# jasperlinthorst/reveal

Measured on AMD Instinct MI355X. Metric: Mbp/s indexed+MUM-anchored (reveal rem), higher is better.
Workload: dtype int32

## Files before the change

reveal_amd/csrc/rv_align.hip:

```cpp
#include "rv_index.h"
#include "rv_split.h"
#include "rv_decide.h"
static_assert(RV_TSUB_TILE == RV_SPLIT_TILE, "one tile -> sub-index table serves the split passes and the multi-sample picker");
#include "rv_leaf.h"
#include "rv_cascade.h"
#include <string.h>
#include <algorithm>
#include <chrono>
#include <thread>
#include <atomic>
#include "rv_graphrem.h"

namespace {

double now_s() {
    return std::chrono::duration<double>(std::chrono::steady_clock::now().time_since_epoch()).count();
}

u64 hash_step(u64 acc, u64 i, int64_t v) {
    u64 x = (u64)v + (i + 1) * 0x9E3779B97F4A7C15ULL;
    x ^= x >> 30; x *= 0xbf58476d1ce4e5b9ULL;
    x ^= x >> 27; x *= 0x94d049bb133111ebULL;
    x ^= x >> 31;
    return acc + x;
// ... 133 lines not shown
    bool leaf_pending[RV_LEVEL_BUFS + 1] = {};
    size_t leaf_anchor_cap = 0, leaf_trace_cap = 0;
    std::vector<uint8_t> leaf_done;
    std::vector<RvLeafRoot> leaf_roots[2];
    Packer pk;
    std::vector<int> stamp; int epoch = 0;
    std::vector<sa_t> cb, ce, mb, me, cut_lo, cut_hi, mend_pos;
    std::vector<uint8_t> cc;
    std::vector<int> ctab_first, mtab_first, cut_first, mend_first, split_subs;
    std::vector<u32> sub_off_h;
    std::vector<int> tile_sub;
    std::vector<int64_t> mpre, sub_start, woff, toff, next_ss;
    const int64_t *d_next_ss = nullptr;
    const int *d_next_want = nullptr;
    const int *d_next_tsub = nullptr;
    std::vector<int> next_tsub;
    std::vector<u32> pick_l; std::vector<sa_t> pick_pos;
    std::vector<u32> child_base, child_n;
    std::vector<RvBubbleDesc> descs;
    std::vector<std::vector<RvBubbleDesc>> rounds;
    std::vector<RvBubbleDesc> kids_small, kids_big, kids_lds;
    struct Kid { int64_t off, n; int c0, c1; int64_t m0, wsum; };
    std::vector<Kid> kid_tmp;
    std::vector<u32> an_l; std::vector<int64_t> an_off, an_pos;
    bool trace_on = false;
    std::vector<rv_trace> trace;
    rv_align_stats st{};
    double lg[8] = {0}, lgx[8] = {0}, lg_t0 = 0;
    int leaf_flip = 0;
    bool leaf_launch_due = false, hook_early = false;
    size_t last_leaf_count = 0;
    bool running = false;
    u32 *lf_counters = nullptr; unsigned long long *lf_stats = nullptr; u32 *lf_l = nullptr; int64_t *lf_pos = nullptr; rv_trace *lf_tr = nullptr;
    size_t leaf_na = 0;
    void release() {
        if (leaf_stream) (void)hipStreamSynchronize(leaf_stream);
        if (leaf_stream2) (void)hipStreamSynchronize(leaf_stream2);
        if (bub_stream) { (void)hipStreamSynchronize(bub_stream); (void)hipStreamSynchronize(bub_stream2); }
        for (int k = 0; k < RV_LEVEL_BUFS; k++) { lvSA[k].release(); lvLCP[k].release(); lvBWT[k].release(); }
        scrSA.release(); scrLCP.release(); scrBWT.release(); cas.release();
        dTmin.release(); dPbReady.release(); dNextTsub.release(); dD.release(); dTab.release(); dTile.release(); dList.release(); dFlag.release(); dPar.release(); dDbg.release(); pk.release(); dDec.release(); dErr.release(); dTab0.release(); hLeafRoots[0].release(); hLeafRoots[1].release(); hLeafOut.release(); dLeaf.release(); dLeafRoots[0].release(); dLeafRoots[1].release();
        if (leaf_stream) { rv_stream_put(leaf_stream); leaf_stream = nullptr; }
        if (leaf_stream2) { rv_stream_put(leaf_stream2); leaf_stream2 = nullptr; }
        if (bub_stream) { rv_stream_put(bub_stream); bub_stream = nullptr; rv_stream_put(bub_stream2); bub_stream2 = nullptr; (void)hipEventDestroy(ev_fork); (void)hipEventDestroy(ev_join); (void)hipEventDestroy(ev_join2); ev_fork = ev_join = ev_join2 = nullptr; }
        if (ev_ready) { (void)hipEventDestroy(ev_ready); ev_ready = nullptr; }
        for (int k = 0; k <= RV_LEVEL_BUFS; k++) if (ev_leaf[k]) { (void)hipEventDestroy(ev_leaf[k]); ev_leaf[k] = nullptr; }
        for (int k = 0; k < 2; k++) if (ev_roots[k]) { (void)hipEventDestroy(ev_roots[k]); ev_roots[k] = nullptr; }
    }
};

void rv_align_free(rv_index *h) {
    if (h->al && h->al->feed) { (void)rv_replay_feed_finish(h->al->feed); h->al->feed = nullptr; }
    if (h->al) { h->al->release(); delete h->al; h->al = nullptr; }
}

static int report_dev_err(u32 err) {
    if (err & 1u) { rv_set_error("split: the intervals returned by graphalign do not partition the sub-index (child size mismatch)"); return -1; }
    if (err & 4u) { rv_set_error("device-side decision: a picked match does not lie inside the intervals of its sub-index"); return -1; }
    if (err & 2u) { rv_set_error("bubble_sort (data-parallel rounds): a mover found no landing site"); return -1; }
    if (err & 16u) { rv_set_error("bubble_sort (data-parallel rounds): a tile waited in vain for the tile above it (workgroups not dispatched in index order?)"); return -1; }
    if (err) { rv_set_error("device-side error word %u", err); return -1; }
    return 0;
}

static int64_t bubble_par_default(bool multi) { return multi ? (int64_t)262144 : (int64_t)RV_BUBBLE_PAR_N; }

// ... 342 lines not shown
        d.child_n = t.child_n; d.child_base = t.child_base; d.sub_off = t.sub_off; d.expect_total = t.expect_total;
        d.err = a->dErr.as<u32>();
        d.kid = kid;
    };
    if (a->multi) {
        RvDecideMultiArgs d;
        outputs(d);
        d.W = W; d.minl = a->minl; d.minn = a->minn;
        d.nodes = a->d_next_nodes; d.want = a->d_next_want;
        d.pick_l = h->ws.misc[13].as<u32>(); d.pick_pos = h->ws.misc[7].as<sa_t>();
        d.cand_count = h->ws.misc[1].as<u32>() + RV_MULTI_REGIONS * 64;
        d.cand_cap = (u32)std::min<size_t>(h->ws.misc[8].cap / RV_MULTI_CAND_BYTES / RV_MULTI_REGIONS, 0xffffffffu);
        RV_TRY(rv_decide_multi_launch(h->ws, d));
    } else {
        RvDecideArgs d;
        outputs(d);
        d.nodes = a->d_next_nodes; d.flags = a->d_next_flags; d.picks = h->hscan.as<RvPairRec>();
        d.ovf_cap = (u32)std::min<size_t>(h->ws.misc[4].cap / sizeof(RvPairRec), 0xffffffffu);
        RV_TRY(rv_decide_launch(h->ws, d));
    }
    RvLabelTabs lt; RvSplitArgs sa;
    split_args(h, t, nxt, lt, sa);
    int64_t biggest = 0;
    for (int s2 = 0; s2 < ns; s2++) biggest = std::max<int64_t>(biggest, lv.n[(size_t)s2]);
    if (biggest > a->par_min_cur) RV_TRY(tmin_preset(h, sa));
    int id = h->prof.begin(q, RV_K_SPLIT, (double)m * (2 * (sizeof(sa_t) + sizeof(lcp_t) + 2)) + (double)m * (sizeof(sa_t) + sizeof(lcp_t) + 1));
    RV_TRY(rv_split_launch(h->ws, cur_sa(h), cur_lcp(h), a->dD.as<uint8_t>(), cur_bwt(h), m, lt, sa, 1));
    h->prof.end(q, id);
    a->early_done = true;
    a->early_bubble = false;
    const bool all_classes = a->multi || ns > 4096;
    if (biggest <= a->par_min_cur && !h->ws.opt.no_early_bubble &&
        (a->multi || (!h->ws.opt.bubble_lds_always && (!all_classes || h->ws.opt.early_bubble_many)))) {
        RV_TRY(rv_lower_ranges_launch(h->ws, h->dT.as<uint8_t>(), t.mb, t.me, W * ns));
        RV_TRY(bubble_flags(h, m));
        RvBubbleArgs ba;
        memset(&ba, 0, sizeof ba);
        ba.flag = a->dFlag.as<uint8_t>();
        ba.SA = sa.SA_out; ba.LCP = sa.LCP_out; ba.BWT = sa.BWT_out; ba.SAi = sa.SAi; ba.cut_lo = t.cut_lo; ba.cut_hi = t.cut_hi; ba.err = a->dErr.as<u32>();
        id = h->prof.begin(q, RV_K_BUBBLE, 0.0);
        if (!all_classes) {
            RV_TRY(rv_bubble_children_dev_launch(h->ws, ba, kid, ns, a->par_min_cur));
        } else {
            RV_TRY(bubble_fork(h, true, true, true));
            Workspace wl, wk; wl.stream = a->bub_stream; wk.stream = a->bub_stream2;
            RV_TRY(rv_bubble_children_dev_classes_launch(wl, wk, ba, kid, ns, a->par_min_cur));
            RV_TRY(bubble_join(h, true, true));
        }
        h->prof.end(q, id);
        a->early_bubble = true;
    }
    return 0;
}

static int level_hook(rv_index *h) {
    Align *a = h->al;
    if (a->hook_early) RV_TRY(early_split(h));
    if (a->leaf_launch_due) RV_TRY(leaf_launch(h));
    return 0;
}

static void build_preselection(Align *a) {
    const int ns = a->lv.size();
    a->sel.clear(); a->sel_first.assign((size_t)ns + 1, 0);
    std::vector<int64_t> &tmp = a->sel_tmp;
    for (int s = 0; s < ns; s++) {
// ... 589 lines not shown
        a->d_next_tsub = a->dNextTsub.as<int>();
    }
    return 0;
}

static int commit_split(rv_index *h, const Commit &cm, RvSplitArgs &sa) {
    Align *a = h->al;
    hipStream_t q = h->ws.stream;
    const Level &lv = a->lv;
    const int nxt = cm.nxt;
    uint8_t *tb = a->dTab.as<uint8_t>();
    RV_TRY(split_reserve(h, nxt, lv.m, cm.m_next));
    RV_TRY(a->dList.reserve((size_t)a->woff.back() * 4 + 64));
    RV_TRY(leaf_wait(h, nxt));
    if (h->ws.opt.bubble_parent_scratch && !a->descs.empty()) RV_TRY(leaf_wait(h, a->level == 0 ? RV_LEVEL_BUFS : a->cur));
    SplitTabs t;
    t.sub_start = (const int64_t *)(tb + cm.o_ss); t.tile_sub = (const int *)(tb + cm.o_tsub);
    t.ctab_first = (int *)(tb + cm.o_ctf); t.mtab_first = (int *)(tb + cm.o_mtf); t.cut_first = (int *)(tb + cm.o_cf); t.mend_first = (int *)(tb + cm.o_mf);
    t.cb = (sa_t *)(tb + cm.o_cb); t.ce = (sa_t *)(tb + cm.o_ce); t.cc = tb + cm.o_cc; t.mb = (sa_t *)(tb + cm.o_mb); t.me = (sa_t *)(tb + cm.o_me);
    t.cut_lo = (sa_t *)(tb + cm.o_clo); t.cut_hi = (sa_t *)(tb + cm.o_chi); t.mend_pos = (sa_t *)(tb + cm.o_mp);
    t.child_n = (u32 *)(tb + cm.o_cn); t.child_base = (u32 *)(tb + cm.o_cbase); t.sub_off = (u32 *)(tb + cm.o_suboff); t.expect_total = (u32 *)(tb + cm.o_expect);
    t.total = (u32 *)(tb + cm.o_total);
    t.nmatch = (int)a->mb.size();
    RvLabelTabs lt;
    split_args(h, t, nxt, lt, sa);
    sa.mend_all = a->dec.host_lists ? 1 : 0;
    int id = a->early_done ? -1 : h->prof.begin(q, RV_K_SPLIT, (double)lv.m * (2 * (sizeof(sa_t) + sizeof(lcp_t) + 2)) + (double)cm.m_next * (sizeof(sa_t) + sizeof(lcp_t) + 1));
    if (!a->early_done) {
        if (!a->descs.empty()) RV_TRY(tmin_preset(h, sa));
        RV_TRY(rv_split_launch(h->ws, cur_sa(h), cur_lcp(h), a->dD.as<uint8_t>(), cur_bwt(h), lv.m, lt, sa, (int)a->split_subs.size()));
    }
    h->prof.end(q, id);
    if (!a->early_bubble) {
        if (lt.nmatch > 256 && a->mpre.back() / lt.nmatch <= 512) RV_TRY(rv_lower_ranges_launch(h->ws, h->dT.as<uint8_t>(), lt.mbegin, lt.mend, lt.nmatch));
        else RV_TRY(rv_lower_launch(h->ws, h->dT.as<uint8_t>(), lt.mbegin, lt.mend, (const int64_t *)(tb + cm.o_mpre), lt.nmatch, a->mpre.back()));
    }
    return 0;
}

static int commit_bubble(rv_index *h, const Commit &cm, const RvSplitArgs &sa) {
    Align *a = h->al;
    hipStream_t q = h->ws.stream;
    uint8_t *tb = a->dTab.as<uint8_t>();
    const int64_t m_next = cm.m_next;
    if (a->descs.empty() && a->kids_small.empty() && a->kids_big.empty() && a->kids_lds.empty()) return 0;
    RvBubbleArgs ba;
    ba.desc = (const RvBubbleDesc *)(tb + cm.o_desc); ba.woff = (const int64_t *)(tb + cm.o_woff);
    ba.cnt = (u32 *)(tb + cm.o_bcnt); ba.list = a->dList.as<u32>();
    RV_TRY(bubble_flags(h, m_next));
    ba.flag = a->dFlag.as<uint8_t>();
    ba.SA = sa.SA_out; ba.LCP = sa.LCP_out; ba.BWT = sa.BWT_out; ba.SAi = sa.SAi; ba.cut_lo = sa.cut_lo; ba.cut_hi = sa.cut_hi; ba.err = sa.err;
    ba.state = (RvBubbleState *)(tb + cm.o_bstate);
    ba.dbg = nullptr;
    if (h->ws.opt.level_log) { if (!a->dDbg.p) { RV_TRY(a->dDbg.reserve(64)); RV_HIP(hipMemsetAsync(a->dDbg.p, 0, 64, q)); } ba.dbg = a->dDbg.as<unsigned long long>(); }
    ba.scrSA = const_cast<sa_t *>(cur_sa(h)); ba.scrLCP = const_cast<lcp_t *>(cur_lcp(h)); ba.scrBWT = const_cast<uint8_t *>(cur_bwt(h));
    if (!a->descs.empty() && !h->ws.opt.bubble_parent_scratch) {
        RV_TRY(a->scrSA.reserve((size_t)(m_next + 64) * sizeof(sa_t)));
        RV_TRY(a->scrLCP.reserve((size_t)(m_next + 64) * sizeof(lcp_t)));
        RV_TRY(a->scrBWT.reserve((size_t)m_next + 64));
        ba.scrSA = a->scrSA.as<sa_t>(); ba.scrLCP = a->scrLCP.as<lcp_t>(); ba.scrBWT = a->scrBWT.as<uint8_t>();
    }
    if (!a->descs.empty()) {
        const size_t W = (size_t)a->woff.back() + 16, TT = (size_t)a->toff.back() + 16;
        RV_TRY(a->dPar.reserve(TT * 4 + W * (8 + 7 * 4 + sizeof(sa_t) + 2) + 256));
        uint8_t *pb = a->dPar.as<uint8_t>();
        ba.par.toff = (const int64_t *)(tb + cm.o_toff);
// ... 94 lines not shown

static int builtin_leaf_setup(rv_index *h) {
    Align *a = h->al;
    hipStream_t q = h->ws.stream;
    a->use_leaf = !a->multi && !h->ws.opt.no_leaf && a->picker == 0;
    a->leaf_flip = 0;
    if (!a->use_leaf) return 0;
    a->leaf_anchor_cap = (size_t)(h->nT / std::max(a->minl, 1)) + 1024;
    a->leaf_trace_cap = a->trace_on ? 2 * a->leaf_anchor_cap + 1024 : 0;
    const size_t bytes = 256 + a->leaf_anchor_cap * (4 + 8 + 8) + a->leaf_trace_cap * sizeof(rv_trace) + 64;
    RV_TRY(a->dLeaf.reserve(bytes));
    uint8_t *base = a->dLeaf.as<uint8_t>();
    a->lf_counters = (u32 *)base;
    a->lf_stats = (unsigned long long *)(base + 64);
    a->lf_pos = (int64_t *)(base + 256); a->lf_l = (u32 *)(a->lf_pos + 2 * a->leaf_anchor_cap);
    a->lf_tr = (rv_trace *)(base + 256 + a->leaf_anchor_cap * 20 + ((8 - (a->leaf_anchor_cap * 20) % 8) % 8));
    RV_HIP(hipMemsetAsync(base, 0, 256, q));
    if (!a->leaf_stream) {
        RV_HIP(rv_stream_get(&a->leaf_stream));
        RV_HIP(rv_stream_get(&a->leaf_stream2));
        RV_HIP(hipEventCreateWithFlags(&a->ev_ready, hipEventDisableTiming));
        for (int k = 0; k <= RV_LEVEL_BUFS; k++) RV_HIP(hipEventCreateWithFlags(&a->ev_leaf[k], hipEventDisableTiming));
        for (int k = 0; k < 2; k++) RV_HIP(hipEventCreateWithFlags(&a->ev_roots[k], hipEventDisableTiming));
    }
    for (int k = 0; k <= RV_LEVEL_BUFS; k++) a->leaf_pending[k] = false;
    a->roots_inflight[0] = a->roots_inflight[1] = false;
    return 0;
}

static int builtin_setup(rv_index *h, int minl, int minn) {
    RV_TRY(align_begin(h, minl, minn, h->al && h->al->trace_on));
    Align *a = h->al;
    a->full_only = !a->trace_on && a->picker == 0;
    a->an_l.clear(); a->an_off.assign(1, 0); a->an_pos.clear(); a->trace.clear(); a->leaf_na = 0;
    a->seeds_cur.clear(); a->seeds_lead.clear(); a->seeds_trail.clear(); a->picker_calls = a->picker_seeded = 0; a->picker_ns = a->picker_list_ns = a->galign_ns = 0;
    if (a->picker == 1) {
        if ((int)h->nodes.size() != h->nsamples) { rv_set_error("the native picker (rv_set_picker) takes one sequence per sample: %d sequences in %d samples", (int)h->nodes.size(), h->nsamples); return -1; }
        if (h->rc) { rv_set_error("the native picker (rv_set_picker) with construct(rc=1) is not supported"); return -1; }
    }
    if (a->picker != 0 && a->multi && !a->trace_on) { a->presel_on = true; a->pick_filter = true; }
    else a->pick_filter = false;
    if (a->picker == 2) {
        if (!a->ggraph) { rv_set_error("rv_set_graph_picker: no graph"); return -1; }
        if (h->rc) { rv_set_error("the native picker (rv_set_graph_picker) with construct(rc=1) is not supported"); return -1; }
        a->g_left.assign((size_t)a->lv.size(), RvGraphIv{-1, -1}); a->g_right.assign((size_t)a->lv.size(), RvGraphIv{-1, -1});
    }
    const bool use_leaf = !a->multi && !h->ws.opt.no_leaf && a->picker == 0;
    a->use_leaf = use_leaf;
    if (!a->multi && a->full_only && h->n < ((int64_t)1 << 32)) {
        prep_level_tables(h, a->lv, h->n);
        if (a->next_dev_ok) {
            a->pk.clear();
            RV_TRY(publish_next_tables(h, a->dTab0, a->lv.nsamples, false));
            a->cur_dev_ok = true;
        }
    }
    RV_TRY(builtin_leaf_setup(h));
    a->running = true;
    return 0;
}

struct PickScratch {
    std::vector<u32> pk_l, pk_sl; std::vector<int32_t> pk_n, pk_sn; std::vector<int64_t> pk_off, pk_mpos, pk_sb, pk_ib, pk_ie, pk_soff, pk_spos, pk_ssc;
    std::vector<uint16_t> pk_mso, pk_sso; std::vector<uint8_t> pk_srt;
};
struct PickRes {
    int rc = -9;
// ... 352 lines not shown
        const size_t lo = na / nt * t, hi = t + 1 == nt ? na : na / nt * (t + 1);
        th.emplace_back([=]() { for (size_t k = lo; k < hi; k++) off[k] = base + 2 * (int64_t)(k + 1); });
    }
    for (size_t k = 0; k < na / nt; k++) off[k] = base + 2 * (int64_t)(k + 1);
    for (auto &x : th) x.join();
}
static int builtin_finish(rv_index *h, rv_align_stats *out) {
    Align *a = h->al;
    hipStream_t q = h->ws.stream;
    h->rb.direct = false;
    if (a->use_leaf && a->running) {
        u32 *lf_counters = a->lf_counters; u32 *lf_l = a->lf_l; int64_t *lf_pos = a->lf_pos; rv_trace *lf_tr = a->lf_tr;
        RV_HIP(hipStreamSynchronize(a->leaf_stream));
        RV_HIP(hipStreamSynchronize(a->leaf_stream2));
        for (int k = 0; k <= RV_LEVEL_BUFS; k++) a->leaf_pending[k] = false;
        RV_TRY(a->hLeafOut.reserve(256));
        RV_HIP(hipMemcpyAsync(a->hLeafOut.p, lf_counters, 128, hipMemcpyDeviceToHost, q));
        RV_HIP(hipStreamSynchronize(q));
        u32 cnt[4]; unsigned long long stv[8];
        memcpy(cnt, a->hLeafOut.p, sizeof cnt); memcpy(stv, a->hLeafOut.as<uint8_t>() + 64, sizeof stv);
        if (h->ws.opt.leaf_prof)
            fprintf(stderr, "leaf: steps %llu splits %llu | cycles idle %llu scan %llu split %llu bubble %llu\n", stv[0], stv[1], stv[4], stv[5], stv[6], stv[7]);
        if (cnt[2]) { rv_set_error(cnt[2] & 4u ? "leaf kernel: recursion stack overflow" : "leaf kernel: a sub-index does not match its intervals"); return -1; }
        if (cnt[0] > a->leaf_anchor_cap || cnt[1] > a->leaf_trace_cap) { rv_set_error("leaf kernel: output buffer too small"); return -1; }
        a->leaf_na = 0;
        if (cnt[0]) {
            const size_t na = cnt[0];
            const size_t nl = a->an_l.size(), np = a->an_pos.size();
            rv_index::ResultBufs &rb = h->rb;
            rb.direct = rb.l && (int64_t)(nl + na) <= rb.l_cap && (int64_t)(nl + na + 1) <= rb.off_cap && (int64_t)(np + 2 * na) <= rb.pos_cap;
            int64_t *pp; u32 *pl;
            if (rb.direct) { pp = rb.pos + np; pl = rb.l + nl; }
            else { RV_TRY(a->hLeafOut.reserve(na * 20 + 64)); pp = a->hLeafOut.as<int64_t>(); pl = (u32 *)(pp + 2 * na); }
            RV_HIP(hipMemcpyAsync(pp, lf_pos, na * 16, hipMemcpyDeviceToHost, a->leaf_stream));
            RV_HIP(hipMemcpyAsync(pl, lf_l, na * 4, hipMemcpyDeviceToHost, a->leaf_stream));
            RV_TRY(rv_leaf_lower_launch(h->ws, h->dT.as<uint8_t>(), lf_pos, lf_l, (u32)na));
            if (rb.direct) fill_offsets(rb.off + nl + 1, na, (int64_t)np);
            RV_HIP(hipStreamSynchronize(a->leaf_stream));
            RV_HIP(hipStreamSynchronize(q));
            a->leaf_na = na;
        }
        if (a->trace_on && cnt[1]) {
            const size_t at = a->trace.size();
            a->trace.resize(at + cnt[1]);
            RV_HIP(hipMemcpy(a->trace.data() + at, lf_tr, (size_t)cnt[1] * sizeof(rv_trace), hipMemcpyDeviceToHost));
        }
        a->st.steps += (int64_t)stv[0]; a->st.splits += (int64_t)stv[1]; a->st.anchored_bp += (int64_t)stv[2];
        if ((int64_t)stv[3] > a->st.maxdepth) a->st.maxdepth = (int32_t)stv[3];
    }
    a->running = false;
    if (out) *out = a->st;
    return 0;
}

static int install_frontier(rv_index *h, int level, int nsubs, const int64_t *meta, const int64_t *node_first, const int64_t *nodes, int64_t m,
                            const void *sa, const void *lcp, const void *bwt, int on_device);
static int builtin_cascade(rv_index *h) {
    Align *a = h->al;
    memset(&a->cas_out, 0, sizeof a->cas_out);
    if (a->trace_on || h->rc != 0 || h->n <= RV_LEAF_N || a->minl < 4 || h->ws.opt.no_cascade || a->picker != 0) return 0;
    const bool second_try = !a->multi && a->use_leaf && h->ws.opt.cascade_second == 2;
    auto interval_cascade = [&]() -> int {
        RvCascadeMultiOut mo;
        RV_TRY(rv_cascade_multi_run(h, a->cas, a->minl, &mo));
        a->cas_out.done = mo.done; a->cas_out.levels = mo.levels; a->cas_out.cands = mo.cands; a->cas_out.witnesses = mo.witnesses; a->cas_out.children = mo.children;
        a->cas_out.undecided = mo.undecided; a->cas_out.rebuilt_ranks = mo.rebuilt_ranks; a->cas_out.why = mo.why;
        if (!mo.done) return 0;
        const int k = h->nsamples;
        a->st.splits += (int64_t)mo.an_l.size(); a->st.steps += mo.steps; a->st.levels += mo.levels; a->st.scanned_ranks += h->n;
        if (mo.maxdepth > a->st.maxdepth) a->st.maxdepth = mo.maxdepth;
        h->main_arrays_freed = true;
        if (mo.undecided > 0) {
            RV_TRY(install_frontier(h, 1, (int)mo.undecided, mo.meta.data(), mo.node_first.data(), mo.nodes.data(), mo.rebuilt_ranks, mo.d_sa, mo.d_lcp, mo.d_bwt, 1));
        } else {
            a->lv.clear();
            a->level = 1;
        }
        {
            const size_t na = mo.an_l.size(), l0 = a->an_l.size(), p0 = a->an_pos.size(), o0 = a->an_off.size();
            a->an_l.insert(a->an_l.end(), mo.an_l.begin(), mo.an_l.end());
            a->an_pos.resize(p0 + na * (size_t)k);
            for (size_t x = 0; x < na * (size_t)k; x++) a->an_pos[p0 + x] = (int64_t)mo.an_pos[x];
            a->an_off.resize(o0 + na);
            for (size_t x = 0; x < na; x++) a->an_off[o0 + x] = (int64_t)(p0 + (x + 1) * (size_t)k);
            int64_t bp = 0;
            for (size_t x = 0; x < na; x++) bp += mo.an_l[x];
            a->st.anchored_bp += bp;
            (void)l0;
        }
        return 0;
    };
    if (a->multi || second_try) return interval_cascade();
    if (!a->use_leaf) return 0;
    RvCascadeIO io;
    io.anchor_count = a->lf_counters; io.anchor_cap = (u32)a->leaf_anchor_cap; io.anchor_l = a->lf_l; io.anchor_pos = a->lf_pos;
    io.stats = a->lf_stats; io.leaf_err = a->lf_counters + 2;
    io.stage_cap = (u32)h->ws.opt.leaf_acap;
    io.lvSA = &a->lvSA[0]; io.lvLCP = &a->lvLCP[0]; io.lvBWT = &a->lvBWT[0]; io.roots = &a->dLeafRoots[0];
    const int dmode = (int)h->ws.opt.cascade_danger;
    RV_TRY(rv_cascade_run(h, a->cas, io, a->minl, &a->cas_out, dmode == 2 ? 1 : 0, 0));
    if (!a->cas_out.done && a->cas_out.undecided > 0 && dmode == 1) {
        RV_HIP(hipMemsetAsync(a->dLeaf.p, 0, 256, h->ws.stream));
        RV_TRY(rv_cascade_run(h, a->cas, io, a->minl, &a->cas_out, 1, 1));
    }
    if (!a->cas_out.done) {
        RV_HIP(hipMemsetAsync(a->dLeaf.p, 0, 256, h->ws.stream));
        if (a->cas_out.undecided > 0 && !h->ws.opt.cascade_second_off) return interval_cascade();
        return 0;
    }
    a->st.levels += a->cas_out.levels;
    a->st.scanned_ranks += h->n;
    if (!a->cas.lin_rest.empty() && h->nodes.size() > 2) {
        std::vector<RvIntv> rest, gone;
        for (size_t k = 0; k + 1 < a->cas.lin_rest.size(); k += 2) rest.push_back({a->cas.lin_rest[k], a->cas.lin_rest[k + 1]});
        std::sort(rest.begin(), rest.end(), intv_less);
        for (const RvIntv &v : h->nodes) {
            if (v.end <= v.begin) continue;
            const auto it = std::lower_bound(rest.begin(), rest.end(), v, intv_less);
            if (it == rest.end() || it->begin != v.begin) gone.push_back(v);
        }
        RV_TRY(add_decision(h, 0, 0, nullptr, 0, gone.data(), (int)gone.size(), nullptr, 0, nullptr, 0, rest.data(), (int)rest.size()));
        a->dec.drop_lead = true;
        RV_TRY(rv_frontier_commit(h, nullptr));
        for (size_t s2 = 0; s2 < a->lv.depth.size(); s2++) a->lv.depth[s2] = a->cas.lin_rest_depth;
        return 0;
    }
    h->main_arrays_freed = true;
    a->level = 1;
    a->lv.clear();
    return 0;
}

int rv_cascade_info(const rv_index *h, int64_t *out) {
    for (int k = 0; k < 8; k++) out[k] = 0;
    if (!h->al) return 0;
    const RvCascadeOut &c = h->al->cas_out;
    out[0] = c.done ? 1 : 0; out[1] = c.levels; out[2] = c.cands; out[3] = c.witnesses; out[4] = c.children; out[5] = c.undecided; out[6] = c.rebuilt_ranks; out[7] = c.solved;
    return 0;
}

const char *rv_cascade_why(const rv_index *h) {
    if (!h->al || h->al->cas_out.done || !h->al->cas_out.why) return "";
    return h->al->cas_out.why;
}
// ... 143 lines not shown
    return 0;
}


int rv_frontier_import(rv_index *h, int minl, int minn, uint32_t maxlcp, int level, int nsubs, const int64_t *meta,
                       const int64_t *node_first, const int64_t *nodes, int64_t m, const void *sa, const void *lcp, const void *bwt, int on_device) {
    RV_HIP(hipSetDevice(h->device));
    if (h->nsamples < 2) { rv_set_error("align needs at least two samples"); return -1; }
    if (nsubs < 0 || m < 0 || m >= ((int64_t)1 << 32)) { rv_set_error("rv_frontier_import: bad sizes"); return -1; }
    const bool fresh = !(h->al && h->al->running);
    if (fresh) {
        if (h->text_only) h->maxlcp = maxlcp;
        else if (!h->constructed || h->main_arrays_freed) RV_TRY(rv_text_only(h, maxlcp));
        const bool keep_trace = h->al && h->al->trace_on;
        if (!h->al) h->al = new Align();
        Align *a = h->al;
        a->trace_on = keep_trace;
        a->minl = minl; a->minn = minn;
        a->multi = h->nsamples > 2;
        a->scanned = false; a->d_err = nullptr; a->flag_clean = false;
        a->next_dev_ok = a->cur_dev_ok = a->early_done = a->early_bubble = false;
        a->par_min_cur = (h->ws.opt.bubble_par_min >= 0 ? h->ws.opt.bubble_par_min : bubble_par_default(a->multi));
        RV_TRY(a->dErr.reserve(64));
        memset(&a->st, 0, sizeof a->st);
        a->full_only = !a->trace_on && a->picker == 0;
        a->pick_filter = a->picker != 0 && a->multi && !a->trace_on;
        if (a->pick_filter) a->presel_on = true;
        if (a->picker == 2) { rv_set_error("rv_frontier_import: a run on a graph (rv_set_graph_picker) is not handed off -- its sub-indices share the graph"); return -1; }
        if (a->picker == 1) {
            if ((int)h->nodes.size() != h->nsamples) { rv_set_error("the native picker (rv_set_picker) takes one sequence per sample: %d sequences in %d samples", (int)h->nodes.size(), h->nsamples); return -1; }
            if (h->rc) { rv_set_error("the native picker (rv_set_picker) with construct(rc=1) is not supported"); return -1; }
        }
        a->picker_calls = a->picker_seeded = 0; a->picker_ns = a->picker_list_ns = a->galign_ns = 0;
        a->an_l.clear(); a->an_off.assign(1, 0); a->an_pos.clear(); a->trace.clear(); a->leaf_na = 0;
        RV_TRY(builtin_leaf_setup(h));
    }
    RV_TRY(install_frontier(h, level, nsubs, meta, node_first, nodes, m, sa, lcp, bwt, on_device));
    h->al->running = true;
    return 0;
}

int64_t rv_frontier_seeds_export(rv_index *h, const int32_t *subs, int k, int64_t *out, int64_t cap) {
    if (need_align(h)) return -1;
    const Align *a = h->al;
    const int ns = a->lv.size();
    int64_t need = 0;
    for (int pass = 0; pass < 2; pass++) {
        int64_t at = 0;
        for (int i = 0; i < k; i++) {
            const int s = subs[i];
            if (s < 0 || s >= ns) { rv_set_error("sub-index %d out of range", s); return -1; }
            const Align::SeedList *sd = (s < (int)a->seeds_cur.size() && a->seeds_cur[(size_t)s].size() > 0) ? &a->seeds_cur[(size_t)s] : nullptr;
            if (pass) out[at] = sd ? (int64_t)sd->size() : 0;
            at++;
            if (!sd) continue;
            for (size_t r = 0; r < sd->size(); r++) {
                const int64_t mem = sd->off[r + 1] - sd->off[r];
                if (pass) {
                    out[at] = sd->l[r]; out[at + 1] = sd->n[r]; out[at + 2] = sd->score[r]; out[at + 3] = mem;
                    for (int64_t q2 = 0; q2 < mem; q2++) { out[at + 4 + 2 * q2] = sd->so[(size_t)(sd->off[r] + q2)]; out[at + 5 + 2 * q2] = sd->pos[(size_t)(sd->off[r] + q2)]; }
                }
                at += 4 + 2 * mem;
            }
        }
        need = at;
        if (!out || cap < need) break;
    }
// ... 370 lines not shown
```

reveal_amd/csrc/rv_api.hip:

```cpp
#include "rv_index.h"
#include "rv_cascade.h"
#include <limits>
#include <stdarg.h>
#include <stdio.h>
#include <string.h>
#include <limits.h>
#include <algorithm>
#include <thread>

static thread_local char g_err[1024] = "";

void rv_set_error(const char *fmt, ...) {
    va_list ap;
    va_start(ap, fmt);
    vsnprintf(g_err, sizeof g_err, fmt, ap);
    va_end(ap);
}

static std::vector<rv_index *> &live_handles() { static std::vector<rv_index *> v; return v; }
std::mutex &rv_trim_mutex() { static std::mutex *m = new std::mutex(); return *m; }
bool rv_oom_trim() {
    size_t got = 0;
    bool log = false;
    int caller_dev = 0;
// ... 40 lines not shown
        rv_set_error("device %d is %s; this library is built for gfx950 (MI355X) only", device, prop.gcnArchName);
        return nullptr;
    }
    rv_index *h = new rv_index();
    h->device = device;
    if (rv_stream_get(&h->ws.stream) != hipSuccess) {
        rv_set_error("hipStreamCreate failed");
        delete h;
        return nullptr;
    }
    h->T.push_back('\0');
    h->ws.prof_ctx = &h->prof;
    h->ws.prof_begin_fn = [](void *c, hipStream_t st, int k, double b) { return ((RvProf *)c)->begin(st, k, b); };
    h->ws.prof_end_fn = [](void *c, hipStream_t st, int id) { ((RvProf *)c)->end(st, id); };
    { std::lock_guard<std::mutex> g(rv_trim_mutex()); live_handles().push_back(h); }
    return h;
}

void rv_free(rv_index *h) {
    if (!h) return;
    { std::lock_guard<std::mutex> g(rv_trim_mutex()); auto &v = live_handles(); v.erase(std::remove(v.begin(), v.end(), h), v.end()); }
    (void)hipSetDevice(h->device);
    if (h->ws.stream) (void)hipStreamSynchronize(h->ws.stream);
    h->rb.direct = false;
    (void)rv_set_result_buffers(h, nullptr, 0, nullptr, 0, nullptr, 0);
    rv_align_free(h);
    h->prof.release();
    h->dT.release(); h->dT0.release(); h->dSA.release(); h->dSAi.release(); h->dLCP.release(); h->dBWT.release(); h->dNsep.release();
    h->ws.release();
    h->hscan.release();
    for (auto &b : h->ps) b.release();
    h->hupload.release();
    if (h->ev_picks) { (void)hipEventDestroy(h->ev_picks); h->ev_picks = nullptr; }
    if (h->ws.stream) rv_stream_put(h->ws.stream);
    delete h;
}

int rv_set_option(rv_index *h, const char *name, int64_t value) {
    if (!h || !name) { rv_set_error("rv_set_option: null argument"); return -1; }
    int64_t *f = h->ws.opt.find(name);
    if (!f) { rv_set_error("rv_set_option: unknown option %s", name); return -1; }
    *f = value;
    return 0;
}
int rv_set_launch_trace(int on) {
    const int was = g_rv_launch_trace;
    g_rv_launch_trace = on != 0;
    return was;
}
int rv_get_option(rv_index *h, const char *name, int64_t *value) {
    if (!h || !name || !value) { rv_set_error("rv_get_option: null argument"); return -1; }
    const int64_t *f = h->ws.opt.find(name);
    if (!f) { rv_set_error("rv_get_option: unknown option %s", name); return -1; }
    *value = *f;
    return 0;
}
int rv_option_count(void) {
    int c = 0;
#define RV_X_(f, nm, def) c++;
    RV_OPTION_LIST(RV_X_)
#undef RV_X_
    return c;
}
const char *rv_option_name(int k) {
    static const char *const names[] = {
#define RV_X_(f, nm, def) nm,
        RV_OPTION_LIST(RV_X_)
#undef RV_X_
    };
    return k >= 0 && k < rv_option_count() ? names[k] : nullptr;
}

rv_index *rv_clone(rv_index *h) {
    if (!h->constructed || h->main_arrays_freed) { rv_set_error("Index not yet constructed."); return nullptr; }
    if (rv_need_sai(h)) return nullptr;
    rv_index *c = rv_new(h->device);
    if (!c) return nullptr;
    try { c->T = h->T; c->nsep = h->nsep; c->nodes = h->nodes; }
    catch (...) { rv_set_error("copy of the index: out of host memory"); rv_free(c); return nullptr; }
    if (c->T.size() != h->T.size()) { rv_free(c); return nullptr; }
    c->nsamples = h->nsamples; c->n = h->n; c->nT = h->nT; c->rc = h->rc;
    c->maxlcp = h->maxlcp; c->sa_stats = h->sa_stats; c->text_dirty = true;
    c->ws.opt = h->ws.opt;
    const int64_t n = h->n;
    hipStream_t q = c->ws.stream;
    bool ok = rv_upload(c) == 0;
    ok = ok && c->dT.reserve((size_t)n + 64) == 0 && c->dSA.reserve((size_t)(n + 64) * sizeof(sa_t)) == 0 && c->dSAi.reserve((size_t)(n + 64) * sizeof(sa_t)) == 0
            && c->dLCP.reserve((size_t)(n + 64) * sizeof(lcp_t)) == 0 && c->dBWT.reserve((size_t)n + 64) == 0 && c->dNsep.reserve((h->nsep.size() + 1) * sizeof(sa_t)) == 0;
    ok = ok && hipStreamSynchronize(h->ws.stream) == hipSuccess;
    ok = ok && hipMemcpyAsync(c->dT.p, h->dT.p, (size_t)n + 64, hipMemcpyDeviceToDevice, q) == hipSuccess;
    ok = ok && hipMemcpyAsync(c->dSA.p, h->dSA.p, (size_t)n * sizeof(sa_t), hipMemcpyDeviceToDevice, q) == hipSuccess;
    ok = ok && hipMemcpyAsync(c->dSAi.p, h->dSAi.p, (size_t)n * sizeof(sa_t), hipMemcpyDeviceToDevice, q) == hipSuccess;
    ok = ok && hipMemcpyAsync(c->dLCP.p, h->dLCP.p, (size_t)n * sizeof(lcp_t), hipMemcpyDeviceToDevice, q) == hipSuccess;
    ok = ok && hipMemcpyAsync(c->dBWT.p, h->dBWT.p, (size_t)n, hipMemcpyDeviceToDevice, q) == hipSuccess;
    ok = ok && hipMemcpyAsync(c->dNsep.p, h->dNsep.p, (h->nsep.size() + 1) * sizeof(sa_t), hipMemcpyDeviceToDevice, q) == hipSuccess;
    ok = ok && hipStreamSynchronize(q) == hipSuccess;
    if (!ok) { rv_set_error("copy of the index failed"); rv_free(c); return nullptr; }
    c->nsep_dev = h->nsep_dev;
    c->constructed = true; c->sai_valid = true;
    return c;
}

int rv_add_sample(rv_index *h) {
    if (h->nsamples > 0) h->nsep.push_back(h->n - 1);
    h->nsamples++;
    h->constructed = false; h->text_only = false;
    return 0;
}

int rv_add_sequence(rv_index *h, const char *seq, int64_t len, int64_t *begin, int64_t *end) {
    if (len < 0 || !seq) { rv_set_error("addsequence: bad sequence"); return -1; }
#ifndef RV_SA64
    if ((uint64_t)h->n + (uint64_t)(len + 1) + 1 > (uint64_t)INT_MAX) {
        rv_set_error("Total amount of sequence too large, use \"reveal <subcommand> --64\" to use 64 bit suffix arrays instead.");
        return -1;
    }
#endif
    const int64_t s = h->n;
    if ((size_t)(h->n + len + 2) > h->T.cap) (void)hipSetDevice(h->device);
// ... 198 lines not shown
            RV_HIP(hipMemcpyAsync(h->dT0.as<char>() + at, dst, len, hipMemcpyHostToDevice, q));
            RV_HIP(hipEventRecord(ev[slot], q));
            used[slot] = true;
        }
        RV_HIP(hipStreamSynchronize(q));
    }
    RV_HIP(hipStreamSynchronize(q));
    h->text_dirty = false;
    return 0;
}

int rv_upload_again(rv_index *h) {
    h->text_dirty = true;
    return rv_upload(h);
}

int rv_construct(rv_index *h, int rc, const char *safile, const char *lcpfile, int cache) {
    RV_HIP(hipSetDevice(h->device));
    if (rc == 1) {
        if (h->nsep.empty()) { rv_set_error("construct(rc=1) needs at least two samples"); return -1; }
        h->rc = 1;
        revcomp(h->T.data() + h->nsep[0], h->n - h->nsep[0]);
        h->text_dirty = true;
    } else {
        h->rc = 0;
    }
    if (h->n == 0) { rv_set_error("No text to index."); return -1; }
    const int64_t n = h->n;
    if (n >= ((int64_t)1 << 32) - 2) { rv_set_error("index of %lld positions: this build carries ranks in 32 bits (n < 2^32 - 2)", (long long)n); return -1; }
    if (cache == 1) RV_TRY(write_raw(".reveal.t", h->T.data(), (size_t)n));
    if (h->al) (void)rv_align_end(h);
    h->nT = n;
    hipStream_t q = h->ws.stream;
    RV_TRY(rv_upload(h));
    RV_TRY(h->dT.reserve((size_t)n + 64));
    RV_HIP(hipMemcpyAsync(h->dT.p, h->dT0.p, (size_t)n + 64, hipMemcpyDeviceToDevice, q));
    RV_TRY(h->dSA.reserve((size_t)(n + 64) * sizeof(sa_t)));
    RV_TRY(h->dSAi.reserve((size_t)(n + 64) * sizeof(sa_t)));
    RV_TRY(h->dLCP.reserve((size_t)(n + 64) * sizeof(lcp_t)));
    RV_TRY(h->dBWT.reserve((size_t)n + 64));
    memset(&h->sa_stats, 0, sizeof h->sa_stats);
    RV_TRY(h->ws.misc[0].reserve(64));
    u32 *d_max = h->ws.misc[0].as<u32>();
    const sa_t side_sep = !h->nsep.empty() ? (sa_t)h->nsep[0] : std::numeric_limits<sa_t>::max();
    const bool lcp_from_file = lcpfile && lcpfile[0];
    bool lcp_done = false;
    SaScratchInUse in_use(h->ws);
    if (!safile || !safile[0]) {
        int id = h->prof.begin(q, RV_K_SA_SORT, 5.0 * (double)n);
        if (lcp_from_file) RV_TRY(rv_build_sa(h->ws, h->dT.as<uint8_t>(), n, h->dSA.as<sa_t>(), &h->sa_stats));
        else RV_TRY(rv_build_sa(h->ws, h->dT.as<uint8_t>(), n, h->dSA.as<sa_t>(), &h->sa_stats, h->dLCP.as<lcp_t>(), h->dBWT.as<uint8_t>(), side_sep, d_max, &lcp_done,
                                 h->nsep.data(), (int)h->nsep.size()));
        h->prof.end(q, id);
    } else {
        std::vector<sa_t> tmp((size_t)n);
        RV_TRY(read_raw(safile, tmp.data(), (size_t)n * sizeof(sa_t)));
        RV_HIP(hipMemcpyAsync(h->dSA.p, tmp.data(), (size_t)n * sizeof(sa_t), hipMemcpyHostToDevice, q));
        RV_HIP(hipStreamSynchronize(q));
    }
    h->sai_valid = false;
    if (safile && safile[0]) { RV_TRY(rv_build_inverse_checked(h->ws, h->dSA.as<sa_t>(), h->dSAi.as<sa_t>(), n)); h->sai_valid = true; }
    if (!lcp_from_file) {
        if (!lcp_done) {
            int id = h->prof.begin(q, RV_K_LCP, 13.0 * (double)n);
            RV_TRY(rv_build_lcp(h->ws, h->dT.as<uint8_t>(), h->dSA.as<sa_t>(), false, h->dLCP.as<lcp_t>(), n, d_max, h->dBWT.as<uint8_t>(), side_sep));
            h->prof.end(q, id);
        }
        RV_TRY(rv_read_back(h->ws, &h->maxlcp, d_max, 4));
    } else {
        std::vector<lcp_t> tmp((size_t)n);
        RV_TRY(read_raw(lcpfile, tmp.data(), (size_t)n * sizeof(lcp_t)));
        u32 mx = 0;
        for (int64_t i = 0; i < n; i++) if ((u32)tmp[(size_t)i] > mx) mx = (u32)tmp[(size_t)i];
        h->maxlcp = mx;
        RV_HIP(hipMemcpyAsync(h->dLCP.p, tmp.data(), (size_t)n * sizeof(lcp_t), hipMemcpyHostToDevice, q));
        RV_TRY(rv_build_bwt(h->ws, h->dT.as<uint8_t>(), h->dSA.as<sa_t>(), n, h->dBWT.as<uint8_t>(), side_sep));
        RV_HIP(hipStreamSynchronize(q));
    }
    if (cache == 1) {
        std::vector<sa_t> sa((size_t)n);
        std::vector<lcp_t> lc((size_t)n);
        RV_HIP(hipMemcpy(sa.data(), h->dSA.p, (size_t)n * sizeof(sa_t), hipMemcpyDeviceToHost));
        RV_HIP(hipMemcpy(lc.data(), h->dLCP.p, (size_t)n * sizeof(lcp_t), hipMemcpyDeviceToHost));
        RV_TRY(write_raw(".reveal.sa", sa.data(), (size_t)n * sizeof(sa_t)));
        RV_TRY(write_raw(".reveal.lcp", lc.data(), (size_t)n * sizeof(lcp_t)));
    }
    {
        if (h->nsep_dev != h->nsep || !h->dNsep.p) {
            std::vector<sa_t> ns(h->nsep.size() + 1, 0);
            for (size_t k = 0; k < h->nsep.size(); k++) ns[k] = (sa_t)h->nsep[k];
            RV_TRY(h->dNsep.reserve(ns.size() * sizeof(sa_t)));
            RV_HIP(hipMemcpy(h->dNsep.p, ns.data(), ns.size() * sizeof(sa_t), hipMemcpyHostToDevice));
            h->nsep_dev = h->nsep;
        }
    }
    h->constructed = true;
    h->main_arrays_freed = false;
    h->text_only = false;
    return 0;
}

int64_t rv_get_array(rv_index *h, int which, void *out, int64_t cap) {
    (void)hipSetDevice(h->device);
    const int64_t n = h->n;
    switch (which) {
    case RV_T:
        if (cap < n) { rv_set_error("buffer too small"); return -1; }
        if (h->constructed || h->text_only) {
            if (hipMemcpy(out, h->dT.p, (size_t)n, hipMemcpyDeviceToHost) != hipSuccess) { rv_set_error("D2H failed"); return -1; }
        } else {
            memcpy(out, h->T.data(), (size_t)n);
        }
        return n;
    case RV_SA: case RV_SAI: case RV_LCP: {
        if (!h->constructed || (which != RV_SAI && h->main_arrays_freed)) { rv_set_error("Index not yet constructed."); return -2; }
        if (which == RV_SAI && rv_need_sai(h)) return -2;
        if (cap < h->nT && which == RV_SAI) { rv_set_error("buffer too small"); return -1; }
        if (cap < n && which != RV_SAI) { rv_set_error("buffer too small"); return -1; }
        const void *src = which == RV_SA ? h->dSA.p : which == RV_SAI ? h->dSAi.p : h->dLCP.p;
        const size_t esz = which == RV_LCP ? sizeof(lcp_t) : sizeof(sa_t);
        const int64_t cnt = which == RV_SAI ? h->nT : n;
        (void)hipStreamSynchronize(h->ws.stream);
        if (hipMemcpy(out, src, (size_t)cnt * esz, hipMemcpyDeviceToHost) != hipSuccess) { rv_set_error("D2H failed"); return -1; }
        return cnt;
    }
    case RV_SO: {
        if (!h->constructed || h->nsamples <= 2) { rv_set_error("SO not available."); return -2; }
        if (cap < h->nT) { rv_set_error("buffer too small"); return -1; }
        uint16_t *so = (uint16_t *)out;
        int64_t j = 0;
        for (int i = 0; i < h->nsamples; i++) {
            const int64_t hi = (i == h->nsamples - 1) ? h->nT - 1 : h->nsep[(size_t)i];
            for (; j <= hi; j++) so[j] = (uint16_t)i;
        }
        return h->nT;
    }
    case RV_NSEP:
        if (cap < (int64_t)h->nsep.size()) { rv_set_error("buffer too small"); return -1; }
        for (size_t k = 0; k < h->nsep.size(); k++) ((int64_t *)out)[k] = h->nsep[k];
        return (int64_t)h->nsep.size();
    case RV_NODES:
        if (cap < (int64_t)h->nodes.size() * 2) { rv_set_error("buffer too small"); return -1; }
        for (size_t k = 0; k < h->nodes.size(); k++) { ((int64_t *)out)[2 * k] = h->nodes[k].begin; ((int64_t *)out)[2 * k + 1] = h->nodes[k].end; }
        return (int64_t)h->nodes.size() * 2;
    }
    rv_set_error("unknown array id %d", which);
    return -1;
}

}

int rv_need_sai(rv_index *h) {
    if (h->sai_valid) return 0;
    if (!h->constructed || h->main_arrays_freed) { rv_set_error("the inverse suffix array was not requested before align() consumed the main index"); return -1; }
    RV_HIP(hipSetDevice(h->device));
    RV_TRY(rv_build_inverse(h->ws, h->dSA.as<sa_t>(), h->dSAi.as<sa_t>(), h->n));
    h->sai_valid = true;
    return 0;
}

int rv_text_only(rv_index *h, u32 maxlcp) {
    RV_HIP(hipSetDevice(h->device));
    if (h->n == 0) { rv_set_error("No text to index."); return -1; }
    if (h->nsep.empty()) { rv_set_error("a worker index needs at least two samples"); return -1; }
    const int64_t n = h->n;
    hipStream_t q = h->ws.stream;
    h->rc = 0; h->nT = n;
    RV_TRY(rv_upload(h));
    RV_TRY(h->dT.reserve((size_t)n + 64));
    RV_HIP(hipMemcpyAsync(h->dT.p, h->dT0.p, (size_t)n + 64, hipMemcpyDeviceToDevice, q));
    RV_TRY(h->dSAi.reserve((size_t)(n + 64) * sizeof(sa_t)));
    std::vector<sa_t> ns(h->nsep.size() + 1, 0);
    for (size_t k = 0; k < h->nsep.size(); k++) ns[k] = (sa_t)h->nsep[k];
    RV_TRY(h->dNsep.reserve(ns.size() * sizeof(sa_t)));
    RV_HIP(hipMemcpy(h->dNsep.p, ns.data(), ns.size() * sizeof(sa_t), hipMemcpyHostToDevice));
    h->nsep_dev = h->nsep;
    RV_HIP(hipStreamSynchronize(q));
    h->maxlcp = maxlcp;
    h->constructed = false; h->main_arrays_freed = true; h->text_only = true; h->sai_valid = false;
    return 0;
}

namespace {
__global__ __launch_bounds__(256) void k_ps_keys(const RvPairRec *__restrict__ recs, u32 total, const int64_t *__restrict__ ss, int ns, u64 *__restrict__ keys, u32 *__restrict__ vals) {
    const u32 i = blockIdx.x * 256u + threadIdx.x;
    if (i >= total) return;
    const int64_t r = (int64_t)recs[i].rank;
    int lo = 0, hi = ns;
    while (hi - lo > 1) { const int mid = (lo + hi) >> 1; if (ss[mid] <= r) lo = mid; else hi = mid; }
    keys[i] = ((u64)(u32)lo << 32) | (u64)recs[i].l;
    vals[i] = i;
}
__global__ __launch_bounds__(256) void k_ps_mark(const u64 *__restrict__ skeys, const u32 *__restrict__ svals, u32 total, u32 presel, u32 *__restrict__ flag) {
    const u32 p = blockIdx.x * 256u + threadIdx.x;
    if (p >= total) return;
    const u64 next = ((skeys[p] >> 32) + 1ull) << 32;
    u32 lo = p, hi = total;
    while (hi - lo > 1) { const u32 mid = lo + ((hi - lo) >> 1); if (skeys[mid] < next) lo = mid; else hi = mid; }
    flag[svals[p]] = (hi - p <= presel) ? 1u : 0u;
}
__global__ __launch_bounds__(256) void k_ps_emit(const RvPairRec *__restrict__ recs, const u32 *__restrict__ flag, const u32 *__restrict__ off, u32 total, RvPairRec *__restrict__ out) {
    const u32 i = blockIdx.x * 256u + threadIdx.x;
    if (i < total && flag[i]) out[off[i]] = recs[i];
// ... 588 lines not shown
```

reveal_amd/csrc/rv_cascade.h:

```cpp
#pragma once
#include "rv_common.h"
#include <vector>

struct RvCascadeBufs {
    DBuf d[40];
    HBuf hstage, hstage2;
    u32 M = 0, NW = 0;
    u32 lin_roots = 0, lin_picks = 0, lin_nA = 0, lin_nB = 0;
    int64_t lin_steps = 0; int lin_maxdepth = 0; size_t lin_off[6] = {0, 0, 0, 0, 0, 0};
    std::vector<int64_t> lin_rest; int lin_rest_depth = 0;
    hipStream_t prio_stream = nullptr; hipEvent_t ev_in = nullptr, ev_out = nullptr;
    void release() {
        for (auto &b : d) b.release(); hstage.release(); hstage2.release();
        if (prio_stream) { (void)hipStreamDestroy(prio_stream); prio_stream = nullptr; }
        if (ev_in) { (void)hipEventDestroy(ev_in); ev_in = nullptr; }
        if (ev_out) { (void)hipEventDestroy(ev_out); ev_out = nullptr; }
    }
};

struct RvCascadeIO {
    u32 *anchor_count; u32 anchor_cap; u32 *anchor_l; int64_t *anchor_pos;
    unsigned long long *stats;
    u32 *leaf_err;
    u32 stage_cap;
    DBuf *lvSA, *lvLCP, *lvBWT, *roots;
};

struct RvCascadeOut {
    bool done;
    int levels;
    int64_t cands, witnesses, children, undecided, rebuilt_ranks;
    int64_t solved, unsolved;
    const char *why;
};

#define RV_CASM_K 16
struct RvCascadeMultiOut {
    bool done; int levels; int64_t cands, witnesses, children, undecided, rebuilt_ranks, steps; int maxdepth; const char *why;
    int64_t big, big_ranks;
    std::vector<u32> an_l; std::vector<int64_t> an_pos;
    std::vector<int64_t> meta, node_first, nodes;
    const void *d_sa, *d_lcp, *d_bwt;
};

struct rv_index;
struct RvBatchGroup;
RvBatchGroup *rv_batch_group_new(int device);
void rv_batch_group_begin(RvBatchGroup *g, int total);
void rv_batch_group_leave(RvBatchGroup *g);
void rv_batch_group_free(RvBatchGroup *g);
void rv_batch_group_info(const RvBatchGroup *g, int64_t *out);
int rv_cascade_multi_run(rv_index *h, RvCascadeBufs &cb, int minl, RvCascadeMultiOut *out);
int rv_cascade_run(rv_index *h, RvCascadeBufs &cb, const RvCascadeIO &io, int minl, RvCascadeOut *out, int danger = 0, int reuse = 0);
```

reveal_amd/csrc/rv_cascade.hip:

```cpp
#include "rv_index.h"
#include "rv_cascade.h"
#include "rv_leaf.h"
#include <algorithm>
#include <string.h>
#include <stdio.h>
#include <stdlib.h>
#include <chrono>

namespace {

constexpr int TB = 256;
constexpr u32 NONE = 0xFFFFFFFFu;
#ifdef RV_SA64
constexpr int KEY_SHIFT = 40;
#else
constexpr int KEY_SHIFT = 32;
#endif
constexpr u64 KEY_LOW = (1ull << KEY_SHIFT) - 1;

struct CasIv { sa_t a0, a1, b0, b1; };
struct CasRes { sa_t qa, qb; u32 ql, lead, trail, state; };
enum { C_NCHILD = 0, C_NUND = 1, C_NWIT = 2, C_ERR = 3, C_MAXN = 4, C_LO = 5, C_HI = 6, C_LEVELS = 7, C_NSOLVED = 8, C_NUNSOLVED = 9, C_NRETRY = 10, C_TICKET = 11 };

__device__ inline bool cas_cut(const CasIv &iv, int64_t pa, int64_t pb, int64_t len, int64_t minl, int64_t *qa, int64_t *qb, int64_t *ql) {
    const int64_t ka = (int64_t)iv.a0 - pa, kb = (int64_t)iv.b0 - pb;
    int64_t k = ka > kb ? ka : kb;
    k = k > 0 ? k : 0;
    const int64_t a = pa + k, b = pb + k;
    int64_t l = len - k;
    const int64_t ra = (int64_t)iv.a1 - a, rb = (int64_t)iv.b1 - b;
    l = l < ra ? l : ra;
    l = l < rb ? l : rb;
    *qa = a; *qb = b; *ql = l;
    return l >= minl;
}
__device__ inline u64 cas_key(int64_t qa, int64_t ql) { return ((u64)ql << KEY_SHIFT) | (KEY_LOW - (u64)qa); }

__device__ inline u64 shfl_up64(u64 v, int d) {
    const u32 lo = __shfl_up((u32)v, d, 64), hi = __shfl_up((u32)(v >> 32), d, 64);
    return ((u64)hi << 32) | lo;
}
__device__ inline void seg_atomic_max64(u64 *__restrict__ dst, u32 child, u64 val, bool active) {
    const int lane = threadIdx.x & 63;
    if (!active) { child = NONE; val = 0; }
    val = rv_wave_seg_max_u64(child, val);
    const u32 nc = __shfl_down(child, 1, 64);
    const bool last = lane == 63 || nc != child;
    if (active && last && val > dst[child]) atomicMax((unsigned long long *)&dst[child], (unsigned long long)val);
}
__device__ inline void seg_atomic_max32(u32 *__restrict__ dst, u32 child, u32 val, bool active) {
    const int lane = threadIdx.x & 63;
    if (!active) { child = NONE; val = 0; }
    val = rv_wave_seg_max_u32(child, val);
    const u32 nc = __shfl_down(child, 1, 64);
    const bool last = lane == 63 || nc != child;
// ... 501 lines not shown
                    iv[slot] = c; best[slot] = 0; wmax[slot] = 0; depth[slot] = dp + 1; res[slot] = nr;
                    if (danger) { dg.best[slot] = 0; dg.flag[slot] = 0; dg.ceil[slot] = 0; }
                    r.lead = slot;
                } else atomicOr(&counters[C_ERR], 1u);
                slot++;
            }
            if (trail) {
                if (slot < child_cap) {
                    CasIv c; c.a0 = (sa_t)((int64_t)r.qa + r.ql); c.a1 = p.a1; c.b0 = (sa_t)((int64_t)r.qb + r.ql); c.b1 = p.b1;
                    iv[slot] = c; best[slot] = 0; wmax[slot] = 0; depth[slot] = dp + 1; res[slot] = nr;
                    if (danger) { dg.best[slot] = 0; dg.flag[slot] = 0; dg.ceil[slot] = 0; }
                    r.trail = slot;
                } else atomicOr(&counters[C_ERR], 1u);
            }
            const u32 as = base_a + (u32)__popcll(b_split & lt);
            if (as < io.anchor_cap) { io.anchor_l[as] = r.ql; io.anchor_pos[2 * (size_t)as] = (int64_t)r.qa; io.anchor_pos[2 * (size_t)as + 1] = (int64_t)r.qb; }
            else atomicOr(&counters[C_ERR], 4u);
            r.state = 1;
        } else {
            r.state = 2;
        }
        if (in) res[id] = r;
        if (und) {
            und_list[base_u + (u32)__popcll(b_und & lt)] = id;
            if ((u64)(la + lb) > (u64)leaf_n) atomicMax(&counters[C_MAXN], (u32)((la + lb) > 0xFFFFFFFFll ? 0xFFFFFFFFll : (la + lb)));
        }
        __syncthreads();
    }
    if (threadIdx.x == 0) {
        __threadfence();
        if (atomicAdd(&counters[C_TICKET], 1u) == gridDim.x - 1) {
            if (hi > lo) counters[C_LEVELS]++;
            counters[C_LO] = hi; counters[C_HI] = atomicAdd(&counters[C_NCHILD], 0u);
            counters[C_TICKET] = 0;
        }
    }
}
__global__ __launch_bounds__(TB) void k_cas_stats(const u32 *__restrict__ counters, const int32_t *__restrict__ depth, RvCascadeIO io) {
    __shared__ unsigned long long s_bp[TB / 64];
    __shared__ u32 s_md[TB / 64];
    const u32 nchild = counters[C_NCHILD], na = *io.anchor_count;
    unsigned long long bp = 0; u32 md = 0;
    for (u32 i = blockIdx.x * TB + threadIdx.x; i < na; i += gridDim.x * TB) bp += io.anchor_l[i];
    for (u32 i = blockIdx.x * TB + threadIdx.x; i < nchild; i += gridDim.x * TB) { const u32 d = (u32)depth[i]; md = d > md ? d : md; }
#pragma unroll
    for (int d = 32; d >= 1; d >>= 1) {
        bp += ((unsigned long long)(u32)__shfl_down((u32)(bp >> 32), d, 64) << 32) + (unsigned long long)(u32)__shfl_down((u32)bp, d, 64);
        const u32 om = __shfl_down(md, d, 64);
        md = om > md ? om : md;
    }
    if ((threadIdx.x & 63) == 0) { s_bp[threadIdx.x >> 6] = bp; s_md[threadIdx.x >> 6] = md; }
    __syncthreads();
    if (threadIdx.x == 0) {
        for (int k = 1; k < TB / 64; k++) { bp += s_bp[k]; md = s_md[k] > md ? s_md[k] : md; }
        if (bp) atomicAdd(&io.stats[2], bp);
        if (md) atomicMax(&io.stats[3], (unsigned long long)md);
        if (blockIdx.x == 0) { atomicAdd(&io.stats[0], (unsigned long long)(nchild - counters[C_NUND] - counters[C_NRETRY])); atomicAdd(&io.stats[1], (unsigned long long)na); }
    }
}

__global__ __launch_bounds__(TB) void k_cas_sizes(const u32 *__restrict__ und_list, u32 U, const CasIv *__restrict__ iv, u64 *__restrict__ sizes) {
    const u32 u = blockIdx.x * TB + threadIdx.x;
    if (u < U) { const CasIv p = iv[und_list[u]]; sizes[u] = (u64)(((int64_t)p.a1 - p.a0) + ((int64_t)p.b1 - p.b0)); }
    if (u == U) sizes[u] = 0;
}
__global__ __launch_bounds__(TB) void k_cas_roots(const u32 *__restrict__ und_list, u32 U, const CasIv *__restrict__ iv, const int32_t *__restrict__ depth,
// ... 187 lines not shown
    if (nLiveA + nLiveB > 0) {
        if (stalled || (nLiveA && nLiveB && chain_wmax() >= minl)) {
            for (size_t c = 0; c < nA; c++) if (liveA[c]) { cb.lin_rest.push_back(CA[c].begin); cb.lin_rest.push_back(CA[c].end); }
            for (size_t c = 0; c < nB; c++) if (liveB[c]) { cb.lin_rest.push_back(CB[c].begin); cb.lin_rest.push_back(CB[c].end); }
        } else { steps++; maxdepth = depth; }
    }
    const u32 R = (u32)roots.size(), P = (u32)anl.size();
    RV_TRY(broots.reserve((size_t)std::max<u32>(R, 1) * sizeof(CasIv))); RV_TRY(bdepth.reserve((size_t)std::max<u32>(R, 1) * 4));
    const size_t tab_bytes = (nA + nB) * (sizeof(sa_t) + 4) + (size_t)P * 8 + 64;
    RV_TRY(btabs.reserve(tab_bytes + 64)); RV_TRY(banch.reserve((size_t)P * (4 + 16) + 64));
    std::vector<uint8_t> stage(tab_bytes + 64, 0);
    size_t o = 0;
    auto put = [&](const void *src, size_t bytes) { memcpy(stage.data() + o, src, bytes); const size_t at = o; o += (bytes + 15) / 16 * 16; return at; };
    std::vector<sa_t> bA(nA), bB(nB);
    for (size_t c = 0; c < nA; c++) bA[c] = (sa_t)CA[c].begin;
    for (size_t c = 0; c < nB; c++) bB[c] = (sa_t)CB[c].begin;
    stage.resize((nA + nB) * (sizeof(sa_t) + 4) + (size_t)P * 8 + 16 * 8 + 64);
    const size_t oA = put(bA.data(), nA * sizeof(sa_t)), oB = put(bB.data(), nB * sizeof(sa_t)), opA = put(pickA.data(), nA * 4), opB = put(pickB.data(), nB * 4),
                 oL = put(rootLead.data(), (size_t)P * 4), oT = put(rootTrail.data(), (size_t)P * 4);
    RV_TRY(btabs.reserve(o + 64));
    RV_HIP(hipMemcpyAsync(btabs.p, stage.data(), o, hipMemcpyHostToDevice, q));
    if (R) {
        RV_HIP(hipMemcpyAsync(broots.p, roots.data(), (size_t)R * sizeof(CasIv), hipMemcpyHostToDevice, q));
        RV_HIP(hipMemcpyAsync(bdepth.p, rdepth.data(), (size_t)R * 4, hipMemcpyHostToDevice, q));
    }
    RV_HIP(hipMemcpyAsync(banch.p, anp.data(), (size_t)P * 16, hipMemcpyHostToDevice, q));
    RV_HIP(hipMemcpyAsync((uint8_t *)banch.p + (size_t)P * 16, anl.data(), (size_t)P * 4, hipMemcpyHostToDevice, q));
    RV_HIP(hipStreamSynchronize(q));
    cb.lin_roots = R; cb.lin_picks = P; cb.lin_nA = (u32)nA; cb.lin_nB = (u32)nB; cb.lin_steps = steps; cb.lin_maxdepth = maxdepth;
    cb.lin_off[0] = oA; cb.lin_off[1] = oB; cb.lin_off[2] = opA; cb.lin_off[3] = opB; cb.lin_off[4] = oL; cb.lin_off[5] = oT;
    return 0;
}

int rv_cascade_run(rv_index *h, RvCascadeBufs &cb, const RvCascadeIO &io, int minl_in, RvCascadeOut *out, int danger, int reuse) {
    memset(out, 0, sizeof *out);
    out->done = false;
    Workspace &ws = h->ws;
    hipStream_t q = ws.stream;
    const int64_t n = h->n;
    const u32 minl = (u32)std::max(minl_in, 1);
    const bool verbose = (ws.opt.cascade_log != 0);
    double tp[6] = {0, 0, 0, 0, 0, 0};
    if (verbose) { (void)hipStreamSynchronize(q); tp[0] = cas_now(); }
#define GIVE_UP(msg) do { out->why = msg; if (verbose) fprintf(stderr, "cascade: gave up: %s\n", msg); return 0; } while (0)
    if (h->nsamples != 2 || h->nsep.size() != 1 || h->nodes.size() < 2) GIVE_UP("not two samples");
    std::vector<RvIntv> CA, CB;
    for (const RvIntv &v : h->nodes) if (v.end > v.begin) (v.begin < h->nsep[0] ? CA : CB).push_back(v);
    std::sort(CA.begin(), CA.end(), [](const RvIntv &x, const RvIntv &y) { return x.begin < y.begin; });
    std::sort(CB.begin(), CB.end(), [](const RvIntv &x, const RvIntv &y) { return x.begin < y.begin; });
    if (CA.empty() || CB.empty()) GIVE_UP("an empty sample");
    const bool chain = CA.size() > 1 || CB.size() > 1;
    if (chain && ws.opt.no_cascade_chain) GIVE_UP("several sequences per sample (switched off)");
    if (n >= ((int64_t)1 << 32) - 2) GIVE_UP("index above 2^32 positions");
#ifdef RV_SA64
    if ((u64)h->maxlcp >= (1ull << 24) || n >= ((int64_t)1 << 40)) GIVE_UP("bid word too narrow");
#endif
    CasIv root; root.a0 = root.a1 = root.b0 = root.b1 = 0;
    root.a0 = (sa_t)CA[0].begin; root.a1 = (sa_t)CA[0].end; root.b0 = (sa_t)CB[0].begin; root.b1 = (sa_t)CB[0].end;
    if (root.a0 >= root.a1 || root.b0 >= root.b1 || (int64_t)root.a1 > h->nsep[0] || (int64_t)root.b0 <= h->nsep[0]) GIVE_UP("an empty sample");

    const sa_t *SA = h->dSA.as<sa_t>(); const lcp_t *LCP = h->dLCP.as<lcp_t>(); const uint8_t *BWT = h->dBWT.as<uint8_t>();

    const int64_t ntile = ceil_div(n, RV_PAIR_TILE);
    DBuf &bcnt = ws.misc[14], &btab = ws.misc[2], &bslot = ws.misc[3], &bovf = ws.misc[4], &bout = ws.misc[5];
    if (bcnt.cap == 0) { RV_TRY(bcnt.reserve(64)); RV_HIP(hipMemsetAsync(bcnt.p, 0, 64, q)); }
    RV_TRY(btab.reserve((size_t)(ntile + 1) * 3 * sizeof(u32)));
    RV_TRY(bslot.reserve((size_t)ntile * RV_PAIR_SLOTS * sizeof(RvPairRec)));
// ... 137 lines not shown
        }
        dg.leaf_n = (u32)ws.opt.cascade_danger_min;
    }
    const sa_t *d_beginA = nullptr, *d_beginB = nullptr;
    if (!chain) {
        hipLaunchKernelGGL(k_cas_init, dim3((unsigned)std::max<int64_t>(1, ceil_div((int64_t)NW, TB))), dim3(TB), 0, q, biv.as<CasIv>(), bbest.as<u64>(), bwm.as<u32>(),
                           bdep.as<int32_t>(), bres.as<CasRes>(), counters, root, bwc.as<u32>(), NW, dg.best, dg.flag, dg.ceil);
        RV_LAUNCH_CHECK();
    } else {
        const u32 R = cb.lin_roots, P = cb.lin_picks;
        if ((int64_t)R + 16 > (int64_t)ccap || P > io.anchor_cap) GIVE_UP("more sequences than the cascade's tables hold");
        const uint8_t *tb = cb.d[32].as<uint8_t>();
        CasRootTabs rt;
        rt.beginA = (const sa_t *)(tb + cb.lin_off[0]); rt.beginB = (const sa_t *)(tb + cb.lin_off[1]);
        rt.pickA = (const int32_t *)(tb + cb.lin_off[2]); rt.pickB = (const int32_t *)(tb + cb.lin_off[3]);
        rt.rootLead = (const u32 *)(tb + cb.lin_off[4]); rt.rootTrail = (const u32 *)(tb + cb.lin_off[5]);
        rt.nA = cb.lin_nA; rt.nB = cb.lin_nB;
        d_beginA = rt.beginA; d_beginB = rt.beginB;
        hipLaunchKernelGGL(k_cas_init_roots, dim3((unsigned)std::max<int64_t>(1, ceil_div((int64_t)R, TB))), dim3(TB), 0, q, biv.as<CasIv>(), bbest.as<u64>(), bwm.as<u32>(),
                           bdep.as<int32_t>(), bres.as<CasRes>(), counters, (const CasIv *)cb.d[30].as<CasIv>(), (const int32_t *)cb.d[31].as<int32_t>(), R, dg.best, dg.flag, dg.ceil);
        RV_LAUNCH_CHECK();
        hipLaunchKernelGGL(k_cas_assign_roots, dim3((unsigned)std::max<int64_t>(1, ceil_div((int64_t)std::max(M, NW), TB))), dim3(TB), 0, q, (const sa_t *)bpa.as<sa_t>(),
                           (const sa_t *)bpb.as<sa_t>(), (const u32 *)blen.as<u32>(), bcc.as<u32>(), M, wp, bwc.as<u32>(), NW, (const CasIv *)cb.d[30].as<CasIv>(), rt, (int64_t)minl);
        RV_LAUNCH_CHECK();
        RV_HIP(hipMemcpyAsync(io.anchor_pos, cb.d[33].p, (size_t)P * 16, hipMemcpyDeviceToDevice, q));
        RV_HIP(hipMemcpyAsync(io.anchor_l, (const uint8_t *)cb.d[33].p + (size_t)P * 16, (size_t)P * 4, hipMemcpyDeviceToDevice, q));
        RV_HIP(hipMemcpyAsync(io.anchor_count, &cb.lin_picks, 4, hipMemcpyHostToDevice, q));
    }

    if (verbose) { (void)hipStreamSynchronize(q); tp[2] = cas_now(); }
    const unsigned agrid = (unsigned)(ceil_div((int64_t)M, TB * CAS_ITEMS) + ceil_div((int64_t)NW, TB * CAS_ITEMS));
    const int batch = std::max(1, (int)ws.opt.cascade_batch);
    int queued = 0;
    struct PrioScope {
        Workspace &w; hipStream_t home; RvCascadeBufs &cb; bool on = false;
        ~PrioScope() { leave(); }
        void leave() {
            if (!on) return;
            on = false;
            (void)hipEventRecord(cb.ev_out, w.stream);
            w.stream = home;
            (void)hipStreamWaitEvent(home, cb.ev_out, 0);
        }
    } prio{ws, q, cb};
    if (ws.opt.cascade_prio) {
        if (!cb.prio_stream) {
            int plo = 0, phi = 0;
            RV_HIP(hipDeviceGetStreamPriorityRange(&plo, &phi));
            RV_HIP(hipStreamCreateWithPriority(&cb.prio_stream, hipStreamNonBlocking, phi));
            RV_HIP(hipEventCreateWithFlags(&cb.ev_in, hipEventDisableTiming));
            RV_HIP(hipEventCreateWithFlags(&cb.ev_out, hipEventDisableTiming));
        }
        RV_HIP(hipEventRecord(cb.ev_in, q));
        RV_HIP(hipStreamWaitEvent(cb.prio_stream, cb.ev_in, 0));
        ws.stream = cb.prio_stream; prio.on = true;
        q = cb.prio_stream;
    }
    for (;;) {
        for (int b = 0; b < batch; b++, queued++) {
            hipLaunchKernelGGL(k_cas_assign, dim3(agrid), dim3(TB), 0, q, (const sa_t *)bpa.as<sa_t>(), (const sa_t *)bpb.as<sa_t>(), (const u32 *)blen.as<u32>(), bcc.as<u32>(), M,
                               wp, wv, bwc.as<u32>(), NW, (const CasIv *)biv.as<CasIv>(), (const CasRes *)bres.as<CasRes>(),
                               bbest.as<u64>(), bwm.as<u32>(), (int64_t)minl, queued == 0 ? 1 : 0, (const u64 *)((danger && NW) ? dg.ceil : nullptr));
            RV_LAUNCH_CHECK();
            hipLaunchKernelGGL(k_cas_winner, dim3((unsigned)ceil_div((int64_t)M, TB)), dim3(TB), 0, q, (const sa_t *)bpa.as<sa_t>(), (const sa_t *)bpb.as<sa_t>(),
                               (const u32 *)blen.as<u32>(), (const u32 *)bcc.as<u32>(), M, (const CasIv *)biv.as<CasIv>(), bres.as<CasRes>(), (const u64 *)bbest.as<u64>(), (int64_t)minl);
            RV_LAUNCH_CHECK();
            if (danger && NW) {
                const unsigned wb = (unsigned)ceil_div((int64_t)NW, TB);
                hipLaunchKernelGGL(k_cas_dmark, dim3(256), dim3(TB), 0, q, (const CasIv *)biv.as<CasIv>(), (const u64 *)bbest.as<u64>(), (const u32 *)bwm.as<u32>(), minl, (const u32 *)counters, dg);
                RV_LAUNCH_CHECK();
                hipLaunchKernelGGL(k_cas_dwalk, dim3(wb), dim3(TB), 0, q, wp, wv, (const u32 *)bwc.as<u32>(), NW, (const CasIv *)biv.as<CasIv>(), (const u64 *)bbest.as<u64>(),
                                   (const u32 *)bwm.as<u32>(), minl, dg);
                RV_LAUNCH_CHECK();
                if (dwalk_nmed) {
                    hipLaunchKernelGGL(k_cas_dwalk_blk, dim3((unsigned)dwalk_nmed), dim3(TB), 0, q, wp, wv, (const u32 *)bwc.as<u32>(), dwalk_boff, dwalk_mlist, dwalk_nmed,
                                       (const CasIv *)biv.as<CasIv>(), (const u64 *)bbest.as<u64>(), (const u32 *)bwm.as<u32>(), minl, dg);
                    RV_LAUNCH_CHECK();
                }
                hipLaunchKernelGGL(k_cas_dpick, dim3(wb), dim3(TB), 0, q, wp, wv, (const u32 *)bwc.as<u32>(), NW, (const CasIv *)biv.as<CasIv>(), (const CasRes *)bres.as<CasRes>(),
                                   (const u64 *)bbest.as<u64>(), (const u32 *)bwm.as<u32>(), minl, dg);
                RV_LAUNCH_CHECK();
                hipLaunchKernelGGL(k_cas_dwrite, dim3(wb), dim3(TB), 0, q, wp, (const u32 *)bwc.as<u32>(), NW, dg);
                RV_LAUNCH_CHECK();
            }
            hipLaunchKernelGGL(k_cas_decide, dim3(256), dim3(TB), 0, q, biv.as<CasIv>(), bbest.as<u64>(), bwm.as<u32>(), bdep.as<int32_t>(),
                               bres.as<CasRes>(), minl, counters, ccap, bund.as<u32>(), (u32)RV_LEAF_N, io, dg, (danger && NW) ? 1 : 0);
            RV_LAUNCH_CHECK();
        }
        RV_TRY(rv_read_back(ws, hc, counters, sizeof hc));
        if (hc[C_ERR] & ~5u) { rv_set_error("cascade: device error %u", hc[C_ERR]); return -1; }
        if (hc[C_ERR]) GIVE_UP("the cascade's tables are full");
        if (hc[C_MAXN] > (u32)RV_LEAF_N) break;
        if (hc[C_HI] == hc[C_LO]) break;
        if (queued > 1000000) { rv_set_error("cascade: no progress"); return -1; }
    }
    prio.leave(); q = ws.stream;
    const int level = (int)hc[C_LEVELS];
    const u32 hi = hc[C_NCHILD];
    if (verbose) tp[3] = cas_now();
    out->levels = level; out->children = hi; out->solved = hc[C_NSOLVED]; out->unsolved = hc[C_NUNSOLVED];
    const u32 U = hc[C_NUND];
    out->undecided = U;
    if (hc[C_MAXN] > (u32)RV_LEAF_N) {
        out->why = "an undecided sub-index above the leaf kernel's size";
        if (verbose) fprintf(stderr, "cascade%s: gave up: %s (%u ranks; %u levels, %u sub-indices, %u undecided, %u decided from witnesses, %u not)\n", danger ? " (second attempt)" : "", out->why, hc[C_MAXN], level, hi, U, hc[C_NSOLVED], hc[C_NUNSOLVED]);
        return 0;
    }
    hipLaunchKernelGGL(k_cas_stats, dim3(256), dim3(TB), 0, q, (const u32 *)counters, (const int32_t *)bdep.as<int32_t>(), io);
    RV_LAUNCH_CHECK();
    if (chain) {
        hipLaunchKernelGGL(k_cas_lineage_stats, dim3(1), dim3(64), 0, q, io.stats, (unsigned long long)cb.lin_steps, (unsigned long long)cb.lin_maxdepth);
        RV_LAUNCH_CHECK();
    }
    if (U > 0) {
        RV_TRY(bsz.reserve((size_t)(U + 1) * 8));
        u64 *sizes = bsz.as<u64>();
        hipLaunchKernelGGL(k_cas_sizes, dim3((unsigned)ceil_div((int64_t)U + 1, TB)), dim3(TB), 0, q, (const u32 *)bund.as<u32>(), U, (const CasIv *)biv.as<CasIv>(), sizes);
        RV_LAUNCH_CHECK();
        RV_TRY(rv_exclusive_sum_u64(ws, sizes, sizes, (int64_t)U + 1));
        u64 mu = 0;
        RV_TRY(rv_read_back(ws, &mu, sizes + U, 8));
        out->rebuilt_ranks = (int64_t)mu;
        RV_TRY(io.lvSA->reserve((size_t)(mu + 64) * sizeof(sa_t))); RV_TRY(io.lvLCP->reserve((size_t)(mu + 64) * sizeof(lcp_t))); RV_TRY(io.lvBWT->reserve((size_t)mu + 64));
        RV_TRY(io.roots->reserve((size_t)U * sizeof(RvLeafRoot)));
        RvLeafRoot *roots = io.roots->as<RvLeafRoot>();
        hipLaunchKernelGGL(k_cas_roots, dim3((unsigned)ceil_div((int64_t)U, TB)), dim3(TB), 0, q, (const u32 *)bund.as<u32>(), U, (const CasIv *)biv.as<CasIv>(),
                           (const int32_t *)bdep.as<int32_t>(), (const u64 *)sizes, roots);
        RV_LAUNCH_CHECK();
        DBuf &bord = cb.d[26];
        RV_TRY(bord.reserve((size_t)(mu + 64) * 2));
        hipLaunchKernelGGL(k_cas_rank, dim3(U, BN / TB), dim3(TB), 0, q, (const RvLeafRoot *)roots, (const uint8_t *)h->dT0.as<uint8_t>(), bord.as<uint16_t>());
        RV_LAUNCH_CHECK();
        hipLaunchKernelGGL(k_cas_emit, dim3(U, BN / TB), dim3(TB), 0, q, (const RvLeafRoot *)roots, (const uint8_t *)h->dT0.as<uint8_t>(), (const uint16_t *)bord.as<uint16_t>(),
                           io.lvSA->as<sa_t>(), io.lvLCP->as<lcp_t>(), io.lvBWT->as<uint8_t>(), h->nsep[0], (int64_t)root.a0, (int64_t)root.b0,
                           d_beginA, cb.lin_nA, d_beginB, cb.lin_nB);
        RV_LAUNCH_CHECK();
        RvLeafArgs la;
        la.roots = roots;
        la.SA = io.lvSA->as<sa_t>(); la.LCP = io.lvLCP->as<lcp_t>(); la.BWT = io.lvBWT->as<uint8_t>();
        la.nsep0 = h->nsep[0]; la.minl = minl_in; la.lcap = h->maxlcp;
        la.stage_cap = io.stage_cap;
        la.anchor_count = io.anchor_count; la.anchor_cap = io.anchor_cap; la.anchor_l = io.anchor_l; la.anchor_pos = io.anchor_pos;
        la.stats = io.stats;
        la.trace = 0; la.trace_count = io.anchor_count + 1; la.trace_cap = 0; la.trace_out = nullptr;
        la.err = io.leaf_err;
        RV_TRY(rv_leaf_launch(ws, la, (int)U));
    }
    if (verbose) {
        (void)hipStreamSynchronize(q); tp[4] = cas_now();
        fprintf(stderr, "cascade%s: %u matches, %u witnesses, %d levels, %u sub-indices, %u undecided (%lld ranks rebuilt), %lld decided from witnesses | ms: scan %.2f witnesses+sort %.2f levels %.2f rebuild+leaf %.2f\n",
                danger ? " (second attempt)" : "", M, NW, level, hi, U, (long long)out->rebuilt_ranks, (long long)out->solved, (tp[1] - tp[0]) * 1e3, (tp[2] - tp[1]) * 1e3, (tp[3] - tp[2]) * 1e3, (tp[4] - tp[3]) * 1e3);
    }
    out->done = true;
    return 0;
#undef GIVE_UP
}
```

reveal_amd/csrc/rv_cascade_multi.hip:

```cpp
#include "rv_index.h"
#include "rv_cascade.h"
#include "rv_leaf.h"
#include <algorithm>
#include <chrono>
#include <condition_variable>
#include <mutex>
#include <string.h>
#include <stdio.h>
#include <stdlib.h>

namespace {

constexpr int TB = 256;
constexpr u32 NONE = 0xFFFFFFFFu;
#ifdef RV_SA64
constexpr int KEY_SHIFT = 40;
#else
constexpr int KEY_SHIFT = 32;
#endif
constexpr u64 KEY_LOW = (1ull << KEY_SHIFT) - 1;
enum { C_NCHILD = 0, C_NUND = 1, C_NWIT = 2, C_ERR = 3, C_MAXN = 4, C_LO = 5, C_HI = 6, C_LEVELS = 7, C_NCAND = 8, C_NANCH = 9, C_STEPS = 10, C_MAXDEPTH = 11, C_TICKET = 12, C_BIGERR = 13, C_BIGTOT = 14  };

__device__ inline int cm_sample(const sa_t *__restrict__ nsep, int k, sa_t pos) {
    int s = 0;
// ... 1057 lines not shown
        for (u32 u2 = 0; u2 < U; u2++) {
            const u32 j = r_job[u2];
            if (j >= (u32)J) return 0;
            RvBatchJob &x = *jobs[j];
            x.und_id.push_back(r_id[u2]); x.und_dep.push_back(r_dep[u2]);
            int64_t sz = 0;
            for (int s2 = 0; s2 < k; s2++) {
                x.und_b.push_back(r_b[(size_t)u2 * k + s2]); x.und_e.push_back(r_e[(size_t)u2 * k + s2]);
                if (r_e[(size_t)u2 * k + s2] > r_b[(size_t)u2 * k + s2]) sz += (int64_t)(r_e[(size_t)u2 * k + s2] - r_b[(size_t)u2 * k + s2]);
            }
            if (sz > x.big_min) { x.maxn = std::max<u32>(x.maxn, (u32)std::min<int64_t>(sz, 0xFFFFFFFFll)); bigtot[j] += (unsigned long long)sz; }
        }
    }
    for (int j = 0; j < J; j++) {
        RvBatchJob &x = *jobs[(size_t)j];
        x.steps = x.nchild - (u32)x.und_id.size();
        x.too_big = x.no_big ? x.maxn > (u32)BN : ((int64_t)x.maxn > x.big_root || (int64_t)bigtot[(size_t)j] > x.big_total);
        const bool nothing = x.und_id.size() == 1 && x.nchild == 1;
        if (x.na && !x.too_big && !nothing) {
            hipLaunchKernelGGL(k_cmj_lower, dim3((unsigned)ceil_div((int64_t)x.na * k * 64, TB)), dim3(TB), 0, q, x.dT, x.d_anl, x.d_anp, x.na, k);
            RV_LAUNCH_CHECK();
        }
    }
    RV_HIP(hipEventRecord(g->ev_done, q));
    for (RvBatchJob *x : jobs) x->ok = true;
    g->joint_runs++; g->joint_jobs += J;
    if (ws.opt.cascade_log)
        fprintf(stderr, "cascade (batch): %d jobs of %d samples in one loop: %u matches, %u witnesses, %u levels, %u sub-indices, %u undecided; %.2f ms from the last arrival to the hand-back\n",
                J, k, M, NW, hc[C_LEVELS], NCH, U, (std::chrono::duration<double>(std::chrono::steady_clock::now() - t_begin).count()) * 1e3);
    return 0;
}

int rv_cascade_multi_run(rv_index *h, RvCascadeBufs &cb, int minl_in, RvCascadeMultiOut *out) {
    out->done = false; out->levels = 0; out->cands = out->witnesses = out->children = out->undecided = out->rebuilt_ranks = 0; out->steps = 0; out->maxdepth = 0;
    out->why = nullptr; out->big = out->big_ranks = 0; out->an_l.clear(); out->an_pos.clear(); out->meta.clear(); out->node_first.clear(); out->nodes.clear(); out->d_sa = out->d_lcp = out->d_bwt = nullptr;
    Workspace &ws = h->ws;
    hipStream_t q = ws.stream;
    const int64_t n = h->n;
    const int k = h->nsamples;
    const u32 minl = (u32)std::max(minl_in, 1);
    struct BatchTicket { rv_index *h; bool settled = false; ~BatchTicket() { if (h->batch && !settled && !h->batch_settled) { h->batch_settled = true; rv_batch_group_leave(h->batch); } } } ticket{h};
    const bool verbose = (ws.opt.cascade_log != 0);
#define GIVE_UP(msg) do { out->why = msg; if (verbose) fprintf(stderr, "cascade (%d samples): gave up: %s\n", k, msg); return 0; } while (0)
    if (k < 2 || k > RV_CASM_K) GIVE_UP("sample count outside the cascade's range");
    if ((int)h->nodes.size() != k || (int)h->nsep.size() != k - 1) GIVE_UP("not one sequence per sample");
    if (n >= ((int64_t)1 << 32) - 2) GIVE_UP("index above 2^32 positions");
#ifdef RV_SA64
    if ((u64)h->maxlcp >= (1ull << 24) || n >= ((int64_t)1 << 40)) GIVE_UP("bid word too narrow");
#endif
    std::vector<sa_t> rb((size_t)k), re((size_t)k);
    {
        std::vector<RvIntv> nd(h->nodes.begin(), h->nodes.end());
        std::sort(nd.begin(), nd.end(), [](const RvIntv &x, const RvIntv &y) { return x.begin < y.begin; });
        for (int s = 0; s < k; s++) {
            if (nd[(size_t)s].end <= nd[(size_t)s].begin) GIVE_UP("an empty sample");
            const int64_t lo = s ? h->nsep[(size_t)s - 1] : -1, hi = s < k - 1 ? h->nsep[(size_t)s] : n;
            if (nd[(size_t)s].begin <= lo || nd[(size_t)s].end > hi) GIVE_UP("not one sequence per sample");
            rb[(size_t)s] = (sa_t)nd[(size_t)s].begin; re[(size_t)s] = (sa_t)nd[(size_t)s].end;
        }
    }
    const sa_t *SA = h->dSA.as<sa_t>(); const lcp_t *LCP = h->dLCP.as<lcp_t>(); const uint8_t *BWT = h->dBWT.as<uint8_t>();
    const sa_t *nsep = h->dNsep.as<sa_t>();

    const u32 mcap = (u32)std::min<int64_t>(std::max<int64_t>(1 << 16, n / (int64_t)k / 4), 0x7fffffff);
    const u32 wcap = (u32)std::min<int64_t>(std::max<int64_t>(1 << 16, n / 16), 0x7fffffff);
    const int64_t ccap64 = 2 * n / ((int64_t)minl * k) + 16;
// ... 318 lines not shown
```

reveal_amd/csrc/rv_common.h:

```cpp
#pragma once
#include <mutex>
#include <thread>
#include <vector>
#include <utility>
#include <hip/hip_runtime.h>
#include <stdint.h>
#include <string.h>
#include <stddef.h>
#include <vector>
#include <string>

#ifdef RV_SA64
typedef int64_t  sa_t;
typedef uint32_t lcp_t;
#else
typedef int32_t  sa_t;
typedef int32_t  lcp_t;
#endif

typedef unsigned long long u64;
typedef unsigned int       u32;

void rv_set_error(const char *fmt, ...);

// ... 275 lines not shown
    int prof_begin(int k, double bytes) { return prof_begin_fn ? prof_begin_fn(prof_ctx, stream, k, bytes) : -1; }
    void prof_end(int id) { if (prof_end_fn && id >= 0) prof_end_fn(prof_ctx, stream, id); }
    bool sa_in_use = false;
    size_t trim_sa() {
        size_t got = 0;
        for (auto &b : sa) { got += b.cap; b.release(); }
        return got;
    }
    void release() {
        hpin.release();
        if (ev_rb) { (void)hipEventDestroy(ev_rb); ev_rb = nullptr; }
        for (auto &b : scan_tmp) b.release();
        rs_hist.release(); rs_digits.release();
        for (auto &b : misc) b.release();
        for (auto &b : sa) b.release();
    }
};

std::mutex &rv_trim_mutex();
struct SaScratchInUse {
    Workspace &w; bool was;
    SaScratchInUse(Workspace &x) : w(x) { std::lock_guard<std::mutex> g(rv_trim_mutex()); was = w.sa_in_use; w.sa_in_use = true; }
    ~SaScratchInUse() { std::lock_guard<std::mutex> g(rv_trim_mutex()); w.sa_in_use = was; }
};

int rv_exclusive_sum_u32(Workspace &ws, const u32 *in, u32 *out, int64_t n);
int rv_exclusive_sum_u64(Workspace &ws, const u64 *in, u64 *out, int64_t n);
int rv_inclusive_max_u32(Workspace &ws, const u32 *in, u32 *out, int64_t n);
int rv_inclusive_max_u64(Workspace &ws, const u64 *in, u64 *out, int64_t n);

int rv_radix_passes(const Workspace &ws, int nbits);
template <class V>
int rv_radix_sort_pairs(Workspace &ws, u64 *k0, V *v0, u64 *k1, V *v1, int64_t n,
                        int bit_lo, int bit_hi, int *result_in_1);

int rv_read_back(Workspace &ws, void *dst, const void *dsrc, size_t bytes);

int rv_h2d_copy(Workspace &ws, const void *pinned_src, void *dst, size_t bytes);

struct RvSaStats {
    int    sigma, bits, k0;
    int    rounds;
    int64_t sorted_elems;
    int    radix_passes;
    int    diag_table;
    int64_t far_pairs;
    int64_t lcp_list;
};
int rv_build_sa(Workspace &ws, const uint8_t *T, int64_t n, sa_t *SA, RvSaStats *st,
                lcp_t *LCP = nullptr, uint8_t *BWT = nullptr, sa_t side_sep = 0, u32 *d_maxlcp = nullptr, bool *fused_done = nullptr,
                const int64_t *seps = nullptr, int nseps = 0);
int rv_build_inverse(Workspace &ws, const sa_t *SA, sa_t *SAi, int64_t n);
int rv_build_inverse_checked(Workspace &ws, const sa_t *SA, sa_t *SAi, int64_t n);
int rv_build_lcp(Workspace &ws, const uint8_t *T, const sa_t *SA, bool by_rank, lcp_t *LCP, int64_t n, u32 *d_maxlcp, uint8_t *BWT, sa_t side_sep);
int rv_build_bwt(Workspace &ws, const uint8_t *T, const sa_t *SA, int64_t n, uint8_t *BWT, sa_t side_sep);
```

reveal_amd/csrc/rv_construct.hip:

```cpp
#include "rv_common.h"
#include <string.h>
#include <stdlib.h>
#include <algorithm>
#include <limits>

#ifdef RV_SA64
typedef u64 sav_t;
#else
typedef u32 sav_t;
#endif

namespace {

constexpr int TB = 256;

__device__ inline u64 swar_eq(u64 v, uint8_t c) {
    const u64 t = v ^ (0x0101010101010101ull * c);
    return ~(((t & 0x7f7f7f7f7f7f7f7full) + 0x7f7f7f7f7f7f7f7full) | t) & 0x8080808080808080ull;
}
__device__ inline u64 swar_acgt(u64 v) { return swar_eq(v, 'A') | swar_eq(v, 'C') | swar_eq(v, 'G') | swar_eq(v, 'T'); }
__device__ inline u32 swar_code2(u64 v) {
    u64 y = ((v >> 1) ^ (v >> 2)) & 0x0303030303030303ull;
    y = (y | (y >> 6)) & 0x000f000f000f000full;
    y = (y | (y >> 12)) & 0x000000ff000000ffull;
// ... 7 lines not shown
    __syncthreads();
    u32 cA = 0, cC = 0, cG = 0, cT = 0, cS = 0;
    const int64_t stride = (int64_t)gridDim.x * TB * 16;
    for (int64_t base = ((int64_t)blockIdx.x * TB + threadIdx.x) * 16; base < n; base += stride) {
        if (base + 16 <= n) {
            const uint4 v = *reinterpret_cast<const uint4 *>(T + base);
            const u64 w[2] = {(u64)v.x | ((u64)v.y << 32), (u64)v.z | ((u64)v.w << 32)};
            u64 sep[2];
#pragma unroll
            for (int k = 0; k < 2; k++) {
                const u64 eA = swar_eq(w[k], 'A'), eC = swar_eq(w[k], 'C'), eG = swar_eq(w[k], 'G'), eT = swar_eq(w[k], 'T'), eS = swar_eq(w[k], '$');
                cA += (u32)__popcll(eA); cC += (u32)__popcll(eC); cG += (u32)__popcll(eG); cT += (u32)__popcll(eT); cS += (u32)__popcll(eS);
                sep[k] = eS;
                u64 other = ~(eA | eC | eG | eT | eS) & 0x8080808080808080ull;
                while (other) {
                    const int b = __builtin_ctzll(other) >> 3;
                    atomicAdd(&hh[(w[k] >> (8 * b)) & 255u], 1u);
                    other &= other - 1;
                }
            }
            if (sep[0] | sep[1]) for (int64_t i = base; i < base + 16; i++) if (T[i] == '$' && i + 1 < n && T[i + 1] == '$') atomicAdd(&hist[256], 1u);
        } else {
            for (int64_t i = base; i < n; i++) { atomicAdd(&hh[T[i]], 1u); if (T[i] == '$' && i + 1 < n && T[i + 1] == '$') atomicAdd(&hist[256], 1u); }
        }
    }
    if (cA) atomicAdd(&hh[(uint8_t)'A'], cA);
    if (cC) atomicAdd(&hh[(uint8_t)'C'], cC);
    if (cG) atomicAdd(&hh[(uint8_t)'G'], cG);
    if (cT) atomicAdd(&hh[(uint8_t)'T'], cT);
    if (cS) atomicAdd(&hh[(uint8_t)'$'], cS);
    __syncthreads();
    const u32 tot = hh[threadIdx.x];
    if (tot) atomicAdd(&hist[threadIdx.x], tot);
}

constexpr int KEY_TILE = 1024;

struct DiagBits { const u64 *stop, *exc, *lt; int64_t D; int tab; };
struct DiagSamples { int ns; int64_t sep[15], Ds[16]; };
__device__ inline int64_t diag_partner(const DiagSamples &ds, int64_t y) {
    int s = 0;
    for (int q = 0; q < ds.ns - 1; q++) s += ds.sep[q] < y ? 1 : 0;
    return s == 0 ? y + ds.Ds[1] : (s < 16 ? y - ds.Ds[s] : -1);
}
__global__ __launch_bounds__(TB) void k_diag_bits(const uint8_t *__restrict__ T, int64_t n, DiagSamples ds, u64 *__restrict__ stop, u64 *__restrict__ exc,
                                                  u64 *__restrict__ lt, int64_t nwords) {
    const int64_t w = (int64_t)blockIdx.x * TB + threadIdx.x;
    if (w >= nwords) return;
    const int64_t y0 = w * 64;
    u64 ws = 0, we = 0, wl = 0;
    const int64_t p0 = diag_partner(ds, y0), p63 = y0 + 63 < n ? diag_partner(ds, y0 + 63) : -1;
    if (y0 + 64 <= n && p0 >= 0 && p63 == p0 + 63 && p0 + 64 <= n) {
        u64 a[8], b[8];
        __builtin_memcpy(a, T + y0, 64);
        __builtin_memcpy(b, T + p0, 64);
#pragma unroll
        for (int k = 0; k < 8; k++)
#pragma unroll
            for (int j = 0; j < 8; j++) {
                const u32 ca = (u32)(a[k] >> (8 * j)) & 0xffu, cb = (u32)(b[k] >> (8 * j)) & 0xffu;
                const bool ea = !((ca == 'A') | (ca == 'C') | (ca == 'G') | (ca == 'T')), eb = !((cb == 'A') | (cb == 'C') | (cb == 'G') | (cb == 'T'));
                const int bit = 8 * k + j;
                we |= (u64)(ea | eb) << bit; ws |= (u64)((ca != cb) | ea | eb) << bit; wl |= (u64)(ca < cb) << bit;
            }
    } else {
        for (int bit = 0; bit < 64; bit++) {
// ... 144 lines not shown
        ws |= (u64)ms << (sub * DT_TILE); we |= (u64)me << (sub * DT_TILE); wl |= (u64)ml << (sub * DT_TILE);
    }
    stop[w] = ws; exc[w] = we; lt[w] = wl;
}
constexpr sav_t TW_FLAG = (sav_t)1 << (sizeof(sav_t) * 8 - 1);
__device__ inline u64 tw_window_clear(u64 prev, u64 lo, u64 hi, int K) {
    u64 a = lo, b = hi;
    int m = 1;
    while (2 * m <= K) { a |= (a >> m) | (b << (64 - m)); b |= b >> m; m *= 2; }
    if (m < K) { const int d = K - m; a |= (a >> d) | (b << (64 - d)); }
    return ~(a | (lo << 1) | (prev >> 63));
}
__device__ inline u64 tw_range(int64_t w, int64_t a, int64_t b) {
    const int64_t lo = a - 64 * w, hi = b - 64 * w;
    if (hi <= 0 || lo >= 64) return 0ull;
    const u64 from = lo <= 0 ? ~0ull : (~0ull << lo), to = hi >= 64 ? ~0ull : ((1ull << hi) - 1ull);
    return from & to;
}
__device__ inline u64 tw_mask(u64 prev, u64 lo, u64 hi, int64_t w, int K, int64_t D, int64_t n, int tab) {
    const int64_t e = 2 * D - 1 < n ? 2 * D - 1 : n;
    return tw_window_clear(prev, lo, hi, K) & (tab ? (tw_range(w, 0, D - 1) | tw_range(w, D, n)) : (tw_range(w, 1, D - 1) | tw_range(w, D + 1, e)));
}
__global__ __launch_bounds__(TB) void k_tw_count(const u64 *__restrict__ stop, int64_t nwords, int K, int64_t D, int64_t n, u32 *__restrict__ tilecnt, int64_t ntiles, int tab) {
    const int64_t w = (int64_t)blockIdx.x * TB + threadIdx.x;
    u32 c = 0;
    if (w < nwords) {
        const u64 prev = w > 0 ? stop[w - 1] : ~0ull, lo = stop[w], hi = w + 1 < nwords ? stop[w + 1] : ~0ull;
        c = (u32)__popcll(tw_range(w, D, n) & ~tw_mask(prev, lo, hi, w, K, D, n, tab));
    }
#pragma unroll
    for (int d = 8; d >= 1; d >>= 1) c += __shfl_down(c, d, 16);
    const int64_t tile = w >> 4;
    if ((threadIdx.x & 15) == 0 && tile < ntiles) tilecnt[tile] = c;
}
struct KeyLayout { int at_shift, at_bits, nd_shift, nd_bits; u64 sortmask; };
struct KeyPack { int g, fb, nf, gl, fbl, bits; u32 rad, fmask, lmask, lscale , fdiv ;
                 u32 lastmul , dmul[4]; };
constexpr int KP_MAXG = 5;
constexpr u32 KP_MAXFIELD = 4096;
__device__ inline u32 key_common_digits(u64 x, u64 y, const KeyPack &kp) {
    const u64 d = x ^ y;
    if (d == 0ull) return (u32)((kp.nf - 1) * kp.g + kp.gl);
    const int top = 63 - __builtin_clzll(d);
    const bool last = top < kp.fbl;
    const u32 f = last ? (u32)(kp.nf - 1) : ((u32)(kp.bits - 1 - top) * kp.fdiv) >> 16;
    const int sh = last ? 0 : kp.bits - (int)(f + 1u) * kp.fb;
    const u32 fm = last ? kp.lmask : kp.fmask, sc = last ? kp.lscale : 1u;
    const u32 a = __umul24((u32)(x >> sh) & fm, sc), b = __umul24((u32)(y >> sh) & fm, sc);
    u32 c = f * (u32)kp.g;
#pragma unroll
    for (int i = 1; i < KP_MAXG; i++)
        if (i < kp.g) c += ((a * kp.dmul[i - 1]) >> 20) == ((b * kp.dmul[i - 1]) >> 20) ? 1u : 0u;
    return c;
}
constexpr int ND_WORDS = 40;
constexpr int IK_AHEAD = 96;
constexpr int IK_WORDS = (KEY_TILE + IK_AHEAD) / 4;
constexpr int IK_FPOS = KEY_TILE + 64;
__device__ inline u32 ik_first_stop(const u32 *s_sc, int k, int K, u32 at_none) {
    const int w = k >> 5, sh = k & 31;
    if (K <= 32) {
        const u32 win = __funnelshift_r(s_sc[w], s_sc[w + 1], (u32)sh) & (K >= 32 ? ~0u : (1u << K) - 1u);
        return win ? (u32)__builtin_ctz(win) : at_none;
    }
    u64 win = (((u64)s_sc[w + 1] << 32) | s_sc[w]) >> sh;
    if (sh) win |= (u64)s_sc[w + 2] << (64 - sh);
// ... 16 lines not shown
#pragma unroll
            for (int r = 0; r < N; r++) lo[r] |= v[r] << sh;
            if (sh + kp.fb > 32) {
#pragma unroll
                for (int r = 0; r < N; r++) hi[r] |= v[r] >> (32 - sh);
            }
        }
    }
#pragma unroll
    for (int r = 0; r < N; r++) lo[r] |= ((u32)s_tf[p + r] * kp.lastmul) >> 20;
}
struct IkFetch { u32 raw0, raw1, pb; u64 ds, de, dl; };
__device__ inline u32 ik_text_word(const uint8_t *__restrict__ T, int64_t n, int64_t i, bool whole) {
    if (whole) return *reinterpret_cast<const u32 *>(T + i);
    u32 raw = 0;
    for (int r = 0; r < 4; r++) if (i + r < n) raw |= (u32)T[i + r] << (8 * r);
    return raw;
}
__device__ inline void ik_fetch(IkFetch &f, const uint8_t *__restrict__ T, int64_t n, const DiagBits &dg, bool hint, int64_t tile, bool aligned) {
    const int64_t base = tile * KEY_TILE;
    const bool whole = aligned && base + KEY_TILE + IK_AHEAD <= n;
    f.raw0 = ik_text_word(T, n, base + 4 * (int64_t)threadIdx.x, whole);
    f.raw1 = (int)threadIdx.x < IK_WORDS - TB ? ik_text_word(T, n, base + 4 * (int64_t)(TB + threadIdx.x), whole) : 0u;
    f.pb = (threadIdx.x == 0 && base > 0) ? (u32)T[base - 1] : (u32)'$';
    f.ds = ~0ull; f.de = ~0ull; f.dl = 0ull;
    if (hint && (int)threadIdx.x <= ND_WORDS) {
        const int64_t w = base / 64 - 1 + threadIdx.x, nwords = (n + 63) / 64;
        if (w >= 0 && w < nwords) { f.ds = dg.stop[w]; if (threadIdx.x) { f.de = dg.exc[w]; f.dl = dg.lt[w]; } }
    }
}
template <int G>
__global__ __launch_bounds__(TB) void k_init_keys(const uint8_t *__restrict__ T, int64_t n, const uint8_t *__restrict__ lut, int K, KeyPack kp,
                                                  u64 *__restrict__ keys, sav_t *__restrict__ vals, int pay, u32 stop0, u32 stop1,
                                                  KeyLayout ly, DiagBits dg, const u32 *__restrict__ tw_off , int64_t ntiles) {
    __shared__ u32 code32[IK_WORDS + 2];
    __shared__ u32 s_sc[IK_WORDS / 8 + 3];
    __shared__ uint8_t slut[256], sstop[256];
    __shared__ __align__(8) uint16_t s_tf[IK_FPOS];
    __shared__ u64 s_stop0[ND_WORDS + 1], s_exc[ND_WORDS], s_lt[ND_WORDS];
    __shared__ u64 s_tw[KEY_TILE / 64], s_keep[KEY_TILE / 64];
    __shared__ u32 s_kpre[KEY_TILE / 64 + 1];
    __shared__ uint16_t s_list[KEY_TILE];
    __shared__ u32 s_nm[64];
    __shared__ u32 s_raw32[KEY_TILE / 4 + 1];
    u64 *const s_stop = s_stop0 + 1;
    uint8_t *const s_raw = reinterpret_cast<uint8_t *>(s_raw32);
    const bool hint = ly.nd_bits > 0;
    const bool aligned = (reinterpret_cast<uintptr_t>(T) & 3u) == 0;
    auto tile_of = [&](int64_t x) { return x; };
    IkFetch fx;
    int64_t x = blockIdx.x;
    if (x < ntiles) ik_fetch(fx, T, n, dg, hint, tile_of(x), aligned);
    {
        const u32 c = lut[threadIdx.x];
        slut[threadIdx.x] = (uint8_t)c;
        sstop[threadIdx.x] = ((c == stop0) | (c == stop1) | (c == 0u)) ? 1 : 0;
        if (threadIdx.x < 2) code32[IK_WORDS + threadIdx.x] = 0u;
        if (threadIdx.x < 3) s_sc[IK_WORDS / 8 + threadIdx.x] = ~0u;
    }
    __syncthreads();
    const u32 at_none = (1u << ly.at_bits) - 1u;
    const int nd_none = hint ? (int)((1u << ly.nd_bits) - 1u) : 0;
    for (; x < ntiles; x += gridDim.x) {
    const int64_t tile = tile_of(x);
    const int64_t base = tile * KEY_TILE;
#pragma unroll
    for (int turn = 0; turn < 2; turn++) {
// ... 61 lines not shown
    __syncthreads();
    if (tw_off && base >= dg.D) {
        {
            const int t = (int)threadIdx.x, xw = t >> 4, b = (t & 15) * 4;
            const u64 kw = s_keep[xw];
            u32 nib = (u32)(kw >> b) & 15u;
            if (nib) {
                u32 at = s_kpre[xw] + (u32)__popcll(kw & ((1ull << b) - 1ull));
                while (nib) { s_list[at++] = (uint16_t)(4 * t + __builtin_ctz(nib)); nib &= nib - 1u; }
            }
        }
        __syncthreads();
        const u32 total = s_kpre[KEY_TILE / 64];
        const int64_t obase = dg.D + (int64_t)tw_off[tile];
        for (u32 j = threadIdx.x; j < total; j += TB) {
            const int k = (int)s_list[j];
            const int64_t i = base + k;
            u32 lo[1], hi[1];
            ik_fields<G, 1>(s_tf, k, kp, lo, hi);
            u64 key = ((u64)hi[0] << 32) | lo[0];
            if (pay) key |= ((u64)s_raw[k + 3] << 56) | ((u64)ik_first_stop(s_sc, k, K, at_none) << ly.at_shift);
            if (hint) {
                const int wi = k >> 6, sft = k & 63;
                const u64 A = s_stop[wi] >> sft;
                const u32 nx = s_nm[wi + 1];
                const bool has = A != 0ull;
                const int d = has ? __builtin_ctzll(A) : (int)(nx >> 2) - k;
                const int at = (sft + d) & 63;
                const u32 f = has ? ((u32)((s_lt[wi] >> at) & 1ull) << 1) | (u32)((s_exc[wi] >> at) & 1ull) : nx & 3u;
                const bool known = (d < nd_none) & !(f & 1u);
                key |= (u64)(known ? (u32)d | ((f >> 1) << ly.nd_bits) : (u32)nd_none) << ly.nd_shift;
            }
            keys[obase + j] = key; vals[obase + j] = (sav_t)i;
        }
    } else {
    constexpr int PER = KEY_TILE / TB;
    static_assert(PER == 4, "four bytes in front of four positions");
    const int k0 = (int)threadIdx.x * PER;
    const int64_t i0 = base + k0;
    u64 okey[PER];
    {
        u32 lo[PER], hi[PER];
        ik_fields<G, PER>(s_tf, k0, kp, lo, hi);
#pragma unroll
        for (int r = 0; r < PER; r++) okey[r] = ((u64)hi[r] << 32) | lo[r];
    }
    if (pay) {
        const u32 prevb = (u32)s_raw[k0 + 3] | (s_raw32[threadIdx.x + 1] << 8);
        const bool clear = K <= 29 && (__funnelshift_r(s_sc[k0 >> 5], s_sc[(k0 >> 5) + 1], (u32)(k0 & 31)) & ((1u << (K + 3)) - 1u)) == 0u;
#pragma unroll
        for (int r = 0; r < PER; r++)
            okey[r] |= ((u64)((prevb >> (8 * r)) & 0xffu) << 56) | ((u64)(clear ? at_none : ik_first_stop(s_sc, k0 + r, K, at_none)) << ly.at_shift);
    }
    if (hint) {
        const int wi = k0 >> 6, sft = k0 & 63;
        const u64 A = s_stop[wi] >> sft, E = s_exc[wi] >> sft, Lt = s_lt[wi] >> sft;
        const u32 nx = s_nm[wi + 1];
        const u64 Ah = A >> 3;
        const bool hh = Ah != 0ull;
        const int dh = hh ? 3 + __builtin_ctzll(Ah) : (int)(nx >> 2) - k0;
        const u32 fh = hh ? ((u32)((Lt >> (dh & 63)) & 1ull) << 1) | (u32)((E >> (dh & 63)) & 1ull) : nx & 3u;
        const u32 a3 = (u32)A & 7u, e3 = (u32)E & 7u, l3 = (u32)Lt & 7u;
#pragma unroll
        for (int r = 0; r < PER; r++) {
            const u32 t = a3 >> r;
            const int m = t ? r + __builtin_ctz(t) : dh;
            const u32 f = t ? (((l3 >> m) & 1u) << 1) | ((e3 >> m) & 1u) : fh;
            const int nd = m - r;
            const bool known = (nd < nd_none) & !(f & 1u);
            okey[r] |= (u64)(known ? (u32)nd | ((f >> 1) << ly.nd_bits) : (u32)nd_none) << ly.nd_shift;
        }
    }
    if (!tw_off || i0 + PER <= dg.D) {
        const u32 twn = tw_off ? (u32)(s_tw[k0 >> 6] >> (k0 & 63)) & 15u : 0u;
        sav_t oval[PER];
#pragma unroll
        for (int r = 0; r < PER; r++) oval[r] = (sav_t)(i0 + r) | (((twn >> r) & 1u) ? TW_FLAG : (sav_t)0);
        if (i0 + PER <= n) {
            ulonglong2 *kd2 = reinterpret_cast<ulonglong2 *>(keys + i0);
            kd2[0] = make_ulonglong2(okey[0], okey[1]); kd2[1] = make_ulonglong2(okey[2], okey[3]);
            if constexpr (sizeof(sav_t) == 4) *reinterpret_cast<uint4 *>(vals + i0) = make_uint4((u32)oval[0], (u32)oval[1], (u32)oval[2], (u32)oval[3]);
            else {
                ulonglong2 *vd2 = reinterpret_cast<ulonglong2 *>(vals + i0);
                vd2[0] = make_ulonglong2((u64)oval[0], (u64)oval[1]); vd2[1] = make_ulonglong2((u64)oval[2], (u64)oval[3]);
            }
        } else {
#pragma unroll
            for (int r = 0; r < PER; r++) if (i0 + r < n) { keys[i0 + r] = okey[r]; vals[i0 + r] = oval[r]; }
        }
    } else {
#pragma unroll
        for (int r = 0; r < PER; r++) {
            const int k = k0 + r;
            const int64_t i = base + k;
            if (i >= n) continue;
            const int xw = k >> 6, b = k & 63;
            const bool twin = (s_tw[xw] >> b) & 1ull;
            if (i < dg.D) { keys[i] = okey[r]; vals[i] = (sav_t)i | (twin ? TW_FLAG : (sav_t)0); }
            else if (!twin) {
                const int64_t o = dg.D + (int64_t)tw_off[tile] + s_kpre[xw] + (u32)__popcll(s_keep[xw] & ((b == 0) ? 0ull : (~0ull >> (64 - b))));
                keys[o] = okey[r]; vals[o] = (sav_t)i;
            }
        }
    }
    }
    __syncthreads();
    }
}

constexpr int HINT_K = 16;
struct KeyDigits { int K; u32 stop0, stop1; KeyPack kp; KeyLayout ly; int64_t D; int ns; int64_t sep[HINT_K - 1], Ds[HINT_K];
                   const int32_t *dtab; };
__device__ inline u32 key_first_stop(u64 key, const KeyDigits &kd) {
    const u32 none = (1u << kd.ly.at_bits) - 1u;
    const u32 at = (u32)(key >> kd.ly.at_shift) & none;
    return at == none ? 0xFFFFFFFFu : at;
}
__device__ inline bool key_hint(u64 key, const KeyDigits &kd, u32 *nd, bool *lt) {
    const u32 none = (1u << kd.ly.nd_bits) - 1u;
    const u32 v = (u32)(key >> kd.ly.nd_shift) & none;
    *nd = v; *lt = (key >> (kd.ly.nd_shift + kd.ly.nd_bits)) & 1ull;
    return kd.ly.nd_bits > 0 && v != none;
}
__device__ inline int hint_sample(const KeyDigits &kd, int64_t p) {
    int s = 0;
    for (int q = 0; q < kd.ns - 1; q++) s += kd.sep[q] < p ? 1 : 0;
    return s;
}
__device__ inline bool hint_cmp(const KeyDigits &kd, int64_t u, u64 key_u, int64_t v, u64 key_v, int *c, u32 *l, bool linked = false) {
    if (kd.ly.nd_bits <= 0) return false;
    const int su = hint_sample(kd, u), sv = hint_sample(kd, v);
    if (su >= HINT_K || sv >= HINT_K) return false;
    if (kd.dtab) {
        if (su == sv) return false;
// ... 347 lines not shown
}
__global__ __launch_bounds__(TB) void k_isa_list(const sa_t *__restrict__ SA, const u32 *__restrict__ P, const u32 *__restrict__ G, int64_t m, u32 *__restrict__ ISA) {
    const int64_t q = (int64_t)blockIdx.x * TB + threadIdx.x;
    if (q < m) ISA[SA[P[q]]] = G[q];
}
__global__ __launch_bounds__(TB) void k_isa_from_groups(const sa_t *__restrict__ SA, const u32 *__restrict__ grp, int64_t n, u32 *__restrict__ ISA) {
    const int64_t j = (int64_t)blockIdx.x * TB + threadIdx.x;
    if (j < n) ISA[SA[j]] = grp[j];
}

constexpr int CP_ITEMS = 8;
constexpr int CP_TILE = TB * CP_ITEMS;

__device__ inline bool unsorted_at(const uint8_t *head, int64_t j, int64_t n) {
    return !(head[j] && (j + 1 == n || head[j + 1]));
}

__global__ __launch_bounds__(TB) void k_cp_count(const uint8_t *__restrict__ head, int64_t n, u32 *__restrict__ tilecnt) {
    __shared__ u32 wsum[TB / 64];
    static_assert(CP_ITEMS == 8, "eight head bytes per load");
    const int64_t j0 = (int64_t)blockIdx.x * CP_TILE + (int64_t)threadIdx.x * CP_ITEMS;
    u32 c = 0;
    if (j0 + CP_ITEMS < n) {
        const u64 hb = *reinterpret_cast<const u64 *>(head + j0);
        const u64 nx = (hb >> 8) | ((u64)head[j0 + CP_ITEMS] << 56);
#pragma unroll
        for (int k = 0; k < CP_ITEMS; k++) c += !(((hb >> (8 * k)) & 0xFFu) && ((nx >> (8 * k)) & 0xFFu));
    } else {
        for (int64_t j = j0; j < j0 + CP_ITEMS && j < n; j++) c += unsorted_at(head, j, n);
    }
    for (int d = 32; d >= 1; d >>= 1) c += __shfl_down(c, d, 64);
    if ((threadIdx.x & 63) == 0) wsum[threadIdx.x >> 6] = c;
    __syncthreads();
    if (threadIdx.x == 0) tilecnt[blockIdx.x] = wsum[0] + wsum[1] + wsum[2] + wsum[3];
}

__global__ __launch_bounds__(TB) void k_cp_emit(const uint8_t *__restrict__ head, int64_t n, const u32 *__restrict__ tileoff,
                                                const u32 *__restrict__ pos_in, const sav_t *__restrict__ suf_in, const u32 *__restrict__ grp_in,
                                                u32 *__restrict__ P, sav_t *__restrict__ S, u32 *__restrict__ G,
                                                const uint8_t *__restrict__ cls_in = nullptr, uint8_t *__restrict__ cls_out = nullptr, int cls_is = 0) {
    __shared__ u32 wbase[TB / 64];
    const int lane = threadIdx.x & 63, w = threadIdx.x >> 6;
    const int64_t base = (int64_t)blockIdx.x * CP_TILE;
    u32 run = tileoff[blockIdx.x];
    const u64 lt = (lane == 0) ? 0ull : (~0ull >> (64 - lane));
#pragma unroll 1
    for (int r = 0; r < CP_ITEMS; r++) {
        const int64_t j = base + (int64_t)r * TB + threadIdx.x;
        const bool f = (j < n) && unsorted_at(head, j, n);
        const u64 bal = __ballot(f);
        if (lane == 0) wbase[w] = (u32)__popcll(bal);
        __syncthreads();
        u32 before = 0, tot = 0;
#pragma unroll
        for (int k = 0; k < TB / 64; k++) { const u32 c = wbase[k]; if (k < w) before += c; tot += c; }
        if (f) {
            const u32 q = run + before + (u32)__popcll(bal & lt);
            P[q] = pos_in ? pos_in[j] : (u32)j;
            S[q] = suf_in[j];
            G[q] = grp_in[j];
            if (cls_out) cls_out[q] = cls_in ? (cls_is ? (cls_in[j] == (uint8_t)cls_is) : cls_in[j]) : (uint8_t)0;
        }
        run += tot;
        __syncthreads();
    }
}

__global__ __launch_bounds__(TB) void k_cp_count_g(const uint8_t *__restrict__ head, int64_t n, u32 *__restrict__ tilecnt, u32 *__restrict__ tilelast) {
    __shared__ u32 wsum[TB / 64], wlast[TB / 64];
    static_assert(CP_ITEMS == 8, "eight head bytes per load");
    const int64_t j0 = (int64_t)blockIdx.x * CP_TILE + (int64_t)threadIdx.x * CP_ITEMS;
    u32 c = 0, last = 0;
    if (j0 + CP_ITEMS < n) {
        const u64 hb = *reinterpret_cast<const u64 *>(head + j0);
        const u64 nx = (hb >> 8) | ((u64)head[j0 + CP_ITEMS] << 56);
#pragma unroll
        for (int k = 0; k < CP_ITEMS; k++) c += !(((hb >> (8 * k)) & 0xFFu) && ((nx >> (8 * k)) & 0xFFu));
        if (hb) last = (u32)(j0 + ((63 - __builtin_clzll(hb)) >> 3) + 1);
    } else {
        for (int64_t j = j0; j < j0 + CP_ITEMS && j < n; j++) { c += unsorted_at(head, j, n); last = head[j] ? (u32)(j + 1) : last; }
    }
    for (int d = 32; d >= 1; d >>= 1) { c += __shfl_down(c, d, 64); const u32 o = __shfl_down(last, d, 64); last = o > last ? o : last; }
    if ((threadIdx.x & 63) == 0) { wsum[threadIdx.x >> 6] = c; wlast[threadIdx.x >> 6] = last; }
    __syncthreads();
    if (threadIdx.x == 0) {
        tilecnt[blockIdx.x] = wsum[0] + wsum[1] + wsum[2] + wsum[3];
        u32 l = wlast[0];
        for (int k = 1; k < TB / 64; k++) l = wlast[k] > l ? wlast[k] : l;
        tilelast[blockIdx.x] = l;
    }
}
__global__ __launch_bounds__(TB) void k_cp_emit_g(const uint8_t *__restrict__ head, int64_t n, const u32 *__restrict__ tileoff, const u32 *__restrict__ tilelast,
                                                  const sav_t *__restrict__ suf_in, u32 *__restrict__ P, sav_t *__restrict__ S, u32 *__restrict__ G) {
    __shared__ u32 wcnt[TB / 64], wlast[TB / 64];
    static_assert(CP_ITEMS == 8, "eight head bytes per load");
    const int lane = threadIdx.x & 63, w = threadIdx.x >> 6;
    const int64_t j0 = (int64_t)blockIdx.x * CP_TILE + (int64_t)threadIdx.x * CP_ITEMS;
    u32 hm = 0, um = 0;
    if (j0 + CP_ITEMS < n) {
        const u64 hb = *reinterpret_cast<const u64 *>(head + j0);
        const u64 nx = (hb >> 8) | ((u64)head[j0 + CP_ITEMS] << 56);
#pragma unroll
        for (int k = 0; k < CP_ITEMS; k++) {
            const bool h = (hb >> (8 * k)) & 0xFFu, hn = (nx >> (8 * k)) & 0xFFu;
            hm |= (u32)h << k; um |= (u32)!(h && hn) << k;
        }
    } else {
        for (int k = 0; k < CP_ITEMS; k++) { const int64_t j = j0 + k; if (j < n) { hm |= (u32)(head[j] != 0) << k; um |= (u32)unsorted_at(head, j, n) << k; } }
    }
    const u32 c = (u32)__popc(um);
    const u32 mylast = hm ? (u32)(j0 + (31 - __clz(hm)) + 1) : 0u;
    u32 inc = c, lastinc = mylast;
#pragma unroll
    for (int d = 1; d < 64; d <<= 1) {
        const u32 t = __shfl_up(inc, d, 64), l = __shfl_up(lastinc, d, 64);
        if (lane >= d) { inc += t; lastinc = l > lastinc ? l : lastinc; }
    }
    if (lane == 63) { wcnt[w] = inc; wlast[w] = lastinc; }
    __syncthreads();
// ... 760 lines not shown
        const u64 stop = stop_mask(wa, wb);
        const u64 bal = __ballot(stop != 0);
        if (bal) {
            const int f = (int)__builtin_ctzll(bal);
            const u32 lo = (u32)__shfl((int)(u32)stop, f, 64), hi = (u32)__shfl((int)(u32)(stop >> 32), f, 64);
            const u64 st = ((u64)hi << 32) | lo;
            h += 8u * (u32)f + (u32)(__builtin_ctzll(st) >> 3);
            done = true;
            break;
        }
        h += 512;
    }
    if (lane == 0) {
        if (!done) { atomicOr(overflow, 1u); return; }
        LCP[k] = (lcp_t)h;
        if (h > __atomic_load_n(maxlcp, __ATOMIC_RELAXED)) atomicMax(maxlcp, h);
    }
}

__global__ __launch_bounds__(TB) void k_flag_count(const uint8_t *__restrict__ flag, int64_t n, u32 *__restrict__ tilecnt) {
    __shared__ u32 wsum[TB / 64];
    const int64_t j0 = (int64_t)blockIdx.x * CP_TILE + (int64_t)threadIdx.x * CP_ITEMS;
    u32 c = 0;
    if (j0 + CP_ITEMS <= n) {
        const u64 f = *reinterpret_cast<const u64 *>(flag + j0);
#pragma unroll
        for (int k = 0; k < CP_ITEMS; k++) c += ((f >> (8 * k)) & 0xFFu) == 1u;
    } else {
        for (int64_t j = j0; j < n && j < j0 + CP_ITEMS; j++) c += flag[j] == 1;
    }
    for (int d = 32; d >= 1; d >>= 1) c += __shfl_down(c, d, 64);
    if ((threadIdx.x & 63) == 0) wsum[threadIdx.x >> 6] = c;
    __syncthreads();
    if (threadIdx.x == 0) tilecnt[blockIdx.x] = wsum[0] + wsum[1] + wsum[2] + wsum[3];
}
__global__ __launch_bounds__(TB) void k_flag_emit(const uint8_t *__restrict__ flag, int64_t n, const u32 *__restrict__ tileoff,
                                                  const u32 *__restrict__ P, const sav_t *__restrict__ S, const u32 *__restrict__ G, int64_t nn, int64_t h,
                                                  const u32 *__restrict__ ISA, u32 *__restrict__ Pb, sav_t *__restrict__ Sb, u32 *__restrict__ Qb, u64 *__restrict__ kk) {
    __shared__ u32 wbase[TB / 64];
    const int lane = threadIdx.x & 63, w = threadIdx.x >> 6;
    const int64_t base = (int64_t)blockIdx.x * CP_TILE;
    u32 run = tileoff[blockIdx.x];
    const u64 lt = (lane == 0) ? 0ull : (~0ull >> (64 - lane));
#pragma unroll 1
    for (int r = 0; r < CP_ITEMS; r++) {
        const int64_t j = base + (int64_t)r * TB + threadIdx.x;
        const bool f = (j < n) && flag[j] == 1;
        const u64 bal = __ballot(f);
        if (lane == 0) wbase[w] = (u32)__popcll(bal);
        __syncthreads();
        u32 before = 0, tot = 0;
#pragma unroll
        for (int k = 0; k < TB / 64; k++) { const u32 c = wbase[k]; if (k < w) before += c; tot += c; }
        if (f) {
            const u32 qb = run + before + (u32)__popcll(bal & lt);
            const sav_t s = S[j];
            Pb[qb] = P[j]; Sb[qb] = s; Qb[qb] = (u32)j;
            kk[qb] = ((u64)G[j] << 32) | key2_of(s, h, nn, ISA);
        }
        run += tot;
        __syncthreads();
    }
}
__global__ __launch_bounds__(TB) void k_big_writeback(const u64 *__restrict__ kk, const u32 *__restrict__ Pb, const u32 *__restrict__ Qb, const sav_t *__restrict__ Sb,
                                                      int64_t mb, sav_t *__restrict__ S, uint8_t *__restrict__ headq, sa_t *__restrict__ SA) {
    const int64_t qb = (int64_t)blockIdx.x * TB + threadIdx.x;
    if (qb >= mb) return;
// ... 258 lines not shown
int rv_build_sa(Workspace &ws, const uint8_t *T, int64_t n, sa_t *SA, RvSaStats *st,
                lcp_t *LCP, uint8_t *BWT, sa_t side_sep, u32 *d_maxlcp, bool *fused_done, const int64_t *seps, int nseps) {
    SaScratchInUse in_use(ws);
    RvSaStats s;
    memset(&s, 0, sizeof s);
    if (fused_done) *fused_done = false;
    if (n <= 0) { if (st) *st = s; return 0; }
    if (n >= ((int64_t)1 << 32) - 2) { rv_set_error("SA build: n >= 2^32-2 not supported yet"); return -1; }
    hipStream_t q = ws.stream;
    if (n <= TINY_N / 2 && LCP && BWT && d_maxlcp && !ws.opt.no_tiny_sa) {
        RV_TRY(ws.sa[0].reserve((size_t)TINY_N * 2 + 64));
        RV_HIP(hipMemsetAsync(d_maxlcp, 0, sizeof(u32), q));
        const unsigned nb = (unsigned)ceil_div(n, TB);
        hipLaunchKernelGGL(k_sa_tiny_rank, dim3(nb), dim3(TB), 0, q, T, (int)n, ws.sa[0].as<uint16_t>());
        RV_LAUNCH_CHECK();
        hipLaunchKernelGGL(k_sa_tiny_emit, dim3(nb), dim3(TB), 0, q, T, (int)n, (const uint16_t *)ws.sa[0].as<uint16_t>(), SA, LCP, BWT, side_sep, d_maxlcp);
        RV_LAUNCH_CHECK();
        s.rounds = 0; s.sorted_elems = 0;
        if (st) *st = s;
        if (fused_done) *fused_done = true;
        return 0;
    }

    DBuf &d_hist = ws.sa[16], &d_lut = ws.sa[17];
    RV_TRY(d_hist.reserve(264 * sizeof(u32)));
    RV_TRY(d_lut.reserve(256));
    RV_HIP(hipMemsetAsync(d_hist.p, 0, 264 * sizeof(u32), q));
    {
        int64_t blocks = ceil_div(n, (int64_t)TB * 16);
        if (blocks > 2048) blocks = 2048;
        hipLaunchKernelGGL(k_hist256, dim3((unsigned)blocks), dim3(TB), 0, q, T, n, d_hist.as<u32>());
        RV_LAUNCH_CHECK();
    }
    u32 hist[257];
    RV_TRY(rv_read_back(ws, hist, d_hist.p, sizeof hist));
    uint8_t lut[256];
    int sigma = 0;
    for (int c = 0; c < 256; c++) lut[c] = hist[c] ? (uint8_t)(++sigma) : (uint8_t)0;
    u32 radix = (u32)sigma + 1;
    if (sigma >= 255) radix = 256;
    if (sigma >= 255) for (int c = 0; c < 256; c++) lut[c] = (uint8_t)c;
    const bool short_alphabet = sigma >= 2 && sigma < 255 && T != nullptr && hist[(uint8_t)'$'] > 0 && lut[(uint8_t)'$'] == 1 && hist[256] == 0 && !ws.opt.no_short_alphabet;
    bool ends_with_sep = false;
    if (short_alphabet) { uint8_t last = 0; RV_TRY(rv_read_back(ws, &last, T + (n - 1), 1)); ends_with_sep = last == (uint8_t)'$'; }
    if (short_alphabet && ends_with_sep) {
        for (int c = 0; c < 256; c++) lut[c] = hist[c] ? (uint8_t)(lut[c] - 1) : (uint8_t)0;
        radix = (u32)sigma;
    }
    int K = 1;
    int bits = 0;
    KeyPack kp;
    {
        const double base = sigma > 2 ? (double)(sigma - 1) : 2.0;
        const double want = (double)n * ((seps && nseps > 1) ? 16.0 : 1.0);
        int best_g = 0, best_K = 0, best_bits = 0;
        u64 rg = 1;
        for (int g = 1; g <= KP_MAXG; g++) {
            rg *= radix;
            if (rg > KP_MAXFIELD && g > 1) break;
            const int fb = bitlen(rg - 1);
            auto bits_of = [&](int k) { u64 rl = 1; for (int e = 0; e < k % g; e++) rl *= radix; return (k / g) * fb + (k % g ? bitlen(rl - 1) : 0); };
            bool exact = true;
            for (int i = 1; i < g && exact; i++) {
                u64 d = 1; for (int e = 0; e < g - i; e++) d *= radix;
                const u32 m = (u32)(((1ull << 20) + d - 1) / d);
                for (u64 f = 0; f < rg && exact; f++) exact = ((f * m) >> 20) == f / d && f * m < (1ull << 32);
            }
            if (!exact) continue;
            int k = 1; double cap = base;
            while (cap < want && bits_of(k + 1) <= 62) { cap *= base; k++; }
            const int passes = rv_radix_passes(ws, bits_of(k));
            while (bits_of(k + 1) <= 62 && rv_radix_passes(ws, bits_of(k + 1)) == passes) k++;
            const int b = bits_of(k);
            if (k > best_K || (k == best_K && b < best_bits)) { best_g = g; best_K = k; best_bits = b; }
        }
        K = best_K; bits = best_bits;
        u64 rgb = 1; for (int e = 0; e < best_g; e++) rgb *= radix;
// ... 40 lines not shown
    SA_TRY(bhead.reserve((size_t)n + 16));
    auto need_seed_grp = [&](int64_t cnt) -> int {
        RV_TRY(bseed.reserve((size_t)std::max<int64_t>(cnt, 1) * (sizeof(sav_t) > 4 ? sizeof(sav_t) : 4)));
        return bgrp.reserve((size_t)std::max<int64_t>(cnt, 1) * 4);
    };
    SA_TRY(bisa.reserve((size_t)n * 4));
    const unsigned nblk = (unsigned)ceil_div(n, TB);

    DiagBits dg; dg.stop = dg.exc = dg.lt = nullptr; dg.D = kd.D; dg.tab = 0;
    kd.dtab = nullptr;
    const int64_t nw = (n + 63) / 64;
    DiagSamples dsm; dsm.ns = kd.ns;
    for (int q2 = 0; q2 < HINT_K - 1; q2++) dsm.sep[q2] = kd.sep[q2];
    for (int q2 = 0; q2 < HINT_K; q2++) dsm.Ds[q2] = kd.Ds[q2];
    if (kd.ly.nd_bits > 0) {
        DBuf &bds = ws.sa[20], &bde = ws.sa[21], &bdl = ws.sa[22];
        SA_TRY(bds.reserve((size_t)nw * 8)); SA_TRY(bde.reserve((size_t)nw * 8)); SA_TRY(bdl.reserve((size_t)nw * 8));
        hipLaunchKernelGGL(k_diag_bits, dim3((unsigned)ceil_div(nw, TB)), dim3(TB), 0, q, T, n, dsm, bds.as<u64>(), bde.as<u64>(), bdl.as<u64>(), nw);
        SA_HIP(hipGetLastError());
        dg.stop = bds.as<u64>(); dg.exc = bde.as<u64>(); dg.lt = bdl.as<u64>();
    }
    const bool collapse = fused && kd.ly.nd_bits > 0 && kd.ns == 2 && K < 64 && kd.D > 1 && n > kd.D + 1 && !ws.opt.no_heads_fusion && !ws.opt.no_twin_collapse
                          && (sizeof(sav_t) > 4 || n < ((int64_t)1 << 31));
    int64_t nsort = n;
    const u32 *tw_off = nullptr;
    if (collapse) {
        const int64_t ntiles = ceil_div(n, KEY_TILE);
        DBuf &btw = ws.sa[23];
        SA_TRY(btw.reserve((size_t)(std::max<int64_t>(ntiles, ceil_div(n, TB)) + 1) * 4 + 64));
        u32 *tc = btw.as<u32>();
        auto count_kept = [&](int tab, u32 *kept_out) -> int {
            hipLaunchKernelGGL(k_tw_count, dim3((unsigned)ceil_div(nw, TB)), dim3(TB), 0, q, (const u64 *)dg.stop, nw, K, kd.D, n, tc, ntiles, tab);
            RV_LAUNCH_CHECK();
            RV_HIP(hipMemsetAsync(tc + ntiles, 0, 4, q));
            RV_TRY(rv_exclusive_sum_u32(ws, tc, tc, ntiles + 1));
            return rv_read_back(ws, kept_out, tc + ntiles, 4);
        };
        u32 kept = 0;
        SA_TRY(count_kept(0, &kept));
        const int dt_mode = (int)ws.opt.diag_table;
        const int64_t n2 = n - kd.D;
        if (dt_mode != 0 && n >= 4096 && (dt_mode == 1 || (int64_t)kept * 10 > n2 * 3)) {
            const int64_t mseeds = nw * SEED_SLOTS;
            DBuf &bdt = ws.sa[25];
            const int64_t ndt = (n >> DT_SHIFT) + 1;
            SA_TRY(bdt.reserve((size_t)ndt * 8 + 64));
            int32_t *raw = bdt.as<int32_t>(), *tab = raw + ndt;
            const int did = ws.prof_begin(11 , (double)n + (double)mseeds * 12.0);
            hipLaunchKernelGGL(k_seed_sample, dim3((unsigned)ceil_div(nw, TB)), dim3(TB), 0, q, T, n, bk0.as<u64>(), bv0.as<sav_t>(), nw);
            SA_HIP(hipGetLastError());
            int sin1 = 0;
            SA_TRY(rv_radix_sort_pairs<sav_t>(ws, bk0.as<u64>(), bv0.as<sav_t>(), bk1.as<u64>(), bv1.as<sav_t>(), mseeds, 0, 40, &sin1));
            SA_HIP(hipMemsetAsync(raw, 0x7f, (size_t)ndt * 4, q));
            hipLaunchKernelGGL(k_seed_pairs, dim3((unsigned)ceil_div(mseeds, TB)), dim3(TB), 0, q, (const u64 *)(sin1 ? bk1.as<u64>() : bk0.as<u64>()),
                               (const sav_t *)(sin1 ? bv1.as<sav_t>() : bv0.as<sav_t>()), mseeds, kd.D, kd.D, raw);
            SA_HIP(hipGetLastError());
            hipLaunchKernelGGL(k_dtab_fill, dim3((unsigned)ceil_div(ndt, TB)), dim3(TB), 0, q, T, n, kd.D, kd.D, (const int32_t *)raw, tab, ndt);
            SA_HIP(hipGetLastError());
            DiagTab dt; dt.dtab = tab; dt.S2 = kd.D; dt.D = kd.D;
            hipLaunchKernelGGL(k_diag_bits_tab, dim3((unsigned)ceil_div(nw, TB)), dim3(TB), 0, q, T, n, dt, ws.sa[20].as<u64>(), ws.sa[21].as<u64>(), ws.sa[22].as<u64>(), nw);
            SA_HIP(hipGetLastError());
            ws.prof_end(did);
            u32 kept_tab = 0;
            SA_TRY(count_kept(1, &kept_tab));
            if (dt_mode == 1 || (int64_t)kept_tab * 5 < (int64_t)kept * 4) { kept = kept_tab; kd.dtab = tab; dg.tab = 1; }
            else {
                hipLaunchKernelGGL(k_diag_bits, dim3((unsigned)ceil_div(nw, TB)), dim3(TB), 0, q, T, n, dsm, ws.sa[20].as<u64>(), ws.sa[21].as<u64>(), ws.sa[22].as<u64>(), nw);
                SA_HIP(hipGetLastError());
                SA_TRY(count_kept(0, &kept));
            }
        }
        nsort = kd.D + (int64_t)kept;
        tw_off = tc;
        s.diag_table = dg.tab;
    }
    {
        const int64_t iktiles = ceil_div(n, KEY_TILE);
        const dim3 ig((unsigned)std::min<int64_t>(iktiles, 256 * 8));
#define RV_IK_(G) hipLaunchKernelGGL(k_init_keys<G>, ig, dim3(TB), 0, q, T, n, d_lut.as<uint8_t>(), K, kp, bk0.as<u64>(), bv0.as<sav_t>(), fused ? 1 : 0, \
                                     kd.stop0, kd.stop1, kd.ly, dg, tw_off, iktiles)
        const int ikid = ws.prof_begin(12 , (double)n + (double)nsort * (8.0 + sizeof(sav_t) + 1.0));
        switch (kp.g) { case 1: RV_IK_(1); break; case 2: RV_IK_(2); break; case 3: RV_IK_(3); break; case 4: RV_IK_(4); break; default: RV_IK_(5); break; }
        ws.prof_end(ikid);
#undef RV_IK_
    }
    SA_HIP(hipGetLastError());
    int in1 = 0;
    SA_TRY(rv_radix_sort_pairs<sav_t>(ws, bk0.as<u64>(), bv0.as<sav_t>(), bk1.as<u64>(), bv1.as<sav_t>(), nsort, 0, bits, &in1));
    s.radix_passes += rv_radix_passes(ws, bits); s.sorted_elems += nsort;
    u64 *ks = in1 ? bk1.as<u64>() : bk0.as<u64>();
    sav_t *vs = in1 ? bv1.as<sav_t>() : bv0.as<sav_t>();
    u64 *kt = in1 ? bk0.as<u64>() : bk1.as<u64>();
    sav_t *vt = in1 ? bv0.as<sav_t>() : bv1.as<sav_t>();

    uint8_t *head = bhead.as<uint8_t>();
    if (!collapse) SA_TRY(need_seed_grp(n));
    u32 *seed = bseed.as<u32>(), *grp = bgrp.as<u32>(), *ISA = bisa.as<u32>();
    const u64 *keys_by_rank = ks;
    const sav_t *vals_by_rank = vs;
    if (collapse) {
        const int64_t nb = ceil_div(nsort, TC_TILE);
        u32 *bc = ws.sa[23].as<u32>();
        hipLaunchKernelGGL(k_tw_flags, dim3((unsigned)nb), dim3(TB), 0, q, (const sav_t *)vs, nsort, bc);
        SA_HIP(hipGetLastError());
        SA_TRY(rv_exclusive_sum_u32(ws, bc, bc, nb));
        sav_t *vexp = reinterpret_cast<sav_t *>(bisa.p);
        if (sizeof(sav_t) > 4) { SA_TRY(ws.sa[24].reserve((size_t)n * sizeof(sav_t))); vexp = ws.sa[24].as<sav_t>(); }
        const int pbid = ws.prof_begin(13 , (double)nsort * 2.0 * (8.0 + sizeof(sav_t)) + (double)n * (1.0 + sizeof(sa_t) + sizeof(lcp_t) + 1.0));
        hipLaunchKernelGGL(k_heads_publish_tc, dim3((unsigned)nb), dim3(TB), 0, q, (const u64 *)ks, (const sav_t *)vs, nsort, (const u32 *)bc, head, LCP, SA, BWT,
                           side_sep, kd, d_maxlcp, ws.opt.no_pub_twins ? 0 : 1, kt, vexp);
        ws.prof_end(pbid);
        SA_HIP(hipGetLastError());
        keys_by_rank = kt; vals_by_rank = vexp;
    } else if (fused && kd.ly.nd_bits > 0 && !ws.opt.no_heads_fusion) {
        hipLaunchKernelGGL(k_heads_publish, dim3((unsigned)ceil_div(n, (int64_t)HP_ITEMS * TB)), dim3(TB), 0, q, (const u64 *)ks, (const sav_t *)vs, n, head, seed, LCP, SA, BWT, side_sep, kd, d_maxlcp,
                           ws.opt.no_pub_twins ? 0 : 1);
        SA_HIP(hipGetLastError());
        SA_TRY(rv_inclusive_max_u32(ws, seed, grp, n));
    } else {
        hipLaunchKernelGGL(k_heads, dim3(nblk), dim3(TB), 0, q, (const u64 *)ks, n, head, seed, fused ? LCP : (lcp_t *)nullptr, kd, fused ? d_maxlcp : (u32 *)nullptr);
        SA_HIP(hipGetLastError());
        SA_TRY(rv_inclusive_max_u32(ws, seed, grp, n));
        {
            KeyDigits kp = kd;
            if (ws.opt.no_pub_twins) kp.ly.nd_bits = 0;
            hipLaunchKernelGGL(k_publish0, dim3(nblk), dim3(TB), 0, q, (const sav_t *)vs, n, SA, (const u64 *)ks, fused ? BWT : (uint8_t *)nullptr, side_sep,
                               kp, fused ? LCP : (lcp_t *)nullptr, head, d_maxlcp, grp);
        }
        SA_HIP(hipGetLastError());
    }
    bool isa_built = false;
    const sav_t *cur_S = nullptr; const u32 *cur_G = nullptr; int64_t cur_m = 0;
    auto need_isa = [&]() -> int {
        if (isa_built) return 0;
        hipLaunchKernelGGL(k_isa_identity, dim3(nblk), dim3(TB), 0, q, (const sa_t *)SA, n, ISA);
        RV_LAUNCH_CHECK();
        if (cur_m > 0) {
            hipLaunchKernelGGL(k_round_isa, dim3((unsigned)ceil_div(cur_m, TB)), dim3(TB), 0, q, cur_S, cur_G, cur_m, ISA);
            RV_LAUNCH_CHECK();
        }
        isa_built = true;
        return 0;
    };

    int64_t ntile = ceil_div(n, CP_TILE);
    SA_TRY(btile.reserve(std::max((size_t)(ntile + 1) * 8 + 64, (size_t)RT_REGIONS * 4)));
    u32 *tile = btile.as<u32>();
    auto count_unsorted = [&](const uint8_t *hd, int64_t len, int64_t *m_out) -> int {
        const int64_t nt = ceil_div(len, CP_TILE);
        hipLaunchKernelGGL(k_cp_count, dim3((unsigned)nt), dim3(TB), 0, q, hd, len, tile);
        RV_LAUNCH_CHECK();
        RV_HIP(hipMemsetAsync(tile + nt, 0, 4, q));
        RV_TRY(rv_exclusive_sum_u32(ws, tile, tile, nt + 1));
        u32 tot = 0;
        RV_TRY(rv_read_back(ws, &tot, tile + nt, 4));
        *m_out = tot;
        return 0;
    };
    auto emit_unsorted = [&](const uint8_t *hd, int64_t len, const u32 *pos_in, const sav_t *suf_in, const u32 *grp_in, u32 *P, sav_t *S, u32 *G,
                             const uint8_t *cls_in = nullptr, uint8_t *cls_out = nullptr, int cls_is = 0) -> int {
        const int64_t nt = ceil_div(len, CP_TILE);
        hipLaunchKernelGGL(k_cp_emit, dim3((unsigned)nt), dim3(TB), 0, q, hd, len, (const u32 *)tile, pos_in, suf_in, grp_in, P, S, G, cls_in, cls_out, cls_is);
        RV_LAUNCH_CHECK();
        return 0;
    };
    int64_t m = 0;
    if (collapse) {
        u32 *tlast = tile + (ntile + 1);
        hipLaunchKernelGGL(k_cp_count_g, dim3((unsigned)ntile), dim3(TB), 0, q, (const uint8_t *)head, n, tile, tlast);
        SA_HIP(hipGetLastError());
        SA_HIP(hipMemsetAsync(tile + ntile, 0, 4, q));
        SA_TRY(rv_exclusive_sum_u32(ws, tile, tile, ntile + 1));
        SA_TRY(rv_inclusive_max_u32(ws, tlast, tlast, ntile));
        u32 tot = 0;
        SA_TRY(rv_read_back(ws, &tot, tile + ntile, 4));
        m = tot;
        SA_TRY(bP0.reserve((size_t)std::max<int64_t>(m, 1) * 4)); SA_TRY(bG0.reserve((size_t)std::max<int64_t>(m, 1) * 4));
        SA_TRY(need_seed_grp(m));
        seed = bseed.as<u32>(); grp = bgrp.as<u32>();
        if (m > 0) {
            hipLaunchKernelGGL(k_cp_emit_g, dim3((unsigned)ntile), dim3(TB), 0, q, (const uint8_t *)head, n, (const u32 *)tile, (const u32 *)tlast, vals_by_rank,
                               bP0.as<u32>(), vt, bG0.as<u32>());
            SA_HIP(hipGetLastError());
        }
    } else {
        SA_TRY(count_unsorted(head, n, &m));
        SA_TRY(bP0.reserve((size_t)std::max<int64_t>(m, 1) * 4)); SA_TRY(bG0.reserve((size_t)std::max<int64_t>(m, 1) * 4));
        if (m > 0) SA_TRY(emit_unsorted(head, n, nullptr, vals_by_rank, grp, bP0.as<u32>(), vt, bG0.as<u32>()));
    }
    const int64_t m_list0 = m;
    u32 *P = bP0.as<u32>(), *G = bG0.as<u32>(), *Pn = nullptr, *Gn = nullptr;
    sav_t *S = vt;
    sav_t *Sfree = vs;
    u64 *kA = ks, *kB = kt;
    if (m > 0) { SA_TRY(bbig.reserve((size_t)m + 16)); SA_TRY(bQb.reserve((size_t)m * 4)); SA_TRY(bPb.reserve((size_t)m * 4)); }

    const int lowbits = bitlen((u64)n), highbits = bitlen((u64)(n > 1 ? n - 1 : 1));
    int64_t h = K;
    const bool can_far = fused && kd.ly.nd_bits > 0 && kd.ns == 2 && dg.stop != nullptr && !ws.opt.no_far_twins;
    const bool can_list = fused && !ws.opt.no_lcp_list;
    bool text_round_ran = false, far_ran = false, partial = false;
    DBuf &btodo = ws.sa[26];
    int64_t ntodo = 0;
    auto todo_add = [&](const u32 *ranks, int64_t cnt) -> int {
// ... 69 lines not shown
            if (tmode == 3 && fused) {
                u32 *work = bQb.as<u32>(), *work_count = tile;
                const u32 reg_cap = (u32)(ceil_div((int64_t)mb, RT_REGIONS) * (TB / 2));
                SA_HIP(hipMemsetAsync(work_count, 0, RT_REGIONS * 4, q));
                hipLaunchKernelGGL((k_round_text3<4>), dim3(mb), dim3(TB), 0, q, T, S, (const u32 *)G, (const u32 *)P, m, n, head, bigflag, SA, Sfree, fo, work, work_count, reg_cap);
                SA_HIP(hipGetLastError());
                u32 cnt[RT_REGIONS];
                SA_TRY(rv_read_back(ws, cnt, work_count, sizeof cnt));
                u32 mx = 0;
                for (int r = 0; r < RT_REGIONS; r++) mx = std::max(mx, cnt[r]);
                if (mx) {
                    const u32 bpr = (u32)ceil_div((int64_t)mx, TB);
                    hipLaunchKernelGGL((k_round_text3b<4>), dim3(bpr * RT_REGIONS), dim3(TB), 0, q, T, S, (const u32 *)G, m, n, head, SA, fo, (const u32 *)work,
                                       (const u32 *)work_count, reg_cap, bpr);
                }
            }
            else if (tmode == 0) RT_LAUNCH(0); else if (tmode == 2) RT_LAUNCH(2); else RT_LAUNCH(1);
#undef RT_LAUNCH
            SA_HIP(hipGetLastError());
            ws.prof_end(tid);
            hipLaunchKernelGGL(k_medium_back, dim3((unsigned)ceil_div(m, (int64_t)TB * 8)), dim3(TB), 0, q, (const uint8_t *)bigflag, (const sav_t *)Sfree, S, m);
        }
        else {
            if (!list_in_todo) { SA_TRY(leave_fused(P, m)); list_in_todo = true; }
            SA_TRY(need_isa());
            const uint8_t *slow = (cls && 2 * h <= TEXT_LIM) ? cls : nullptr;
            hipLaunchKernelGGL(k_round_small, dim3(mb), dim3(TB), 0, q, S, (const u32 *)G, (const u32 *)P, m, n, h, (const u32 *)ISA, head, bigflag, SA, slow);
        }
        SA_HIP(hipGetLastError());
        if (!far_round) {
            const int64_t nt = ceil_div(m, CP_TILE);
            hipLaunchKernelGGL(k_flag_count, dim3((unsigned)nt), dim3(TB), 0, q, (const uint8_t *)bigflag, m, tile);
            SA_HIP(hipGetLastError());
            SA_HIP(hipMemsetAsync(tile + nt, 0, 4, q));
            SA_TRY(rv_exclusive_sum_u32(ws, tile, tile, nt + 1));
            u32 mbig = 0;
            SA_TRY(rv_read_back(ws, &mbig, tile + nt, 4));
            if (mbig > 0) {
                text_big = text_round;
                SA_TRY(need_isa());
                u32 *Pb = bPb.as<u32>(), *Qb = bQb.as<u32>();
                hipLaunchKernelGGL(k_flag_emit, dim3((unsigned)nt), dim3(TB), 0, q, (const uint8_t *)bigflag, m, (const u32 *)tile, (const u32 *)P, (const sav_t *)S,
                                   (const u32 *)G, n, h, (const u32 *)ISA, Pb, Sfree, Qb, kA);
                SA_HIP(hipGetLastError());
                if (!list_in_todo) SA_TRY(leave_fused(Pb, (int64_t)mbig));
                sav_t *sb0 = Sfree, *sb1 = reinterpret_cast<sav_t *>(bseed.p);
                int f1 = 0, f2 = 0;
                SA_TRY(rv_radix_sort_pairs<sav_t>(ws, kA, sb0, kB, sb1, mbig, 0, lowbits, &f1));
                u64 *k_in = f1 ? kB : kA, *k_out = f1 ? kA : kB;
                sav_t *s_in = f1 ? sb1 : sb0, *s_out = f1 ? sb0 : sb1;
                SA_TRY(rv_radix_sort_pairs<sav_t>(ws, k_in, s_in, k_out, s_out, mbig, 32, 32 + highbits, &f2));
                const u64 *kS = f2 ? k_out : k_in;
                const sav_t *sS = f2 ? s_out : s_in;
                s.radix_passes += rv_radix_passes(ws, lowbits) + rv_radix_passes(ws, highbits); s.sorted_elems += mbig;
                hipLaunchKernelGGL(k_big_writeback, dim3((unsigned)ceil_div(mbig, TB)), dim3(TB), 0, q, kS, (const u32 *)Pb, (const u32 *)Qb, sS, (int64_t)mbig, S, head, SA);
                SA_HIP(hipGetLastError());
            }
        }
        int64_t m2 = 0;
        SA_TRY(count_unsorted(head, m, &m2));
        if (far_round) s.far_pairs = (m - m2) / 2;
        if (m2 == 0) break;
        if (!can_far && !can_list) fused = false;
        hipLaunchKernelGGL(k_seed, dim3(mb), dim3(TB), 0, q, (const uint8_t *)head, (const u32 *)P, m, seed);
        SA_HIP(hipGetLastError());
        SA_TRY(rv_inclusive_max_u32(ws, seed, grp, m));
        if (isa_built) {
// ... 41 lines not shown
```

reveal_amd/csrc/rv_index.h:

```cpp
#pragma once
#include "rv_common.h"
#include "rv_scan.h"
#include "../../include/reveal_amd.h"
#include <utility>

struct RvIntv { int64_t begin, end; };

struct RvProf {
    bool on = false;
    u32 mask = 0xFFFFFFFFu;
    struct Span { hipEvent_t a, b; int k; double bytes; };
    std::vector<Span> spans;
    std::vector<hipEvent_t> pool;
    int64_t launches[RV_K_COUNT] = {0};
    double ms[RV_K_COUNT] = {0};
    double bytes[RV_K_COUNT] = {0};
    hipEvent_t get() {
        if (!pool.empty()) { hipEvent_t e = pool.back(); pool.pop_back(); return e; }
        hipEvent_t e = nullptr;
        (void)hipEventCreate(&e);
        return e;
    }
    int begin(hipStream_t s, int k, double nbytes) {
        if (!on || !((mask >> k) & 1u)) return -1;
// ... 62 lines not shown
            else (void)hipGetLastError();
        }
        if (!q) q = (char *)malloc(grow);
        if (!q) { rv_set_error("out of host memory for %zu bytes of text", grow); return -1; }
        if (n) memcpy(q, p, n);
        if (p) { if (pinned) (void)hipHostFree(p); else free(p); }
        p = q; cap = grow; pinned = pin;
        return 0;
    }
    int resize(size_t m) { if (reserve(m) != 0) return -1; n = m; return 0; }
    void push_back(char c) { if (resize(n + 1) == 0) p[n - 1] = c; }
    char *data() { return p; }
    const char *data() const { return p; }
    size_t size() const { return n; }
    char &operator[](size_t k) { return p[k]; }
    const char &operator[](size_t k) const { return p[k]; }
};

struct rv_index {
    int device = 0;
    Workspace ws;
    RvProf prof;
    HostText T;
    std::vector<int64_t> nsep;
    std::vector<int64_t> nsep_dev;
    std::vector<RvIntv> nodes;
    int nsamples = 0;
    int64_t n = 0, nT = 0;
    int rc = 0;
    bool constructed = false, main_arrays_freed = false;
    bool sai_valid = false;
    DBuf dT, dT0, dSA, dSAi, dLCP, dBWT, dNsep;
    bool text_dirty = true;
    bool text_only = false;
    HBuf hscan;
    HBuf hupload;
    hipEvent_t ev_picks = nullptr;
    size_t scan_guess = 4096;
    DBuf ps[7];
    u32 maxlcp = 0;
    RvSaStats sa_stats{};
    std::vector<u32> m_l; std::vector<int64_t> m_a, m_b;
    std::vector<u32> mm_l; std::vector<int32_t> mm_n; std::vector<int64_t> mm_off, mm_pos; std::vector<uint16_t> mm_so;
    struct Align *al = nullptr;
    struct RvBatchGroup *batch = nullptr;
    bool batch_settled = false;
    struct ResultBufs {
        uint32_t *l = nullptr; int64_t *off = nullptr, *pos = nullptr;
        int64_t l_cap = 0, off_cap = 0, pos_cap = 0;
        bool direct = false;
    } rb;
};

int rv_run_multi_pick(rv_index *h, const sa_t *SA, const lcp_t *LCP, const uint8_t *BWT, int64_t m, int minl, int minn,
                      const int64_t *d_sub_start, const int *d_sub_want, int nsubs, const int *d_tile_sub, std::vector<u32> &pick_l, std::vector<sa_t> &pick_pos,
                      int (*after_pick)(rv_index *) = nullptr, bool *redo = nullptr);
int rv_run_pair_scan(rv_index *h, const sa_t *SA, const lcp_t *LCP, const uint8_t *BWT, int64_t m, int minl, std::vector<RvPairRec> &out,
                     const u32 *d_err, u32 *err_out, const int64_t *d_sub_start, int nsubs,
                     int (*after_pick)(rv_index *), bool use_hook,
                     const int *d_tile_sub = nullptr,
                     const int64_t *d_presel_start = nullptr, int presel_subs = 0, int64_t presel = 0);

int rv_text_only(rv_index *h, u32 maxlcp);

int rv_need_sai(rv_index *h);

void rv_align_free(rv_index *h);
```

reveal_amd/csrc/rv_many.hip:

```cpp
#include "rv_index.h"
#include "rv_leaf.h"
#include <algorithm>
#include <limits.h>
#include <new>
#include <stdexcept>

namespace {

constexpr int MT = 256;
constexpr int CAP_L = RV_LEAF_N;
constexpr int CAP_S = 512;
static_assert(CAP_L <= 2048, "local ranks are packed in 12 bits, positions in 16");

struct ManyDevJob { int64_t abeg, bbeg, off; int32_t la, lb; };

#define MANY_WSYNC() do { __builtin_amdgcn_fence(__ATOMIC_ACQ_REL, "workgroup"); __builtin_amdgcn_wave_barrier(); } while (0)

__device__ inline u32 many_wave_incl_max(u32 v) {
    const int lane = threadIdx.x & 63;
#define MANY_STEP_(CTRL, RM, TAKE) { const u32 o = rv_dpp_u32<CTRL, RM>(v); v = ((TAKE) && o > v) ? o : v; }
    RV_WAVE_SCAN_STEPS(MANY_STEP_)
#undef MANY_STEP_
    return v;
}
// ... 276 lines not shown
    if (nsmall < J) {
        hipLaunchKernelGGL((k_many_build<CAP_L, MT>), dim3((unsigned)(J - nsmall)), dim3(MT), 0, q, djobs + nsmall, (int)(J - nsmall), dT,
                           m->dSA.as<sa_t>(), m->dLCP.as<lcp_t>(), m->dBWT.as<uint8_t>(), d_max, d_err);
        RV_LAUNCH_CHECK();
        m->info[4]++;
    }
    u32 cnt[2] = {0, 0};
    RV_TRY(rv_read_back(h->ws, cnt, d_max, 8));
    if (cnt[1]) { rv_set_error("rv_many_run: the index build refused a job (error bits %u)", cnt[1]); return -1; }
    if (m->keep) {
        std::vector<sa_t> sa((size_t)n); std::vector<lcp_t> lc((size_t)n);
        RV_HIP(hipMemcpy(sa.data(), m->dSA.p, (size_t)n * sizeof(sa_t), hipMemcpyDeviceToHost));
        RV_HIP(hipMemcpy(lc.data(), m->dLCP.p, (size_t)n * sizeof(lcp_t), hipMemcpyDeviceToHost));
        const size_t base = m->keep_sa.size();
        m->keep_sa.resize(base + (size_t)n); m->keep_lcp.resize(base + (size_t)n);
        for (size_t s = 0; s < J; s++) {
            m->jobs[(size_t)ord[s]].arr_off = (int64_t)base + dj[s].off;
            for (int64_t r = 0; r < la[s] + lb[s] + 2; r++) {
                const int64_t p = (int64_t)sa[(size_t)(dj[s].off + r)];
                m->keep_sa[base + (size_t)(dj[s].off + r)] = (sa_t)(p >= bbeg[s] ? p - bbeg[s] + la[s] + 1 : p - abeg[s]);
                m->keep_lcp[base + (size_t)(dj[s].off + r)] = lc[(size_t)(dj[s].off + r)];
            }
        }
    }
    RV_TRY(rv_frontier_import(h, minl, minn, cnt[0], 0, (int)J, meta.data(), node_first.data(), nodes.data(), n, m->dSA.p, m->dLCP.p, m->dBWT.p, 1));
    rv_align_stats st;
    memset(&st, 0, sizeof st);
    RV_TRY(rv_align_builtin_resume(h, &st));
    many_add_stats(total, st);
    const size_t rec0 = m->recs.size();
    RV_TRY(many_collect(m, h, -1, ord, abeg, bbeg));
    m->info[4] += st.levels + (m->recs.size() > rec0 ? 2 : 0);
    std::vector<char> txt((size_t)n);
    RV_HIP(hipMemcpy(txt.data(), h->dT.p, (size_t)n, hipMemcpyDeviceToHost));
    for (size_t s = 0; s < J; s++) {
        ManyJob &jb = m->jobs[(size_t)ord[s]];
        jb.text_off = (int64_t)m->out_text.size();
        jb.shared = true;
        m->out_text.insert(m->out_text.end(), txt.begin() + (ptrdiff_t)abeg[s], txt.begin() + (ptrdiff_t)(abeg[s] + la[s] + 1));
        m->out_text.insert(m->out_text.end(), txt.begin() + (ptrdiff_t)bbeg[s], txt.begin() + (ptrdiff_t)(bbeg[s] + lb[s] + 1));
    }
    m->info[1] += (int64_t)J; m->info[3]++;
    return 0;
}

int many_ordinary(rv_many *m, int job, int minl, int minn, rv_align_stats *total) {
    RV_TRY(many_handle(m, &m->ho));
    rv_index *h = m->ho;
    ManyJob &jb = m->jobs[(size_t)job];
    RV_TRY(rv_reset(h));
    for (int s = 0; s < jb.k; s++) {
        RV_TRY(rv_add_sample(h));
        RV_TRY(rv_add_sequence(h, m->in.data() + m->starts[jb.seq0 + (size_t)s], m->lens[jb.seq0 + (size_t)s], nullptr, nullptr));
    }
    RV_TRY(rv_construct(h, 0, nullptr, nullptr, 0));
    rv_align_stats st;
    memset(&st, 0, sizeof st);
    RV_TRY(rv_align_builtin(h, minl, minn, &st));
    many_add_stats(total, st);
    static const std::vector<int> none; static const std::vector<int64_t> none64;
    RV_TRY(many_collect(m, h, job, none, none64, none64));
    jb.text_off = (int64_t)m->out_text.size();
    jb.shared = false;
    m->out_text.resize(m->out_text.size() + (size_t)jb.ranks);
    if (rv_get_array(h, RV_T, m->out_text.data() + jb.text_off, jb.ranks) != jb.ranks) return -1;
    m->info[2]++;
// ... 164 lines not shown
```

reveal_amd/csrc/rv_prims.hip:

```cpp
#include "rv_common.h"
#include <string.h>

namespace {

constexpr int SCAN_THREADS = 256;
constexpr int SCAN_ITEMS   = 8;
constexpr int SCAN_TILE    = SCAN_THREADS * SCAN_ITEMS;

template <class T> struct OpSum {
    __device__ static T id() { return (T)0; }
    __device__ static T f(T a, T b) { return a + b; }
};
template <class T> struct OpMax {
    __device__ static T id() { return (T)0; }
    __device__ static T f(T a, T b) { return a > b ? a : b; }
};

template <class T> __device__ inline T shfl_up_t(T v, int d) { return __shfl_up(v, d, 64); }
template <> __device__ inline u64 shfl_up_t<u64>(u64 v, int d) {
    u32 lo = __shfl_up((u32)v, d, 64), hi = __shfl_up((u32)(v >> 32), d, 64);
    return ((u64)hi << 32) | lo;
}

template <class T, class Op>
// ... 251 lines not shown
            const u32 d = (u32)(key[r] >> shift) & dmask;
            const u32 li = (u32)dstart[d] + (u32)cnt[w][d] + rnk[r];
            skey[li] = key[r];
            sval[li] = val[r];
        }
    }
    __syncthreads();
    const int64_t tbase = (int64_t)tile * RS_TILE;
    const u32 nvalid = (u32)((n - tbase) < (int64_t)RS_TILE ? (n - tbase) : (int64_t)RS_TILE);
    for (u32 li = threadIdx.x; li < nvalid; li += RS_THREADS) {
        const u64 k = skey[li];
        const u32 d = (u32)(k >> shift) & dmask;
        const size_t dst = (size_t)gbase[d] + (li - (u32)dstart[d]);
        kout[dst] = k;
        vout[dst] = sval[li];
        if (dnext) dnext[dst] = (uint8_t)((u32)(k >> nshift) & nmask);
    }
}

template <class V, int BITS, bool XCD, class CNT>
static void rs_scatter_launch(hipStream_t q, u32 nb, const u64 *ki, const V *vi, u64 *ko, V *vo, int64_t n, int shift, u32 dmask, const u32 *bh,
                              uint8_t *dnext, int nshift, u32 nmask) {
    const u32 grid = XCD ? RS_XCDS * ((nb + RS_XCDS - 1) / RS_XCDS) : nb;
    hipLaunchKernelGGL((k_rs_scatter<V, BITS, XCD, CNT>), dim3(grid), dim3(RS_THREADS), 0, q, ki, vi, ko, vo, n, shift, dmask, bh, nb, dnext, nshift, nmask);
}

}

int rv_radix_passes(const Workspace &ws, int nbits) {
    const int w = ws.opt.rs_bits == 10 ? 10 : 8;
    return nbits <= 0 ? 0 : (nbits + w - 1) / w;
}

template <class V>
int rv_radix_sort_pairs(Workspace &ws, u64 *k0, V *v0, u64 *k1, V *v1, int64_t n, int bit_lo, int bit_hi, int *result_in_1) {
    *result_in_1 = 0;
    if (n <= 1 || bit_hi <= bit_lo) return 0;
    if (n >= ((int64_t)1 << 32)) { rv_set_error("radix sort: n >= 2^32 not supported"); return -1; }
    const int width = ws.opt.rs_bits == 10 ? 10 : 8;
    const bool xcd = ws.opt.rs_xcd != 0, c16 = ws.opt.rs_cnt16 != 0;
    const u32 nb = (u32)ceil_div(n, RS_TILE);
    RV_TRY(ws.rs_hist.reserve(((size_t)1 << width) * nb * sizeof(u32)));
    u32 *bh = ws.rs_hist.as<u32>();
    const bool bytes = width == 8 && !ws.opt.rs_no_digit_bytes && n >= ((int64_t)1 << 20) && bit_hi - bit_lo > width;
    if (bytes) RV_TRY(ws.rs_digits.reserve((size_t)n + 64));
    uint8_t *dig = bytes ? ws.rs_digits.as<uint8_t>() : nullptr;
    bool have_digits = false;
    u64 *ki = k0, *ko = k1;
    V *vi = v0, *vo = v1;
    int flip = 0;
    for (int shift = bit_lo; shift < bit_hi; shift += width) {
        const int wbits = bit_hi - shift < width ? bit_hi - shift : width;
        const u32 dmask = (1u << wbits) - 1u;
        int pid = ws.prof_begin(8 , (have_digits ? 1.0 : 8.0) * (double)n);
        const u32 hgrid = xcd ? RS_XCDS * ((nb + RS_XCDS - 1) / RS_XCDS) : nb;
        if (have_digits) {
            if (xcd) hipLaunchKernelGGL((k_rs_hist_bytes<true>), dim3(hgrid), dim3(RS_THREADS), 0, ws.stream, (const uint8_t *)dig, n, bh, nb);
            else hipLaunchKernelGGL((k_rs_hist_bytes<false>), dim3(hgrid), dim3(RS_THREADS), 0, ws.stream, (const uint8_t *)dig, n, bh, nb);
        } else if (width == 10) { if (xcd) hipLaunchKernelGGL((k_rs_hist<10, true>), dim3(hgrid), dim3(RS_THREADS), 0, ws.stream, (const u64 *)ki, n, shift, dmask, bh, nb);
                           else hipLaunchKernelGGL((k_rs_hist<10, false>), dim3(hgrid), dim3(RS_THREADS), 0, ws.stream, (const u64 *)ki, n, shift, dmask, bh, nb); }
        else             { if (xcd) hipLaunchKernelGGL((k_rs_hist<8, true>), dim3(hgrid), dim3(RS_THREADS), 0, ws.stream, (const u64 *)ki, n, shift, dmask, bh, nb);
                           else hipLaunchKernelGGL((k_rs_hist<8, false>), dim3(hgrid), dim3(RS_THREADS), 0, ws.stream, (const u64 *)ki, n, shift, dmask, bh, nb); }
        RV_LAUNCH_CHECK();
        ws.prof_end(pid);
        RV_TRY(rv_exclusive_sum_u32(ws, bh, bh, ((int64_t)1 << width) * nb));
        const int nshift = shift + width;
        const bool more = nshift < bit_hi;
        const u32 nmask = more ? ((1u << (bit_hi - nshift < width ? bit_hi - nshift : width)) - 1u) : 0u;
        uint8_t *dn = (bytes && more) ? dig : nullptr;
        pid = ws.prof_begin(7 , (2.0 * (8.0 + sizeof(V)) + (dn ? 1.0 : 0.0)) * (double)n);
#define RS_GO(B_, X_, C_) rs_scatter_launch<V, B_, X_, C_>(ws.stream, nb, (const u64 *)ki, (const V *)vi, ko, vo, n, shift, dmask, (const u32 *)bh, dn, nshift, nmask)
        if (width == 10) { if (xcd) { if (c16) RS_GO(10, true, uint16_t); else RS_GO(10, true, u32); } else { if (c16) RS_GO(10, false, uint16_t); else RS_GO(10, false, u32); } }
        else             { if (xcd) { if (c16) RS_GO(8, true, uint16_t); else RS_GO(8, true, u32); } else { if (c16) RS_GO(8, false, uint16_t); else RS_GO(8, false, u32); } }
#undef RS_GO
        RV_LAUNCH_CHECK();
        ws.prof_end(pid);
        have_digits = dn != nullptr;
        u64 *tk = ki; ki = ko; ko = tk;
        V *tv = vi; vi = vo; vo = tv;
        flip ^= 1;
    }
    *result_in_1 = flip;
    return 0;
}

__global__ __launch_bounds__(256) void k_h2d_copy(const uint4 *__restrict__ src, uint4 *__restrict__ dst, size_t n16) {
    for (size_t i = (size_t)blockIdx.x * 256 + threadIdx.x; i < n16; i += (size_t)gridDim.x * 256) dst[i] = src[i];
}
int rv_read_back(Workspace &ws, void *dst, const void *dsrc, size_t bytes) {
    RV_TRY(ws.hpin.reserve(bytes < 4096 ? 4096 : bytes));
    if (!ws.ev_rb) RV_HIP(hipEventCreateWithFlags(&ws.ev_rb, hipEventDisableTiming));
    RV_HIP(hipMemcpyAsync(ws.hpin.p, dsrc, bytes, hipMemcpyDeviceToHost, ws.stream));
    RV_HIP(hipEventRecord(ws.ev_rb, ws.stream));
    const hipError_t e = rv_event_wait(ws.ev_rb);
    if (e != hipSuccess) { rv_set_error("rv_read_back: %s", hipGetErrorString(e)); return -1; }
    memcpy(dst, ws.hpin.p, bytes);
    return 0;
}

int rv_h2d_copy(Workspace &ws, const void *pinned_src, void *dst, size_t bytes) {
    const size_t n16 = (bytes + 15) / 16;
    if (n16 == 0) return 0;
    size_t blocks = (n16 + 255) / 256;
    if (blocks > 512) blocks = 512;
    hipLaunchKernelGGL(k_h2d_copy, dim3((unsigned)blocks), dim3(256), 0, ws.stream, (const uint4 *)pinned_src, (uint4 *)dst, n16);
    RV_LAUNCH_CHECK();
    return 0;
}

template int rv_radix_sort_pairs<u32>(Workspace &, u64 *, u32 *, u64 *, u32 *, int64_t, int, int, int *);
template int rv_radix_sort_pairs<u64>(Workspace &, u64 *, u64 *, u64 *, u64 *, int64_t, int, int, int *);
```

Measured before the change: 22210.

## Defer working-text copy, stream cascade anchors early, emit first radix digits in key init

```diff
diff --git a/reveal_amd/csrc/rv_align.hip b/reveal_amd/csrc/rv_align.hip
--- a/reveal_amd/csrc/rv_align.hip
+++ b/reveal_amd/csrc/rv_align.hip
@@ -189,6 +189,7 @@
     size_t last_leaf_count = 0;
     bool running = false;
     u32 *lf_counters = nullptr; unsigned long long *lf_stats = nullptr; u32 *lf_l = nullptr; int64_t *lf_pos = nullptr; rv_trace *lf_tr = nullptr;
+    size_t early_sent = 0; u32 *early_l = nullptr; int64_t *early_pos = nullptr;
     size_t leaf_na = 0;
     void release() {
         if (leaf_stream) (void)hipStreamSynchronize(leaf_stream);
@@ -597,6 +598,7 @@
     const bool all_classes = a->multi || ns > 4096;
     if (biggest <= a->par_min_cur && !h->ws.opt.no_early_bubble &&
         (a->multi || (!h->ws.opt.bubble_lds_always && (!all_classes || h->ws.opt.early_bubble_many)))) {
+        RV_TRY(rv_ensure_working_text(h));
         RV_TRY(rv_lower_ranges_launch(h->ws, h->dT.as<uint8_t>(), t.mb, t.me, W * ns));
         RV_TRY(bubble_flags(h, m));
         RvBubbleArgs ba;
@@ -1252,6 +1254,7 @@
     }
     h->prof.end(q, id);
     if (!a->early_bubble) {
+        RV_TRY(rv_ensure_working_text(h));
         if (lt.nmatch > 256 && a->mpre.back() / lt.nmatch <= 512) RV_TRY(rv_lower_ranges_launch(h->ws, h->dT.as<uint8_t>(), lt.mbegin, lt.mend, lt.nmatch));
         else RV_TRY(rv_lower_launch(h->ws, h->dT.as<uint8_t>(), lt.mbegin, lt.mend, (const int64_t *)(tb + cm.o_mpre), lt.nmatch, a->mpre.back()));
     }
@@ -1412,7 +1415,7 @@
     RV_TRY(align_begin(h, minl, minn, h->al && h->al->trace_on));
     Align *a = h->al;
     a->full_only = !a->trace_on && a->picker == 0;
-    a->an_l.clear(); a->an_off.assign(1, 0); a->an_pos.clear(); a->trace.clear(); a->leaf_na = 0;
+    a->an_l.clear(); a->an_off.assign(1, 0); a->an_pos.clear(); a->trace.clear(); a->leaf_na = 0; a->early_sent = 0;
     a->seeds_cur.clear(); a->seeds_lead.clear(); a->seeds_trail.clear(); a->picker_calls = a->picker_seeded = 0; a->picker_ns = a->picker_list_ns = a->galign_ns = 0;
     if (a->picker == 1) {
         if ((int)h->nodes.size() != h->nsamples) { rv_set_error("the native picker (rv_set_picker) takes one sequence per sample: %d sequences in %d samples", (int)h->nodes.size(), h->nsamples); return -1; }
@@ -1831,8 +1834,12 @@
             int64_t *pp; u32 *pl;
             if (rb.direct) { pp = rb.pos + np; pl = rb.l + nl; }
             else { RV_TRY(a->hLeafOut.reserve(na * 20 + 64)); pp = a->hLeafOut.as<int64_t>(); pl = (u32 *)(pp + 2 * na); }
-            RV_HIP(hipMemcpyAsync(pp, lf_pos, na * 16, hipMemcpyDeviceToHost, a->leaf_stream));
-            RV_HIP(hipMemcpyAsync(pl, lf_l, na * 4, hipMemcpyDeviceToHost, a->leaf_stream));
+            const size_t sent = (rb.direct && a->early_l == pl && a->early_pos == pp) ? std::min(a->early_sent, na) : 0;
+            if (sent < na) {
+                RV_HIP(hipMemcpyAsync(pp + 2 * sent, lf_pos + 2 * sent, (na - sent) * 16, hipMemcpyDeviceToHost, a->leaf_stream));
+                RV_HIP(hipMemcpyAsync(pl + sent, lf_l + sent, (na - sent) * 4, hipMemcpyDeviceToHost, a->leaf_stream));
+            }
+            RV_TRY(rv_ensure_working_text(h));
             RV_TRY(rv_leaf_lower_launch(h->ws, h->dT.as<uint8_t>(), lf_pos, lf_l, (u32)na));
             if (rb.direct) fill_offsets(rb.off + nl + 1, na, (int64_t)np);
             RV_HIP(hipStreamSynchronize(a->leaf_stream));
@@ -1895,20 +1902,30 @@
     io.anchor_count = a->lf_counters; io.anchor_cap = (u32)a->leaf_anchor_cap; io.anchor_l = a->lf_l; io.anchor_pos = a->lf_pos;
     io.stats = a->lf_stats; io.leaf_err = a->lf_counters + 2;
     io.stage_cap = (u32)h->ws.opt.leaf_acap;
+    RvCascadeHost hx;
+    hx.side = a->leaf_stream;
+    a->early_sent = 0;
+    if (h->rb.l) {
+        const int64_t nl = (int64_t)a->an_l.size(), np = (int64_t)a->an_pos.size();
+        const int64_t room = std::min(std::min(h->rb.l_cap - nl, h->rb.off_cap - nl - 1), (h->rb.pos_cap - np) / 2);
+        if (room > 0) { hx.l = h->rb.l + nl; hx.pos = h->rb.pos + np; hx.cap = (u32)std::min<int64_t>(room, 0xffffffffll); }
+    }
     io.lvSA = &a->lvSA[0]; io.lvLCP = &a->lvLCP[0]; io.lvBWT = &a->lvBWT[0]; io.roots = &a->dLeafRoots[0];
     const int dmode = (int)h->ws.opt.cascade_danger;
-    RV_TRY(rv_cascade_run(h, a->cas, io, a->minl, &a->cas_out, dmode == 2 ? 1 : 0, 0));
+    RV_TRY(rv_cascade_run(h, a->cas, io, a->minl, &a->cas_out, dmode == 2 ? 1 : 0, 0, &hx));
     if (!a->cas_out.done && a->cas_out.undecided > 0 && dmode == 1) {
         RV_HIP(hipMemsetAsync(a->dLeaf.p, 0, 256, h->ws.stream));
-        RV_TRY(rv_cascade_run(h, a->cas, io, a->minl, &a->cas_out, 1, 1));
+        RV_TRY(rv_cascade_run(h, a->cas, io, a->minl, &a->cas_out, 1, 1, &hx));
     }
     if (!a->cas_out.done) {
+        if (hx.l) RV_HIP(hipStreamSynchronize(a->leaf_stream));
         RV_HIP(hipMemsetAsync(a->dLeaf.p, 0, 256, h->ws.stream));
         if (a->cas_out.undecided > 0 && !h->ws.opt.cascade_second_off) return interval_cascade();
         return 0;
     }
     a->st.levels += a->cas_out.levels;
     a->st.scanned_ranks += h->n;
+    a->early_sent = a->cas_out.sent; a->early_l = hx.l; a->early_pos = hx.pos;
     if (!a->cas.lin_rest.empty() && h->nodes.size() > 2) {
         std::vector<RvIntv> rest, gone;
         for (size_t k = 0; k + 1 < a->cas.lin_rest.size(); k += 2) rest.push_back({a->cas.lin_rest[k], a->cas.lin_rest[k + 1]});
@@ -2118,7 +2135,7 @@
             if (h->rc) { rv_set_error("the native picker (rv_set_picker) with construct(rc=1) is not supported"); return -1; }
         }
         a->picker_calls = a->picker_seeded = 0; a->picker_ns = a->picker_list_ns = a->galign_ns = 0;
-        a->an_l.clear(); a->an_off.assign(1, 0); a->an_pos.clear(); a->trace.clear(); a->leaf_na = 0;
+        a->an_l.clear(); a->an_off.assign(1, 0); a->an_pos.clear(); a->trace.clear(); a->leaf_na = 0; a->early_sent = 0;
         RV_TRY(builtin_leaf_setup(h));
     }
     RV_TRY(install_frontier(h, level, nsubs, meta, node_first, nodes, m, sa, lcp, bwt, on_device));
diff --git a/reveal_amd/csrc/rv_api.hip b/reveal_amd/csrc/rv_api.hip
--- a/reveal_amd/csrc/rv_api.hip
+++ b/reveal_amd/csrc/rv_api.hip
@@ -96,6 +96,8 @@
     for (auto &b : h->ps) b.release();
     h->hupload.release();
     if (h->ev_picks) { (void)hipEventDestroy(h->ev_picks); h->ev_picks = nullptr; }
+    if (h->ev_text) { (void)hipEventDestroy(h->ev_text); h->ev_text = nullptr; }
+    if (h->ev_text_in) { (void)hipEventDestroy(h->ev_text_in); h->ev_text_in = nullptr; }
     if (h->ws.stream) rv_stream_put(h->ws.stream);
     delete h;
 }
@@ -148,7 +150,7 @@
     c->ws.opt = h->ws.opt;
     const int64_t n = h->n;
     hipStream_t q = c->ws.stream;
-    bool ok = rv_upload(c) == 0;
+    bool ok = rv_upload(c) == 0 && rv_ensure_working_text(h) == 0;
     ok = ok && c->dT.reserve((size_t)n + 64) == 0 && c->dSA.reserve((size_t)(n + 64) * sizeof(sa_t)) == 0 && c->dSAi.reserve((size_t)(n + 64) * sizeof(sa_t)) == 0
             && c->dLCP.reserve((size_t)(n + 64) * sizeof(lcp_t)) == 0 && c->dBWT.reserve((size_t)n + 64) == 0 && c->dNsep.reserve((h->nsep.size() + 1) * sizeof(sa_t)) == 0;
     ok = ok && hipStreamSynchronize(h->ws.stream) == hipSuccess;
@@ -413,9 +415,10 @@
     if (h->al) (void)rv_align_end(h);
     h->nT = n;
     hipStream_t q = h->ws.stream;
+    if (h->dT_inflight) { RV_HIP(hipStreamWaitEvent(q, h->ev_text, 0)); h->dT_inflight = false; }
     RV_TRY(rv_upload(h));
     RV_TRY(h->dT.reserve((size_t)n + 64));
-    RV_HIP(hipMemcpyAsync(h->dT.p, h->dT0.p, (size_t)n + 64, hipMemcpyDeviceToDevice, q));
+    h->dT_pending = true;
     RV_TRY(h->dSA.reserve((size_t)(n + 64) * sizeof(sa_t)));
     RV_TRY(h->dSAi.reserve((size_t)(n + 64) * sizeof(sa_t)));
     RV_TRY(h->dLCP.reserve((size_t)(n + 64) * sizeof(lcp_t)));
@@ -429,8 +432,8 @@
     SaScratchInUse in_use(h->ws);
     if (!safile || !safile[0]) {
         int id = h->prof.begin(q, RV_K_SA_SORT, 5.0 * (double)n);
-        if (lcp_from_file) RV_TRY(rv_build_sa(h->ws, h->dT.as<uint8_t>(), n, h->dSA.as<sa_t>(), &h->sa_stats));
-        else RV_TRY(rv_build_sa(h->ws, h->dT.as<uint8_t>(), n, h->dSA.as<sa_t>(), &h->sa_stats, h->dLCP.as<lcp_t>(), h->dBWT.as<uint8_t>(), side_sep, d_max, &lcp_done,
+        if (lcp_from_file) RV_TRY(rv_build_sa(h->ws, h->dT0.as<uint8_t>(), n, h->dSA.as<sa_t>(), &h->sa_stats));
+        else RV_TRY(rv_build_sa(h->ws, h->dT0.as<uint8_t>(), n, h->dSA.as<sa_t>(), &h->sa_stats, h->dLCP.as<lcp_t>(), h->dBWT.as<uint8_t>(), side_sep, d_max, &lcp_done,
                                  h->nsep.data(), (int)h->nsep.size()));
         h->prof.end(q, id);
     } else {
@@ -444,7 +447,7 @@
     if (!lcp_from_file) {
         if (!lcp_done) {
             int id = h->prof.begin(q, RV_K_LCP, 13.0 * (double)n);
-            RV_TRY(rv_build_lcp(h->ws, h->dT.as<uint8_t>(), h->dSA.as<sa_t>(), false, h->dLCP.as<lcp_t>(), n, d_max, h->dBWT.as<uint8_t>(), side_sep));
+            RV_TRY(rv_build_lcp(h->ws, h->dT0.as<uint8_t>(), h->dSA.as<sa_t>(), false, h->dLCP.as<lcp_t>(), n, d_max, h->dBWT.as<uint8_t>(), side_sep));
             h->prof.end(q, id);
         }
         RV_TRY(rv_read_back(h->ws, &h->maxlcp, d_max, 4));
@@ -455,7 +458,7 @@
         for (int64_t i = 0; i < n; i++) if ((u32)tmp[(size_t)i] > mx) mx = (u32)tmp[(size_t)i];
         h->maxlcp = mx;
         RV_HIP(hipMemcpyAsync(h->dLCP.p, tmp.data(), (size_t)n * sizeof(lcp_t), hipMemcpyHostToDevice, q));
-        RV_TRY(rv_build_bwt(h->ws, h->dT.as<uint8_t>(), h->dSA.as<sa_t>(), n, h->dBWT.as<uint8_t>(), side_sep));
+        RV_TRY(rv_build_bwt(h->ws, h->dT0.as<uint8_t>(), h->dSA.as<sa_t>(), n, h->dBWT.as<uint8_t>(), side_sep));
         RV_HIP(hipStreamSynchronize(q));
     }
     if (cache == 1) {
@@ -488,6 +491,8 @@
     case RV_T:
         if (cap < n) { rv_set_error("buffer too small"); return -1; }
         if (h->constructed || h->text_only) {
+            if (rv_ensure_working_text(h) != 0) return -1;
+            if (hipStreamSynchronize(h->ws.stream) != hipSuccess) { rv_set_error("stream failed"); return -1; }
             if (hipMemcpy(out, h->dT.p, (size_t)n, hipMemcpyDeviceToHost) != hipSuccess) { rv_set_error("D2H failed"); return -1; }
         } else {
             memcpy(out, h->T.data(), (size_t)n);
@@ -540,6 +545,33 @@
     return 0;
 }
 
+int rv_ensure_working_text(rv_index *h) {
+    hipStream_t q = h->ws.stream;
+    if (h->dT_inflight) {
+        RV_HIP(hipStreamWaitEvent(q, h->ev_text, 0));
+        h->dT_inflight = false;
+    }
+    if (!h->dT_pending) return 0;
+    RV_TRY(h->dT.reserve((size_t)h->n + 64));
+    RV_HIP(hipMemcpyAsync(h->dT.p, h->dT0.p, (size_t)h->n + 64, hipMemcpyDeviceToDevice, q));
+    h->dT_pending = false;
+    return 0;
+}
+
+int rv_working_text_begin(rv_index *h, hipStream_t side) {
+    if (!h->dT_pending) return 0;
+    if (!side || side == h->ws.stream) return rv_ensure_working_text(h);
+    if (!h->ev_text) RV_HIP(hipEventCreateWithFlags(&h->ev_text, hipEventDisableTiming));
+    if (!h->ev_text_in) RV_HIP(hipEventCreateWithFlags(&h->ev_text_in, hipEventDisableTiming));
+    RV_TRY(h->dT.reserve((size_t)h->n + 64));
+    RV_HIP(hipEventRecord(h->ev_text_in, h->ws.stream));
+    RV_HIP(hipStreamWaitEvent(side, h->ev_text_in, 0));
+    RV_HIP(hipMemcpyAsync(h->dT.p, h->dT0.p, (size_t)h->n + 64, hipMemcpyDeviceToDevice, side));
+    RV_HIP(hipEventRecord(h->ev_text, side));
+    h->dT_pending = false; h->dT_inflight = true;
+    return 0;
+}
+
 int rv_text_only(rv_index *h, u32 maxlcp) {
     RV_HIP(hipSetDevice(h->device));
     if (h->n == 0) { rv_set_error("No text to index."); return -1; }
@@ -548,8 +580,8 @@
     hipStream_t q = h->ws.stream;
     h->rc = 0; h->nT = n;
     RV_TRY(rv_upload(h));
-    RV_TRY(h->dT.reserve((size_t)n + 64));
-    RV_HIP(hipMemcpyAsync(h->dT.p, h->dT0.p, (size_t)n + 64, hipMemcpyDeviceToDevice, q));
+    h->dT_pending = true;
+    RV_TRY(rv_ensure_working_text(h));
     RV_TRY(h->dSAi.reserve((size_t)(n + 64) * sizeof(sa_t)));
     std::vector<sa_t> ns(h->nsep.size() + 1, 0);
     for (size_t k = 0; k < h->nsep.size(); k++) ns[k] = (sa_t)h->nsep[k];
diff --git a/reveal_amd/csrc/rv_cascade.h b/reveal_amd/csrc/rv_cascade.h
--- a/reveal_amd/csrc/rv_cascade.h
+++ b/reveal_amd/csrc/rv_cascade.h
@@ -26,12 +26,18 @@
     DBuf *lvSA, *lvLCP, *lvBWT, *roots;
 };
 
+struct RvCascadeHost {
+    hipStream_t side = nullptr;
+    int64_t *pos = nullptr; u32 *l = nullptr; u32 cap = 0;
+};
+
 struct RvCascadeOut {
     bool done;
     int levels;
     int64_t cands, witnesses, children, undecided, rebuilt_ranks;
     int64_t solved, unsolved;
     const char *why;
+    u32 sent;
 };
 
 #define RV_CASM_K 16
@@ -51,4 +57,5 @@
 void rv_batch_group_free(RvBatchGroup *g);
 void rv_batch_group_info(const RvBatchGroup *g, int64_t *out);
 int rv_cascade_multi_run(rv_index *h, RvCascadeBufs &cb, int minl, RvCascadeMultiOut *out);
-int rv_cascade_run(rv_index *h, RvCascadeBufs &cb, const RvCascadeIO &io, int minl, RvCascadeOut *out, int danger = 0, int reuse = 0);
+int rv_cascade_run(rv_index *h, RvCascadeBufs &cb, const RvCascadeIO &io, int minl, RvCascadeOut *out, int danger = 0, int reuse = 0,
+                   const RvCascadeHost *host = nullptr);
diff --git a/reveal_amd/csrc/rv_cascade.hip b/reveal_amd/csrc/rv_cascade.hip
--- a/reveal_amd/csrc/rv_cascade.hip
+++ b/reveal_amd/csrc/rv_cascade.hip
@@ -20,7 +20,8 @@
 
 struct CasIv { sa_t a0, a1, b0, b1; };
 struct CasRes { sa_t qa, qb; u32 ql, lead, trail, state; };
-enum { C_NCHILD = 0, C_NUND = 1, C_NWIT = 2, C_ERR = 3, C_MAXN = 4, C_LO = 5, C_HI = 6, C_LEVELS = 7, C_NSOLVED = 8, C_NUNSOLVED = 9, C_NRETRY = 10, C_TICKET = 11 };
+enum { C_NCHILD = 0, C_NUND = 1, C_NWIT = 2, C_ERR = 3, C_MAXN = 4, C_LO = 5, C_HI = 6, C_LEVELS = 7, C_NSOLVED = 8, C_NUNSOLVED = 9, C_NRETRY = 10, C_TICKET = 11,
+       C_NANCH = 12  };
 
 __device__ inline bool cas_cut(const CasIv &iv, int64_t pa, int64_t pb, int64_t len, int64_t minl, int64_t *qa, int64_t *qb, int64_t *ql) {
     const int64_t ka = (int64_t)iv.a0 - pa, kb = (int64_t)iv.b0 - pb;
@@ -588,6 +589,7 @@
         if (atomicAdd(&counters[C_TICKET], 1u) == gridDim.x - 1) {
             if (hi > lo) counters[C_LEVELS]++;
             counters[C_LO] = hi; counters[C_HI] = atomicAdd(&counters[C_NCHILD], 0u);
+            counters[C_NANCH] = atomicAdd(io.anchor_count, 0u);
             counters[C_TICKET] = 0;
         }
     }
@@ -841,7 +843,7 @@
     return 0;
 }
 
-int rv_cascade_run(rv_index *h, RvCascadeBufs &cb, const RvCascadeIO &io, int minl_in, RvCascadeOut *out, int danger, int reuse) {
+int rv_cascade_run(rv_index *h, RvCascadeBufs &cb, const RvCascadeIO &io, int minl_in, RvCascadeOut *out, int danger, int reuse, const RvCascadeHost *host) {
     memset(out, 0, sizeof *out);
     out->done = false;
     Workspace &ws = h->ws;
@@ -1045,6 +1047,15 @@
     const unsigned agrid = (unsigned)(ceil_div((int64_t)M, TB * CAS_ITEMS) + ceil_div((int64_t)NW, TB * CAS_ITEMS));
     const int batch = std::max(1, (int)ws.opt.cascade_batch);
     int queued = 0;
+    RV_TRY(rv_working_text_begin(h, host ? host->side : nullptr));
+    u32 sent = 0, known = 0;
+    auto send_known = [&]() -> int {
+        if (!host || !host->side || !host->l || known <= sent || known > host->cap) return 0;
+        RV_HIP(hipMemcpyAsync(host->pos + 2 * (size_t)sent, io.anchor_pos + 2 * (size_t)sent, (size_t)(known - sent) * 16, hipMemcpyDeviceToHost, host->side));
+        RV_HIP(hipMemcpyAsync(host->l + sent, io.anchor_l + sent, (size_t)(known - sent) * 4, hipMemcpyDeviceToHost, host->side));
+        sent = known;
+        return 0;
+    };
     struct PrioScope {
         Workspace &w; hipStream_t home; RvCascadeBufs &cb; bool on = false;
         ~PrioScope() { leave(); }
@@ -1100,9 +1111,11 @@
                                bres.as<CasRes>(), minl, counters, ccap, bund.as<u32>(), (u32)RV_LEAF_N, io, dg, (danger && NW) ? 1 : 0);
             RV_LAUNCH_CHECK();
         }
+        RV_TRY(send_known());
         RV_TRY(rv_read_back(ws, hc, counters, sizeof hc));
         if (hc[C_ERR] & ~5u) { rv_set_error("cascade: device error %u", hc[C_ERR]); return -1; }
         if (hc[C_ERR]) GIVE_UP("the cascade's tables are full");
+        known = hc[C_NANCH];
         if (hc[C_MAXN] > (u32)RV_LEAF_N) break;
         if (hc[C_HI] == hc[C_LO]) break;
         if (queued > 1000000) { rv_set_error("cascade: no progress"); return -1; }
@@ -1121,6 +1134,7 @@
     }
     hipLaunchKernelGGL(k_cas_stats, dim3(256), dim3(TB), 0, q, (const u32 *)counters, (const int32_t *)bdep.as<int32_t>(), io);
     RV_LAUNCH_CHECK();
+    RV_TRY(send_known());
     if (chain) {
         hipLaunchKernelGGL(k_cas_lineage_stats, dim3(1), dim3(64), 0, q, io.stats, (unsigned long long)cb.lin_steps, (unsigned long long)cb.lin_maxdepth);
         RV_LAUNCH_CHECK();
@@ -1165,6 +1179,7 @@
                 danger ? " (second attempt)" : "", M, NW, level, hi, U, (long long)out->rebuilt_ranks, (long long)out->solved, (tp[1] - tp[0]) * 1e3, (tp[2] - tp[1]) * 1e3, (tp[3] - tp[2]) * 1e3, (tp[4] - tp[3]) * 1e3);
     }
     out->done = true;
+    out->sent = sent;
     return 0;
 #undef GIVE_UP
 }
diff --git a/reveal_amd/csrc/rv_cascade_multi.hip b/reveal_amd/csrc/rv_cascade_multi.hip
--- a/reveal_amd/csrc/rv_cascade_multi.hip
+++ b/reveal_amd/csrc/rv_cascade_multi.hip
@@ -1113,6 +1113,7 @@
 }
 
 int rv_cascade_multi_run(rv_index *h, RvCascadeBufs &cb, int minl_in, RvCascadeMultiOut *out) {
+    RV_TRY(rv_ensure_working_text(h));
     out->done = false; out->levels = 0; out->cands = out->witnesses = out->children = out->undecided = out->rebuilt_ranks = 0; out->steps = 0; out->maxdepth = 0;
     out->why = nullptr; out->big = out->big_ranks = 0; out->an_l.clear(); out->an_pos.clear(); out->meta.clear(); out->node_first.clear(); out->nodes.clear(); out->d_sa = out->d_lcp = out->d_bwt = nullptr;
     Workspace &ws = h->ws;
diff --git a/reveal_amd/csrc/rv_common.h b/reveal_amd/csrc/rv_common.h
--- a/reveal_amd/csrc/rv_common.h
+++ b/reveal_amd/csrc/rv_common.h
@@ -331,7 +331,8 @@
 int rv_radix_passes(const Workspace &ws, int nbits);
 template <class V>
 int rv_radix_sort_pairs(Workspace &ws, u64 *k0, V *v0, u64 *k1, V *v1, int64_t n,
-                        int bit_lo, int bit_hi, int *result_in_1);
+                        int bit_lo, int bit_hi, int *result_in_1, bool first_digits = false);
+uint8_t *rv_radix_first_digits(Workspace &ws, int64_t n, int bit_lo, int bit_hi);
 
 int rv_read_back(Workspace &ws, void *dst, const void *dsrc, size_t bytes);
 
diff --git a/reveal_amd/csrc/rv_construct.hip b/reveal_amd/csrc/rv_construct.hip
--- a/reveal_amd/csrc/rv_construct.hip
+++ b/reveal_amd/csrc/rv_construct.hip
@@ -63,6 +63,7 @@
     __syncthreads();
     const u32 tot = hh[threadIdx.x];
     if (tot) atomicAdd(&hist[threadIdx.x], tot);
+    if (blockIdx.x == 0 && threadIdx.x == 0) hist[257] = T[n - 1];
 }
 
 constexpr int KEY_TILE = 1024;
@@ -273,6 +274,7 @@
     for (int d = 8; d >= 1; d >>= 1) c += __shfl_down(c, d, 16);
     const int64_t tile = w >> 4;
     if ((threadIdx.x & 15) == 0 && tile < ntiles) tilecnt[tile] = c;
+    if (w == 0) tilecnt[ntiles] = 0;
 }
 struct KeyLayout { int at_shift, at_bits, nd_shift, nd_bits; u64 sortmask; };
 struct KeyPack { int g, fb, nf, gl, fbl, bits; u32 rad, fmask, lmask, lscale , fdiv ;
@@ -355,7 +357,8 @@
 template <int G>
 __global__ __launch_bounds__(TB) void k_init_keys(const uint8_t *__restrict__ T, int64_t n, const uint8_t *__restrict__ lut, int K, KeyPack kp,
                                                   u64 *__restrict__ keys, sav_t *__restrict__ vals, int pay, u32 stop0, u32 stop1,
-                                                  KeyLayout ly, DiagBits dg, const u32 *__restrict__ tw_off , int64_t ntiles) {
+                                                  KeyLayout ly, DiagBits dg, const u32 *__restrict__ tw_off , int64_t ntiles,
+                                                  uint8_t *__restrict__ dig0 ) {
     __shared__ u32 code32[IK_WORDS + 2];
     __shared__ u32 s_sc[IK_WORDS / 8 + 3];
     __shared__ uint8_t slut[256], sstop[256];
@@ -483,6 +486,7 @@
                 key |= (u64)(known ? (u32)d | ((f >> 1) << ly.nd_bits) : (u32)nd_none) << ly.nd_shift;
             }
             keys[obase + j] = key; vals[obase + j] = (sav_t)i;
+            if (dig0) dig0[obase + j] = (uint8_t)key;
         }
     } else {
     constexpr int PER = KEY_TILE / TB;
@@ -535,9 +539,10 @@
                 ulonglong2 *vd2 = reinterpret_cast<ulonglong2 *>(vals + i0);
                 vd2[0] = make_ulonglong2((u64)oval[0], (u64)oval[1]); vd2[1] = make_ulonglong2((u64)oval[2], (u64)oval[3]);
             }
+            if (dig0) *reinterpret_cast<u32 *>(dig0 + i0) = ((u32)okey[0] & 0xffu) | (((u32)okey[1] & 0xffu) << 8) | (((u32)okey[2] & 0xffu) << 16) | ((u32)okey[3] << 24);
         } else {
 #pragma unroll
-            for (int r = 0; r < PER; r++) if (i0 + r < n) { keys[i0 + r] = okey[r]; vals[i0 + r] = oval[r]; }
+            for (int r = 0; r < PER; r++) if (i0 + r < n) { keys[i0 + r] = okey[r]; vals[i0 + r] = oval[r]; if (dig0) dig0[i0 + r] = (uint8_t)okey[r]; }
         }
     } else {
 #pragma unroll
@@ -547,10 +552,11 @@
             if (i >= n) continue;
             const int xw = k >> 6, b = k & 63;
             const bool twin = (s_tw[xw] >> b) & 1ull;
-            if (i < dg.D) { keys[i] = okey[r]; vals[i] = (sav_t)i | (twin ? TW_FLAG : (sav_t)0); }
+            if (i < dg.D) { keys[i] = okey[r]; vals[i] = (sav_t)i | (twin ? TW_FLAG : (sav_t)0); if (dig0) dig0[i] = (uint8_t)okey[r]; }
             else if (!twin) {
                 const int64_t o = dg.D + (int64_t)tw_off[tile] + s_kpre[xw] + (u32)__popcll(s_keep[xw] & ((b == 0) ? 0ull : (~0ull >> (64 - b))));
                 keys[o] = okey[r]; vals[o] = (sav_t)i;
+                if (dig0) dig0[o] = (uint8_t)okey[r];
             }
         }
     }
@@ -964,7 +970,10 @@
     for (int d = 32; d >= 1; d >>= 1) c += __shfl_down(c, d, 64);
     if ((threadIdx.x & 63) == 0) wsum[threadIdx.x >> 6] = c;
     __syncthreads();
-    if (threadIdx.x == 0) tilecnt[blockIdx.x] = wsum[0] + wsum[1] + wsum[2] + wsum[3];
+    if (threadIdx.x == 0) {
+        tilecnt[blockIdx.x] = wsum[0] + wsum[1] + wsum[2] + wsum[3];
+        if (blockIdx.x + 1 == gridDim.x) tilecnt[gridDim.x] = 0;
+    }
 }
 
 __global__ __launch_bounds__(TB) void k_cp_emit(const uint8_t *__restrict__ head, int64_t n, const u32 *__restrict__ tileoff,
@@ -1017,6 +1026,7 @@
     __syncthreads();
     if (threadIdx.x == 0) {
         tilecnt[blockIdx.x] = wsum[0] + wsum[1] + wsum[2] + wsum[3];
+        if (blockIdx.x + 1 == gridDim.x) tilecnt[gridDim.x] = 0;
         u32 l = wlast[0];
         for (int k = 1; k < TB / 64; k++) l = wlast[k] > l ? wlast[k] : l;
         tilelast[blockIdx.x] = l;
@@ -1843,7 +1853,10 @@
     for (int d = 32; d >= 1; d >>= 1) c += __shfl_down(c, d, 64);
     if ((threadIdx.x & 63) == 0) wsum[threadIdx.x >> 6] = c;
     __syncthreads();
-    if (threadIdx.x == 0) tilecnt[blockIdx.x] = wsum[0] + wsum[1] + wsum[2] + wsum[3];
+    if (threadIdx.x == 0) {
+        tilecnt[blockIdx.x] = wsum[0] + wsum[1] + wsum[2] + wsum[3];
+        if (blockIdx.x + 1 == gridDim.x) tilecnt[gridDim.x] = 0;
+    }
 }
 __global__ __launch_bounds__(TB) void k_flag_emit(const uint8_t *__restrict__ flag, int64_t n, const u32 *__restrict__ tileoff,
                                                   const u32 *__restrict__ P, const sav_t *__restrict__ S, const u32 *__restrict__ G, int64_t nn, int64_t h,
@@ -2168,7 +2181,7 @@
         hipLaunchKernelGGL(k_hist256, dim3((unsigned)blocks), dim3(TB), 0, q, T, n, d_hist.as<u32>());
         RV_LAUNCH_CHECK();
     }
-    u32 hist[257];
+    u32 hist[258];
     RV_TRY(rv_read_back(ws, hist, d_hist.p, sizeof hist));
     uint8_t lut[256];
     int sigma = 0;
@@ -2178,7 +2191,7 @@
     if (sigma >= 255) for (int c = 0; c < 256; c++) lut[c] = (uint8_t)c;
     const bool short_alphabet = sigma >= 2 && sigma < 255 && T != nullptr && hist[(uint8_t)'$'] > 0 && lut[(uint8_t)'$'] == 1 && hist[256] == 0 && !ws.opt.no_short_alphabet;
     bool ends_with_sep = false;
-    if (short_alphabet) { uint8_t last = 0; RV_TRY(rv_read_back(ws, &last, T + (n - 1), 1)); ends_with_sep = last == (uint8_t)'$'; }
+    if (short_alphabet) ends_with_sep = hist[257] == (u32)(uint8_t)'$';
     if (short_alphabet && ends_with_sep) {
         for (int c = 0; c < 256; c++) lut[c] = hist[c] ? (uint8_t)(lut[c] - 1) : (uint8_t)0;
         radix = (u32)sigma;
@@ -2285,7 +2298,6 @@
         auto count_kept = [&](int tab, u32 *kept_out) -> int {
             hipLaunchKernelGGL(k_tw_count, dim3((unsigned)ceil_div(nw, TB)), dim3(TB), 0, q, (const u64 *)dg.stop, nw, K, kd.D, n, tc, ntiles, tab);
             RV_LAUNCH_CHECK();
-            RV_HIP(hipMemsetAsync(tc + ntiles, 0, 4, q));
             RV_TRY(rv_exclusive_sum_u32(ws, tc, tc, ntiles + 1));
             return rv_read_back(ws, kept_out, tc + ntiles, 4);
         };
@@ -2327,11 +2339,13 @@
         tw_off = tc;
         s.diag_table = dg.tab;
     }
+    uint8_t *dig0 = nullptr;
     {
         const int64_t iktiles = ceil_div(n, KEY_TILE);
         const dim3 ig((unsigned)std::min<int64_t>(iktiles, 256 * 8));
+        dig0 = rv_radix_first_digits(ws, nsort, 0, bits);
 #define RV_IK_(G) hipLaunchKernelGGL(k_init_keys<G>, ig, dim3(TB), 0, q, T, n, d_lut.as<uint8_t>(), K, kp, bk0.as<u64>(), bv0.as<sav_t>(), fused ? 1 : 0, \
-                                     kd.stop0, kd.stop1, kd.ly, dg, tw_off, iktiles)
+                                     kd.stop0, kd.stop1, kd.ly, dg, tw_off, iktiles, dig0)
         const int ikid = ws.prof_begin(12 , (double)n + (double)nsort * (8.0 + sizeof(sav_t) + 1.0));
         switch (kp.g) { case 1: RV_IK_(1); break; case 2: RV_IK_(2); break; case 3: RV_IK_(3); break; case 4: RV_IK_(4); break; default: RV_IK_(5); break; }
         ws.prof_end(ikid);
@@ -2339,7 +2353,7 @@
     }
     SA_HIP(hipGetLastError());
     int in1 = 0;
-    SA_TRY(rv_radix_sort_pairs<sav_t>(ws, bk0.as<u64>(), bv0.as<sav_t>(), bk1.as<u64>(), bv1.as<sav_t>(), nsort, 0, bits, &in1));
+    SA_TRY(rv_radix_sort_pairs<sav_t>(ws, bk0.as<u64>(), bv0.as<sav_t>(), bk1.as<u64>(), bv1.as<sav_t>(), nsort, 0, bits, &in1, dig0 != nullptr));
     s.radix_passes += rv_radix_passes(ws, bits); s.sorted_elems += nsort;
     u64 *ks = in1 ? bk1.as<u64>() : bk0.as<u64>();
     sav_t *vs = in1 ? bv1.as<sav_t>() : bv0.as<sav_t>();
@@ -2403,7 +2417,6 @@
         const int64_t nt = ceil_div(len, CP_TILE);
         hipLaunchKernelGGL(k_cp_count, dim3((unsigned)nt), dim3(TB), 0, q, hd, len, tile);
         RV_LAUNCH_CHECK();
-        RV_HIP(hipMemsetAsync(tile + nt, 0, 4, q));
         RV_TRY(rv_exclusive_sum_u32(ws, tile, tile, nt + 1));
         u32 tot = 0;
         RV_TRY(rv_read_back(ws, &tot, tile + nt, 4));
@@ -2422,7 +2435,6 @@
         u32 *tlast = tile + (ntile + 1);
         hipLaunchKernelGGL(k_cp_count_g, dim3((unsigned)ntile), dim3(TB), 0, q, (const uint8_t *)head, n, tile, tlast);
         SA_HIP(hipGetLastError());
-        SA_HIP(hipMemsetAsync(tile + ntile, 0, 4, q));
         SA_TRY(rv_exclusive_sum_u32(ws, tile, tile, ntile + 1));
         SA_TRY(rv_inclusive_max_u32(ws, tlast, tlast, ntile));
         u32 tot = 0;
@@ -2558,7 +2570,6 @@
             const int64_t nt = ceil_div(m, CP_TILE);
             hipLaunchKernelGGL(k_flag_count, dim3((unsigned)nt), dim3(TB), 0, q, (const uint8_t *)bigflag, m, tile);
             SA_HIP(hipGetLastError());
-            SA_HIP(hipMemsetAsync(tile + nt, 0, 4, q));
             SA_TRY(rv_exclusive_sum_u32(ws, tile, tile, nt + 1));
             u32 mbig = 0;
             SA_TRY(rv_read_back(ws, &mbig, tile + nt, 4));
diff --git a/reveal_amd/csrc/rv_index.h b/reveal_amd/csrc/rv_index.h
--- a/reveal_amd/csrc/rv_index.h
+++ b/reveal_amd/csrc/rv_index.h
@@ -118,6 +118,8 @@
     bool sai_valid = false;
     DBuf dT, dT0, dSA, dSAi, dLCP, dBWT, dNsep;
     bool text_dirty = true;
+    bool dT_pending = false, dT_inflight = false;
+    hipEvent_t ev_text = nullptr, ev_text_in = nullptr;
     bool text_only = false;
     HBuf hscan;
     HBuf hupload;
@@ -151,4 +153,7 @@
 
 int rv_need_sai(rv_index *h);
 
+int rv_ensure_working_text(rv_index *h);
+int rv_working_text_begin(rv_index *h, hipStream_t side);
+
 void rv_align_free(rv_index *h);
diff --git a/reveal_amd/csrc/rv_many.hip b/reveal_amd/csrc/rv_many.hip
--- a/reveal_amd/csrc/rv_many.hip
+++ b/reveal_amd/csrc/rv_many.hip
@@ -332,6 +332,8 @@
     RV_TRY(many_collect(m, h, -1, ord, abeg, bbeg));
     m->info[4] += st.levels + (m->recs.size() > rec0 ? 2 : 0);
     std::vector<char> txt((size_t)n);
+    RV_TRY(rv_ensure_working_text(h));
+    RV_HIP(hipStreamSynchronize(h->ws.stream));
     RV_HIP(hipMemcpy(txt.data(), h->dT.p, (size_t)n, hipMemcpyDeviceToHost));
     for (size_t s = 0; s < J; s++) {
         ManyJob &jb = m->jobs[(size_t)ord[s]];
diff --git a/reveal_amd/csrc/rv_prims.hip b/reveal_amd/csrc/rv_prims.hip
--- a/reveal_amd/csrc/rv_prims.hip
+++ b/reveal_amd/csrc/rv_prims.hip
@@ -307,8 +307,16 @@
     return nbits <= 0 ? 0 : (nbits + w - 1) / w;
 }
 
+static bool rs_digit_bytes(const Workspace &ws, int64_t n, int bit_lo, int bit_hi) {
+    return ws.opt.rs_bits != 10 && !ws.opt.rs_no_digit_bytes && n > 1 && n >= ((int64_t)1 << 20) && n < ((int64_t)1 << 32) && bit_hi - bit_lo > 8;
+}
+uint8_t *rv_radix_first_digits(Workspace &ws, int64_t n, int bit_lo, int bit_hi) {
+    if (!rs_digit_bytes(ws, n, bit_lo, bit_hi) || ws.rs_digits.reserve((size_t)n + 64)) return nullptr;
+    return ws.rs_digits.as<uint8_t>();
+}
+
 template <class V>
-int rv_radix_sort_pairs(Workspace &ws, u64 *k0, V *v0, u64 *k1, V *v1, int64_t n, int bit_lo, int bit_hi, int *result_in_1) {
+int rv_radix_sort_pairs(Workspace &ws, u64 *k0, V *v0, u64 *k1, V *v1, int64_t n, int bit_lo, int bit_hi, int *result_in_1, bool first_digits) {
     *result_in_1 = 0;
     if (n <= 1 || bit_hi <= bit_lo) return 0;
     if (n >= ((int64_t)1 << 32)) { rv_set_error("radix sort: n >= 2^32 not supported"); return -1; }
@@ -317,10 +325,11 @@
     const u32 nb = (u32)ceil_div(n, RS_TILE);
     RV_TRY(ws.rs_hist.reserve(((size_t)1 << width) * nb * sizeof(u32)));
     u32 *bh = ws.rs_hist.as<u32>();
-    const bool bytes = width == 8 && !ws.opt.rs_no_digit_bytes && n >= ((int64_t)1 << 20) && bit_hi - bit_lo > width;
+    const bool bytes = rs_digit_bytes(ws, n, bit_lo, bit_hi);
+    if (first_digits && (!bytes || ws.rs_digits.cap < (size_t)n + 64)) { rv_set_error("radix sort: first digits announced but the byte path is off"); return -1; }
     if (bytes) RV_TRY(ws.rs_digits.reserve((size_t)n + 64));
     uint8_t *dig = bytes ? ws.rs_digits.as<uint8_t>() : nullptr;
-    bool have_digits = false;
+    bool have_digits = first_digits;
     u64 *ki = k0, *ko = k1;
     V *vi = v0, *vo = v1;
     int flip = 0;
@@ -383,5 +392,5 @@
     return 0;
 }
 
-template int rv_radix_sort_pairs<u32>(Workspace &, u64 *, u32 *, u64 *, u32 *, int64_t, int, int, int *);
-template int rv_radix_sort_pairs<u64>(Workspace &, u64 *, u64 *, u64 *, u64 *, int64_t, int, int, int *);
+template int rv_radix_sort_pairs<u32>(Workspace &, u64 *, u32 *, u64 *, u32 *, int64_t, int, int, int *, bool);
+template int rv_radix_sort_pairs<u64>(Workspace &, u64 *, u64 *, u64 *, u64 *, int64_t, int, int, int *, bool);
```

Measured after the change: 23030, median of 6. 1.04x the previous value.
